# Belis0811/MaskUnet

Hardware: AMD Instinct MI355X
Metric: 128x128 images/sec (fwd+bwd) (higher is better)
Workload: dtype f16; 1 GPU; ADE20K-semantic shape 128x128, c_out=150, batch=64/GPU, 1-head MaskAttn-UNet fwd+bwd, train mode; global_batch=64, parallelism=dp1, mask_mode=fixed, loss=maskunet_amd.CrossEntropyLoss on module output, optimizer_in_step=False, hip_graph=False

## Files before the change

include/maskunet_hip.h:

```cpp
#ifndef MASKUNET_HIP_H
#define MASKUNET_HIP_H

#ifdef __cplusplus
extern "C" {
#endif

#define MU_OK 0
#define MU_ERR_ARG (-1)
#define MU_ERR_SHAPE (-2)
#define MU_ERR_LAUNCH (-3)
#define MU_ERR_WORKSPACE (-4)

#define MU_F32 0
#define MU_F16 1
#define MU_F32X 2

#define MU_ACT_NONE 0
#define MU_ACT_GELU 1
#define MU_ACT_RELU 2

const char* mu_version_host(void);

int mu_transpose(const void* src, int src_dtype, long src_ld, void* dst, int dst_dtype, long dst_ld, int batch, int R, int C,
                 void* stream);
int mu_transpose_pad(const void* src, int src_dtype, long src_ld, void* dst, int dst_dtype, long dst_ld, int batch, int R, int C,
                     int R_pad, void* stream);
int mu_split_encode(const void* src, void* dst, long n_elems, void* stream);
int mu_split_encode_h4(const void* src, void* dst, long n_elems, void* stream);
int mu_split_encode_h4x(const void* src, void* dst, void* dst16, long n_elems, void* stream);
long mu_dy_encode_h_workspace_bytes(void);
int mu_dy_encode_h(const void* dy, void* dy_h, float* dy_scale, long n_elems, void* workspace, long ws_bytes, void* stream);
int mu_split_encode_h(const void* src, void* dst, long n_elems, void* stream);
int mu_conv1x1_fwd_enc_h(const void* x, const void* w, const float* bias, void* y, long M, int Cin, int Cout, long x_ld, long y_ld,
                         void* stream);
int mu_cast(const void* src, int src_dtype, void* dst, int dst_dtype, long n, void* stream);
int mu_prep_weight(const float* w_oihw, void* dst, int dtype, int O, int I, int taps, int rows_pad, int cols_pad, int mode,
                   void* stream);

int mu_prep_weights_multi(const void* jobs, int njobs, long ntiles, void* dst_base, int dtype, void* stream);

int mu_prep_qkv(const float* wq, const float* wk, const float* wv, const float* bq, const float* bk, const float* bv, void* dst,
                float* bias, int dtype, int C, void* stream);

int mu_conv_fwd(const void* x, const void* w, const float* bias, void* y, int B, int H, int W, int Cin, int Cout, int taps, long x_ld,
                long y_ld, int dtype, void* stream);
int mu_conv1x1_add_supported(int Cin, int Cout, int dtype);
int mu_conv1x1_fwd_add(const void* x, const void* w, const void* addend, void* y, long M, int Cin, int Cout, long x_ld, long y_ld, int dtype,
                       void* stream);
int mu_conv_fwd_fused(const void* x, const void* w, const float* scale, const float* shift, const void* res, int act, void* y, int B, int H,
                      int W, int Cin, int Cout, int taps, long x_ld, long y_ld, int dtype, void* stream);
int mu_conv_stats_rows(int B, int H, int W, int Cin, int Cout, int taps, int dtype);
int mu_conv_fwd_stats(const void* x, const void* w, const float* bias, void* y, int B, int H, int W, int Cin, int Cout, int taps,
                      long x_ld, long y_ld, int dtype, float* stat_part, void* stream);
int mu_conv_fwd_plan(int B, int H, int W, int Cin, int Cout, int taps, int dtype, int with_stats);
int mu_conv_fwd_fused_plan(int B, int H, int W, int Cin, int Cout, int taps, int dtype);
int mu_conv_dgrad_h_plan(int B, int H, int W, int Cin, int Cout);
int mu_conv_wgrad_plan(int B, int H, int W, int Cin, int Cout, int taps, int cin_valid, int dtype, int pair);
int mu_conv_wgrad_bias_plan(int B, int H, int W, int Cin, int Cout, int taps, int cin_valid, int dtype);
int mu_conv_plan_count(int op);
const char* mu_conv_plan_name(int op, int id);
int mu_conv_dgrad_h(const void* dy_h, const void* w_hl, const float* dy_scale, void* dx, int B, int H, int W, int Cin, int Cout, long dy_ld,
                    long dx_ld, void* stream);
long mu_conv_wgrad_h_workspace_bytes(int B, int H, int W, int Cin, int Cout);
int mu_conv_wgrad_h(const void* x, const void* dy_h, const float* dy_scale, float* dw_oihw, int B, int H, int W, int Cin, int Cout,
                    int cin_valid, int cout_valid, long x_ld, long dy_ld, void* workspace, long ws_bytes, void* stream);
int mu_conv_wgrad_h1(const void* x_h, const void* dy_h, const float* dy_scale, float* dw_oihw, int B, int H, int W, int Cin, int Cout,
                     int cin_valid, int cout_valid, long x_ld, long dy_ld, void* workspace, long ws_bytes, void* stream);
long mu_conv_wgrad_workspace_bytes(int B, int H, int W, int Cin, int Cout, int taps);
int mu_conv_wgrad(const void* x, const void* dy, float* dw_oihw, int B, int H, int W, int Cin, int Cout, int taps, int cin_valid,
                  int cout_valid, long x_ld, long dy_ld, void* workspace, long ws_bytes, int dtype, void* stream);
int mu_conv_wgrad_bias_supported(int Cin, int Cout, int taps, int dtype);
int mu_conv_wgrad_bias(const void* x, const void* dy, float* dw_oihw, float* db, int B, int H, int W, int Cin, int Cout, int taps,
                       int cin_valid, int cout_valid, long x_ld, long dy_ld, void* workspace, long ws_bytes, int dtype, void* stream);
long mu_colsum_workspace_bytes(int C);
int mu_colsum(const void* x, long M, int C, long ld, float* out, void* workspace, long ws_bytes, int dtype, void* stream);

long mu_bn_workspace_bytes(int C);
int mu_bn_train_stats(const void* x, long M, int C, long ld, float* mean, float* rstd, float* running_mean, float* running_var,
                      long* num_batches_tracked, int c_valid, float momentum, float eps, void* workspace, long ws_bytes, int dtype,
                      void* stream);
int mu_bn_train_stats_rows(const float* stat_part, int rows, long M, int C, float* mean, float* rstd, float* running_mean,
                           float* running_var, long* num_batches_tracked, int c_valid, float momentum, float eps, void* workspace,
                           long ws_bytes, void* stream);
int mu_bn_eval_stats(const float* running_mean, const float* running_var, float eps, float* mean, float* rstd, int C, int c_valid,
                     void* stream);
int mu_bn_eval_fold(const float* running_mean1, const float* running_var1, const float* gamma1, const float* beta1, float eps1,
                    const float* running_mean2, const float* running_var2, const float* gamma2, const float* beta2, float eps2,
                    const float* conv_bias, float* scale, float* shift, int C, int c_valid, void* stream);
int mu_bn_act_fwd(const void* x, const void* res, void* y, long M, int C, long ld, const float* mean, const float* rstd,
                  const float* gamma, const float* beta, int act, int dtype, void* stream);
int mu_bn_act_fwd_enc(const void* x, const void* res, void* y_enc, void* y16, long M, int C, const float* mean, const float* rstd,
                      const float* gamma, const float* beta, int act, void* stream);
int mu_bn_act_bwd(const void* x, const void* res, const void* grad_out, void* dx, void* dres, long M, int C, long ld,
                  const float* mean, const float* rstd, const float* gamma, const float* beta, int act, int training, float* dgamma,
                  float* dbeta, void* workspace, long ws_bytes, int dtype, void* stream);
int mu_bn_pair_compose(const float* rstd1, const float* gamma1, const float* beta1, const float* gamma2, int C, int c_valid, long M,
                       float eps1, float eps2, float momentum2, float* running_mean2, float* running_var2,
                       long* num_batches_tracked2, float* gamma_eff, float* xhat_scale, float* dgamma2_coef, float* dgamma1_coef,
                       void* stream);
int mu_bn_act_bwd_scaled(const void* x, const void* res, const void* grad_out, void* dx, void* dres, long M, int C, long ld,
                         const float* mean, const float* rstd, const float* gamma, const float* beta, int act, int training,
                         float* dgamma, float* dbeta, const float* xhat_scale, void* workspace, long ws_bytes, int dtype, void* stream);

int mu_bn_pair_bwd(const void* x, const void* grad_out, void* dx, long M, int C, long ld, const float* mean, const float* rstd,
                   const float* gamma_eff, const float* beta2, const float* xhat_scale, const float* dgamma2_coef,
                   const float* dgamma1_coef, float* pair_grads, float* dbeta2, void* workspace, long ws_bytes, int dtype, void* stream);

int mu_bn_act_bwd_h(const void* x, const void* res, const void* grad_out, void* dx_h, void* dres, long M, int C, const float* mean,
                    const float* rstd, const float* gamma, const float* beta, int act, int training, float* dgamma, float* dbeta,
                    float* dy_scale, void* workspace, long ws_bytes, void* stream);
int mu_bn_pair_bwd_h(const void* x, const void* grad_out, void* dx_h, long M, int C, const float* mean, const float* rstd,
                     const float* gamma_eff, const float* beta2, const float* xhat_scale, const float* dgamma2_coef,
                     const float* dgamma1_coef, float* pair_grads, float* dbeta2, float* dy_scale, void* workspace, long ws_bytes,
                     void* stream);

long mu_ln_sample_workspace_bytes(int B);
int mu_ln_sample_fwd(const void* x, const float* w, const float* b, void* y, float* mean, float* rstd, int B, long L, float eps,
                     void* workspace, long ws_bytes, int dtype, void* stream);
int mu_ln_sample_bwd(const void* x, const void* dy, const float* w, const float* mean, const float* rstd, void* dx, float* dw,
                     float* db, int B, long L, void* workspace, long ws_bytes, int dtype, void* stream);

int mu_maxpool2_fwd(const void* x, void* y, int B, int H, int W, int C, int dtype, void* stream);
int mu_maxpool2_bwd(const void* x, const void* dy, void* dx, int B, int H, int W, int C, int dtype, void* stream);
int mu_maxpool2_bwd_acc(const void* x, const void* dy, const void* dy2, const void* dx_add, void* dx, int B, int H, int W, int C, int dtype,
                        void* stream);
int mu_upcat_fwd(const void* x, const void* skip, void* y, int B, int h, int w, int Cx, int Cs, int dtype, void* stream);
int mu_upcat_bwd(const void* dy, void* dx, void* dskip, int B, int h, int w, int Cx, int Cs, int dtype, void* stream);
int mu_upcat_bwd_acc(const void* dy, const void* dy2, void* dx, void* dskip, int B, int h, int w, int Cx, int Cs, int dtype, void* stream);
int mu_upcat_compact_fwd(const void* x, const void* skip, void* y, int B, int h, int w, int Cx_ld, int Cx_valid, int Cs_ld, int Cs_valid,
                         int Ct_ld, int dtype, void* stream);
int mu_upcat_compact_bwd(const void* dy, void* dx, void* dskip, int B, int h, int w, int Cx_ld, int Cx_valid, int Cs_ld, int Cs_valid,
                         int Ct_ld, int dtype, void* stream);
int mu_dropout(const void* x, void* y, long n, float p, unsigned long long seed, const unsigned char* mask, unsigned char* mask_out,
               int dtype, void* stream);
int mu_dropout_step(const void* x, void* y, long n, float p, unsigned long long seed, const unsigned long long* seed_step,
                    const unsigned char* mask, unsigned char* mask_out, int dtype, void* stream);

int mu_add(const void* a, const void* b, void* out, long n, int dtype, void* stream);

int mu_compact_keys(const void* keep, int keep_elem_bytes, int B, int N, int* kidx, int* kcnt, unsigned char* keep8, void* stream);
int mu_attn_fwd(const void* qkv, const void* x, const int* kidx, const int* kcnt, const float* gamma, const float* beta, void* out,
                void* oattn, float* lse2, float* ln_mean, float* ln_rstd, int B, int N, int C, int nkmax, float eps, int dtype,
                void* stream);
long mu_attn_bwd_workspace_bytes(int B, int N, int C);
int mu_attn_bwd(const void* qkv, const void* x, const void* oattn, const void* grad_out, const int* kidx, const int* kcnt,
                const float* lse2, const float* ln_mean, const float* ln_rstd, const float* gamma, void* dY, float* delta, void* dqkv,
                float* dgamma, float* dbeta, int B, int N, int C, int nkmax, void* workspace, long ws_bytes, int dtype, void* stream);
int mu_attn_fwd_padded(const void* qkv, const void* x, const int* kidx, const int* kcnt, const float* gamma, const float* beta, void* out,
                       void* oattn, float* lse2, float* ln_mean, float* ln_rstd, int B, int N, int C, int c_valid, int nkmax, float eps,
                       int dtype, void* stream);
int mu_attn_bwd_phases_padded(const void* qkv, const void* x, const void* oattn, const void* grad_out, const int* kidx, const int* kcnt,
                              const float* lse2, const float* ln_mean, const float* ln_rstd, const float* gamma, void* dY, float* delta,
                              void* dqkv, float* dgamma, float* dbeta, int B, int N, int C, int c_valid, int nkmax, void* workspace,
                              long ws_bytes, int dtype, int phases, void* stream);
int mu_gather_rows(const void* src, long src_ld, const int* idx, const int* cnt, void* dst, int rows_out, int C, int dtype, void* stream);
int mu_scatter_rows(const float* src, const int* idx, const int* cnt, void* dst, long dst_ld, int dst_rows, int C, int dtype, void* stream);
int mu_softmax_rows(void* S, int N, int ld, const int* cnt, float scale, int dtype, void* stream);
int mu_attn_wide_ds(const void* P, void* dP, int N, int ld, const int* cnt, float scale, int dtype, void* stream);
int mu_ln_rows_fwd(const void* o, const void* x, const float* gamma, const float* beta, void* out, float* mean, float* rstd, long rows,
                   int C, int c_valid, float eps, int dtype, void* stream);
int mu_ln_rows_bwd(const void* grad_out, const void* o, const void* x, const float* mean, const float* rstd, const float* gamma, void* dY,
                   void* g_xhat, long rows, int C, int c_valid, int dtype, void* stream);
#define MU_ATTN_KIDX_PERMUTATION 8
#define MU_ATTN_DQKV_ENCODED 16
int mu_attn_bwd_phases(const void* qkv, const void* x, const void* oattn, const void* grad_out, const int* kidx, const int* kcnt,
                       const float* lse2, const float* ln_mean, const float* ln_rstd, const float* gamma, void* dY, float* delta,
                       void* dqkv, float* dgamma, float* dbeta, int B, int N, int C, int nkmax, void* workspace, long ws_bytes,
                       int dtype, int phases, void* stream);

long mu_ce_workspace_bytes(void);
int mu_ce_fwd(const void* logits, const long* labels, long M, int Cp, int C, long ignore_index, float* lse, float* loss, float* count,
              void* workspace, long ws_bytes, int dtype, void* stream);
int mu_ce_bwd(const void* logits, const long* labels, const float* lse, const float* count, const float* grad_out, float grad_scale,
              long M, int Cp, int C, long ignore_index, void* dlogits, int dtype, void* stream);
int mu_ce_nchw_fwd(const void* logits, const long* labels, int B, int C, long HW, long ignore_index, float* lse, float* loss,
                   float* count, void* workspace, long ws_bytes, int dtype, void* stream);
int mu_ce_nchw_bwd(const void* logits, const long* labels, const float* lse, const float* count, const float* grad_out,
                   float grad_scale, int B, int C, long HW, long ignore_index, void* dlogits, int dtype, void* stream);
int mu_mean_iou(const void* logits, const long* labels, long M, int C, long inner, long outer_stride, long c_stride, long p_stride,
                float smooth, unsigned int* counts, float* out, int dtype, void* stream);
long mu_inst_triplet_workspace_bytes(int id_cap, int max_inst);
int mu_inst_triplet_fwd(const float* feat, const long* mask, int B, int C, int H, int W, int ignore_label, float margin,
                        const float* u, int id_cap, int max_inst, void* workspace, long ws_bytes, float* loss, void* stream);
int mu_inst_triplet_bwd(const float* feat, int B, int C, int H, int W, const void* workspace, int id_cap, int max_inst,
                        const float* grad_out, float* dfeat, void* stream);
int mu_argmax_prob(const void* logits, long M, int C, long inner, long outer_stride, long c_stride, long p_stride,
                   float inv_temperature, int* cls, float* prob_or_null, int dtype, void* stream);
long mu_instances_workspace_bytes(int B, int H, int W, int max_inst);
int mu_instances_supported(int H, int W, int max_inst);
int mu_instances(const int* cls, const float* prob_or_null, int B, int H, int W, int max_inst, int* ids, int* table, float* score,
                 int* count, int* order, void* workspace, long ws_bytes, void* stream);
long mu_dbscan_workspace_bytes(int B, int H, int W, int num_classes, int max_inst);
int mu_dbscan_supported(int H, int W, int D, int num_classes, int max_inst);
int mu_dbscan_instances(const int* cls, const void* emb, int B, int H, int W, int D, long inner, long outer_stride, long c_stride,
                        long p_stride, int dtype, int num_classes, float eps, int min_samples, int max_inst, int* ids, int* table,
                        float* score, int* count, int* order, void* workspace, long ws_bytes, void* stream);
#define MU_IDMAP_I32 0
#define MU_IDMAP_I64 1
#define MU_IDMAP_RGB8 2
int mu_id_instances_supported(int H, int W, int max_inst, int class_cap);
long mu_id_instances_workspace_bytes(int B, int H, int W, int max_inst, int class_cap);
int mu_id_instances(const void* id_map, int id_kind, const int* sem, int B, int H, int W, int max_inst, int class_cap, int* ids,
                    int* table, float* score, int* count, int* order, int* values, int* invalid, void* workspace, long ws_bytes,
                    void* stream);
#define MU_SEM_EVAL_LDS_MAX_C 192
int mu_sem_eval_supported(int C);
long mu_sem_eval_workspace_bytes(int B, long HW, int C);
int mu_sem_eval(const void* logits, const long* labels, int B, long HW, int C, long inner, long outer_stride, long c_stride,
                long p_stride, long ignore_index, float inv_temperature, int* img_counts, double* img_loss, long* confusion,
                int* cls_or_null, float* prob_or_null, void* workspace, long ws_bytes, int dtype, void* stream);
int mu_instance_pairs_supported(int H, int W, int max_inst_pred, int max_inst_gt);
long mu_instance_pairs_workspace_bytes(int B, int H, int W, int max_inst_pred, int max_inst_gt);
int mu_instance_pairs(const int* pred_ids, const int* gt_ids, int B, int H, int W, int max_inst_pred, int max_inst_gt, int* pairs,
                      int* n_pairs, void* workspace, long ws_bytes, void* stream);
int mu_instance_match_supported(int H, int W, int max_inst_pred, int max_inst_gt, int num_classes, int K, int max_dets, int T);
long mu_instance_match_workspace_bytes(int B, int K);
int mu_instance_match(const int* pairs, const int* n_pairs, const int* pred_table, const float* pred_score, const int* pred_order,
                      const int* pred_count, const int* gt_table, const int* gt_count, int B, int H, int W, int max_inst_pred,
                      int max_inst_gt, int num_classes, int K, int max_dets, const double* thr, int T, int* det_valid, int* det_class,
                      float* det_score, int* det_gt, double* det_iou, int* gt_per_class, int* pq_gt, double* pq_iou, int* pq_fp,
                      int* overflow, void* workspace, long ws_bytes, void* stream);
int mu_coco_match_supported(int H, int W, int max_inst_pred, int max_inst_gt, int num_classes, int K, int max_dets, int T, int A);
long mu_coco_match_workspace_bytes(int B, int K);
int mu_coco_match(const int* pairs, const int* n_pairs, const int* pred_table, const float* pred_score, const int* pred_order,
                  const int* pred_count, const int* gt_table, const int* gt_count, const int* gt_crowd_or_null,
                  const double* gt_area_or_null, int B, int H, int W, int max_inst_pred, int max_inst_gt, int num_classes, int K,
                  int max_dets, const double* thr, int T, const double* area_rng, int A, int* det_valid, int* det_class, int* det_rank,
                  float* det_score, int* det_gt, double* det_iou, unsigned char* det_ignore, int* gt_counted, int* pq_gt_per_class,
                  int* pq_gt, double* pq_iou, int* pq_fp, int* overflow, void* workspace, long ws_bytes, void* stream);
int mu_rle_encode_supported(int H, int W, int K, int max_id);
long mu_rle_encode_workspace_bytes(int B, int H, int W, int K, int max_id);
int mu_rle_encode(const int* ids, const int* sel, int B, int H, int W, int K, int max_id, int* offsets, int* counts, int* area,
                  int* str_offsets, unsigned char* str_bytes, void* workspace, long ws_bytes, void* stream);
int mu_rle_decode_supported(int H, int W, int K);
int mu_rle_decode(const int* offsets, const int* counts, int B, int H, int W, int K, long counts_per_image, int* ids, int* valid,
                  void* stream);
int mu_coco_masks_supported(int Ho, int Wo, int max_points);
long mu_coco_masks_workspace_bytes(int B, int A, int Ho, int Wo);
int mu_coco_masks(const double* xy, const int* poly_offsets, const int* ann_poly_offsets, const int* rle_counts, const int* ann_rle_offsets,
                  const int* img_ann_offsets, const int* sizes, int B, int A, int P, long n_points, long n_counts, int Ho, int Wo,
                  int max_points, long* cover, int* ids, unsigned char* masks_or_null, int* area, int* valid, void* workspace,
                  long ws_bytes, void* stream);
int mu_u8_to_nhwc(const unsigned char* src, void* dst, long npix, int C, int Cp, int dtype, void* stream);
int mu_resize_u8_nhwc(const unsigned char* src, int B, int Hs, int Ws, int C, int swap_rb, void* dst, unsigned char* u8_out, int Hd, int Wd,
                      int Cp, int dtype, void* stream);
int mu_resize_nearest_u8(const unsigned char* src, int B, int Hs, int Ws, long* dst, int Hd, int Wd, void* stream);
long mu_pil_resize_workspace_bytes(int B, int max_h, int max_w, int Hd, int Wd);
int mu_pil_resize_u8_nhwc(const unsigned char* src, const long* offsets, const int* sizes, int B, int C, int max_h, int max_w, int swap_rb,
// ... 14 lines not shown
```

maskunet_amd/_lib.py:

```python
from __future__ import annotations

import ctypes
import os
from ctypes import c_char_p, c_float, c_int, c_long, c_ulonglong, c_void_p

import torch

_HERE = os.path.dirname(os.path.abspath(__file__))
LIB_PATH = os.environ.get("MU_LIB_PATH") or os.path.join(_HERE, "libmaskunet_hip.so")

MU_F32, MU_F16, MU_F32X = 0, 1, 2
ACT_NONE, ACT_GELU, ACT_RELU = 0, 1, 2
MU_IDMAP_I32, MU_IDMAP_I64, MU_IDMAP_RGB8 = 0, 1, 2
_ERR = {-1: "MU_ERR_ARG", -2: "MU_ERR_SHAPE", -3: "MU_ERR_LAUNCH", -4: "MU_ERR_WORKSPACE"}

P, I, L, F = c_void_p, c_int, c_long, c_float
SIGNATURES = {
    "mu_version_host": (c_char_p, []),
    "mu_transpose": (I, [P, I, L, P, I, L, I, I, I, P]),
    "mu_transpose_pad": (I, [P, I, L, P, I, L, I, I, I, I, P]),
    "mu_cast": (I, [P, I, P, I, L, P]),
    "mu_split_encode": (I, [P, P, L, P]),
    "mu_split_encode_h": (I, [P, P, L, P]),
    "mu_split_encode_h4": (I, [P, P, L, P]),
    "mu_split_encode_h4x": (I, [P, P, P, L, P]),
    "mu_conv_wgrad_h1": (I, [P, P, P, P, I, I, I, I, I, I, I, L, L, P, L, P]),
    "mu_bn_act_fwd_enc": (I, [P, P, P, P, L, I, P, P, P, P, I, P]),
    "mu_dy_encode_h_workspace_bytes": (L, []),
    "mu_dy_encode_h": (I, [P, P, P, L, P, L, P]),
    "mu_conv_dgrad_h": (I, [P, P, P, P, I, I, I, I, I, L, L, P]),
    "mu_conv_wgrad_h_workspace_bytes": (L, [I, I, I, I, I]),
    "mu_conv_wgrad_h": (I, [P, P, P, P, I, I, I, I, I, I, I, L, L, P, L, P]),
    "mu_bn_act_bwd_h": (I, [P, P, P, P, P, L, I, P, P, P, P, I, I, P, P, P, P, L, P]),
    "mu_bn_pair_bwd_h": (I, [P, P, P, L, I, P, P, P, P, P, P, P, P, P, P, P, L, P]),
    "mu_conv1x1_fwd_enc_h": (I, [P, P, P, P, L, I, I, L, L, P]),
    "mu_prep_weight": (I, [P, P, I, I, I, I, I, I, I, P]),
    "mu_conv_fwd": (I, [P, P, P, P, I, I, I, I, I, I, L, L, I, P]),
    "mu_conv_stats_rows": (I, [I, I, I, I, I, I, I]),
    "mu_conv_fwd_plan": (I, [I, I, I, I, I, I, I, I]),
    "mu_conv_fwd_fused_plan": (I, [I, I, I, I, I, I, I]),
    "mu_conv_dgrad_h_plan": (I, [I, I, I, I, I]),
    "mu_conv_wgrad_plan": (I, [I, I, I, I, I, I, I, I, I]),
    "mu_conv_wgrad_bias_plan": (I, [I, I, I, I, I, I, I, I]),
    "mu_conv_plan_count": (I, [I]),
    "mu_conv_plan_name": (c_char_p, [I, I]),
    "mu_conv_fwd_stats": (I, [P, P, P, P, I, I, I, I, I, I, L, L, I, P, P]),
    "mu_conv_wgrad_workspace_bytes": (L, [I, I, I, I, I, I]),
    "mu_conv_wgrad": (I, [P, P, P, I, I, I, I, I, I, I, I, L, L, P, L, I, P]),
    "mu_conv_wgrad_bias_supported": (I, [I, I, I, I]),
    "mu_conv_wgrad_bias": (I, [P, P, P, P, I, I, I, I, I, I, I, I, L, L, P, L, I, P]),
    "mu_colsum_workspace_bytes": (L, [I]),
    "mu_colsum": (I, [P, L, I, L, P, P, L, I, P]),
    "mu_bn_workspace_bytes": (L, [I]),
    "mu_bn_train_stats": (I, [P, L, I, L, P, P, P, P, P, I, F, F, P, L, I, P]),
    "mu_bn_train_stats_rows": (I, [P, I, L, I, P, P, P, P, P, I, F, F, P, L, P]),
    "mu_bn_eval_stats": (I, [P, P, F, P, P, I, I, P]),
    "mu_bn_act_fwd": (I, [P, P, P, L, I, L, P, P, P, P, I, I, P]),
    "mu_bn_act_bwd": (I, [P, P, P, P, P, L, I, L, P, P, P, P, I, I, P, P, P, L, I, P]),
    "mu_bn_pair_compose": (I, [P, P, P, P, I, I, L, F, F, F, P, P, P, P, P, P, P, P]),
    "mu_bn_act_bwd_scaled": (I, [P, P, P, P, P, L, I, L, P, P, P, P, I, I, P, P, P, P, L, I, P]),
    "mu_bn_pair_bwd": (I, [P, P, P, L, I, L, P, P, P, P, P, P, P, P, P, P, L, I, P]),
    "mu_ln_sample_workspace_bytes": (L, [I]),
    "mu_ln_sample_fwd": (I, [P, P, P, P, P, P, I, L, F, P, L, I, P]),
    "mu_ln_sample_bwd": (I, [P, P, P, P, P, P, P, P, I, L, P, L, I, P]),
    "mu_maxpool2_fwd": (I, [P, P, I, I, I, I, I, P]),
    "mu_maxpool2_bwd": (I, [P, P, P, I, I, I, I, I, P]),
    "mu_upcat_fwd": (I, [P, P, P, I, I, I, I, I, I, P]),
    "mu_upcat_bwd": (I, [P, P, P, I, I, I, I, I, I, P]),
    "mu_upcat_compact_fwd": (I, [P, P, P, I, I, I, I, I, I, I, I, I, P]),
    "mu_upcat_compact_bwd": (I, [P, P, P, I, I, I, I, I, I, I, I, I, P]),
    "mu_dropout": (I, [P, P, L, F, c_ulonglong, P, P, I, P]),
    "mu_dropout_step": (I, [P, P, L, F, c_ulonglong, P, P, P, I, P]),
    "mu_add": (I, [P, P, P, L, I, P]),
    "mu_attn_fwd": (I, [P, P, P, P, P, P, P, P, P, P, P, I, I, I, I, F, I, P]),
    "mu_attn_bwd_workspace_bytes": (L, [I, I, I]),
    "mu_attn_bwd": (I, [P, P, P, P, P, P, P, P, P, P, P, P, P, P, P, I, I, I, I, P, L, I, P]),
    "mu_gather_rows": (I, [P, L, P, P, P, I, I, I, P]),
    "mu_scatter_rows": (I, [P, P, P, P, L, I, I, I, P]),
    "mu_softmax_rows": (I, [P, I, I, P, F, I, P]),
    "mu_attn_wide_ds": (I, [P, P, I, I, P, F, I, P]),
    "mu_ln_rows_fwd": (I, [P, P, P, P, P, P, P, L, I, I, F, I, P]),
    "mu_ln_rows_bwd": (I, [P, P, P, P, P, P, P, P, L, I, I, I, P]),
    "mu_ce_workspace_bytes": (L, []),
    "mu_ce_fwd": (I, [P, P, L, I, I, L, P, P, P, P, L, I, P]),
    "mu_ce_bwd": (I, [P, P, P, P, P, F, L, I, I, L, P, I, P]),
    "mu_ce_nchw_fwd": (I, [P, P, I, I, L, L, P, P, P, P, L, I, P]),
    "mu_ce_nchw_bwd": (I, [P, P, P, P, P, F, I, I, L, L, P, I, P]),
    "mu_mean_iou": (I, [P, P, L, I, L, L, L, L, F, P, P, I, P]),
    "mu_sem_eval_supported": (I, [I]),
    "mu_sem_eval_workspace_bytes": (L, [I, L, I]),
    "mu_sem_eval": (I, [P, P, I, L, I, L, L, L, L, L, F, P, P, P, P, P, P, L, I, P]),
    "mu_inst_triplet_workspace_bytes": (L, [I, I]),
    "mu_inst_triplet_fwd": (I, [P, P, I, I, I, I, I, F, P, I, I, P, L, P, P]),
    "mu_inst_triplet_bwd": (I, [P, I, I, I, I, P, I, I, P, P, P]),
    "mu_argmax_prob": (I, [P, L, I, L, L, L, L, F, P, P, I, P]),
    "mu_instances_workspace_bytes": (L, [I, I, I, I]),
    "mu_instances_supported": (I, [I, I, I]),
    "mu_instances": (I, [P, P, I, I, I, I, P, P, P, P, P, P, L, P]),
    "mu_dbscan_workspace_bytes": (L, [I, I, I, I, I]),
    "mu_dbscan_supported": (I, [I, I, I, I, I]),
    "mu_dbscan_instances": (I, [P, P, I, I, I, I, L, L, L, L, I, I, F, I, I, P, P, P, P, P, P, L, P]),
    "mu_id_instances_supported": (I, [I, I, I, I]),
    "mu_id_instances_workspace_bytes": (L, [I, I, I, I, I]),
    "mu_id_instances": (I, [P, I, P, I, I, I, I, I] + [P] * 8 + [L, P]),
    "mu_instance_pairs_supported": (I, [I, I, I, I]),
    "mu_instance_pairs_workspace_bytes": (L, [I, I, I, I, I]),
    "mu_instance_pairs": (I, [P, P, I, I, I, I, I, P, P, P, L, P]),
    "mu_instance_match_supported": (I, [I, I, I, I, I, I, I, I]),
    "mu_instance_match_workspace_bytes": (L, [I, I]),
    "mu_instance_match": (I, [P] * 8 + [I] * 8 + [P, I] + [P] * 10 + [P, L, P]),
    "mu_coco_match_supported": (I, [I, I, I, I, I, I, I, I, I]),
    "mu_coco_match_workspace_bytes": (L, [I, I]),
    "mu_coco_match": (I, [P] * 10 + [I] * 8 + [P, I, P, I] + [P] * 13 + [P, L, P]),
    "mu_rle_encode_supported": (I, [I, I, I, I]),
    "mu_rle_encode_workspace_bytes": (L, [I, I, I, I, I]),
    "mu_rle_encode": (I, [P, P, I, I, I, I, I, P, P, P, P, P, P, L, P]),
    "mu_rle_decode_supported": (I, [I, I, I]),
    "mu_rle_decode": (I, [P, P, I, I, I, I, L, P, P, P]),
    "mu_coco_masks_supported": (I, [I, I, I]),
    "mu_coco_masks_workspace_bytes": (L, [I, I, I, I]),
    "mu_coco_masks": (I, [P] * 7 + [I, I, I, L, L, I, I, I] + [P] * 6 + [L, P]),
    "mu_u8_to_nhwc": (I, [P, P, L, I, I, I, P]),
    "mu_adamw_chunk": (I, []),
    "mu_adamw_multi": (I, [P, P, P, I, I, F, F, F, F, F, F, P, P, I, P, P]),
    "mu_prep_qkv": (I, [P, P, P, P, P, P, P, P, I, I, P]),
    "mu_prep_weights_multi": (I, [P, I, L, P, I, P]),
    "mu_conv1x1_add_supported": (I, [I, I, I]),
    "mu_conv1x1_fwd_add": (I, [P, P, P, P, L, I, I, L, L, I, P]),
    "mu_maxpool2_bwd_acc": (I, [P, P, P, P, P, I, I, I, I, I, P]),
    "mu_upcat_bwd_acc": (I, [P, P, P, P, I, I, I, I, I, I, P]),
    "mu_compact_keys": (I, [P, I, I, I, P, P, P, P]),
    "mu_resize_u8_nhwc": (I, [P, I, I, I, I, I, P, P, I, I, I, I, P]),
    "mu_resize_nearest_u8": (I, [P, I, I, I, P, I, I, P]),
    "mu_pil_resize_workspace_bytes": (L, [I, I, I, I, I]),
    "mu_pil_resize_u8_nhwc": (I, [P, P, P, I, I, I, I, I, P, P, P, I, I, I, I, P, L, P]),
    "mu_conv_fwd_fused": (I, [P, P, P, P, P, I, P, I, I, I, I, I, I, L, L, I, P]),
    "mu_bn_eval_fold": (I, [P, P, P, P, F, P, P, P, P, F, P, P, P, I, I, P]),
    "mu_attn_bwd_phases": (I, [P, P, P, P, P, P, P, P, P, P, P, P, P, P, P, I, I, I, I, P, L, I, I, P]),
    "mu_clock_probe": (I, [P, P, I, I, P]),
    "mu_attn_fwd_padded": (I, [P, P, P, P, P, P, P, P, P, P, P, I, I, I, I, I, F, I, P]),
    "mu_attn_bwd_phases_padded": (I, [P, P, P, P, P, P, P, P, P, P, P, P, P, P, P, I, I, I, I, I, P, L, I, I, P]),
}

_lib = None


def load() -> ctypes.CDLL:
    global _lib
    if _lib is not None:
        return _lib
    if not os.path.exists(LIB_PATH):
        raise RuntimeError(
            f"maskunet_amd: HIP library not found at {LIB_PATH}. It must be built (hipcc --offload-arch=gfx950): "
            "run `make -C maskunet_amd/csrc` or `python -c 'import __graft_entry__ as g; g.build()'`. "
            "There is no CPU fallback.")
    lib = ctypes.CDLL(LIB_PATH)
    for name, (res, args) in SIGNATURES.items():
        if os.environ.get("MU_LIB_PATH") and not hasattr(lib, name):
            continue
        fn = getattr(lib, name)
        fn.restype = res
        fn.argtypes = args
    _lib = lib
    return lib


def dt(t_or_dtype) -> int:
    d = t_or_dtype.dtype if isinstance(t_or_dtype, torch.Tensor) else t_or_dtype
    if d == torch.float32:
        return MU_F32
    if d == torch.float16:
        return MU_F16
    raise TypeError(f"maskunet_amd supports float32 and float16 compute, got {d}")


F32_MATMUL_PRECISION = os.environ.get("MU_F32_MATMUL", "highest")
if F32_MATMUL_PRECISION not in ("highest", "high"):
    raise ValueError(f'MU_F32_MATMUL must be "highest" or "high", got {F32_MATMUL_PRECISION!r}')


def set_float32_matmul_precision(precision: str):
    global F32_MATMUL_PRECISION
    if precision not in ("highest", "high"):
        raise ValueError('precision must be "highest" or "high"')
    F32_MATMUL_PRECISION = precision


def get_float32_matmul_precision() -> str:
    return F32_MATMUL_PRECISION


def mdt(t_or_dtype) -> int:
    d = dt(t_or_dtype)
    return MU_F32X if (d == MU_F32 and F32_MATMUL_PRECISION == "high") else d


def ptr(t):
    if t is None:
        return None
# ... 54 lines not shown
```

maskunet_amd/csrc/conv.hip:

```cpp
#include "common.h"
#include <stdlib.h>
#include <type_traits>
#include "../../include/maskunet_hip.h"

template <typename T> struct Mma;
template <> struct Mma<h16> {
    static constexpr int VN = 8;
    using Frag = h16x8;
    static __device__ __forceinline__ Frag ld(const void* p) { return *reinterpret_cast<const Frag*>(p); }
    static __device__ __forceinline__ void mma(const Frag& a, const Frag& b, f32x4& c) {
        c = __builtin_amdgcn_mfma_f32_16x16x32_f16(a, b, c, 0, 0, 0);
    }
    static constexpr bool PAIR = false;
    using Frag2 = Frag;
    static __device__ __forceinline__ Frag2 ld2(const void* p0, const void*) { return ld(p0); }
    static __device__ __forceinline__ void mma2(const Frag2& a, const Frag2& b, f32x4& c) { mma(a, b, c); }
};
template <> struct Mma<xf32> {
    static constexpr int VN = 4;
    using Frag = SplitF4;
    static __device__ __forceinline__ Frag ld(const void* p) { return mu_frag_enc(*reinterpret_cast<const uint4*>(p)); }
    static __device__ __forceinline__ void mma(const Frag& a, const Frag& b, f32x4& c) { mu_mma_split(a, b, c); }
    static constexpr bool PAIR = true;
    using Frag2 = SplitF8;
// ... 357 lines not shown
    for (int i = 0; i < TM; ++i)
#pragma unroll
        for (int j = 0; j < TN; ++j) acc[i][j] = (f32x4){0.f, 0.f, 0.f, 0.f};

    stage(0, 0);
    __syncthreads();
    for (int s = 0; s < nsteps; ++s) {
        const int buf = s & 1;
        if (s + 1 < nsteps) stage(s + 1, buf ^ 1);
        const char* Ab = lds + buf * STAGE;
        const char* Bb = Ab + BCO * 128;
        if constexpr (M_::PAIR) {
            typename M_::Frag2 a[TM], b[TN];
#pragma unroll
            for (int i = 0; i < TM; ++i) {
                const int row = (wr * TM + i) * 16 + r16;
                a[i] = M_::ld2(Ab + row * 128 + ((g ^ (row & 7)) << 4), Ab + row * 128 + (((4 + g) ^ (row & 7)) << 4));
            }
#pragma unroll
            for (int j = 0; j < TN; ++j) {
                const int row = (wc * TN + j) * 16 + r16;
                b[j] = M_::ld2(Bb + row * 128 + ((g ^ (row & 7)) << 4), Bb + row * 128 + (((4 + g) ^ (row & 7)) << 4));
            }
#pragma unroll
            for (int i = 0; i < TM; ++i)
#pragma unroll
                for (int j = 0; j < TN; ++j) M_::mma2(a[i], b[j], acc[i][j]);
        } else {
#pragma unroll
        for (int kk = 0; kk < 2; ++kk) {
            Frag a[TM], b[TN];
#pragma unroll
            for (int i = 0; i < TM; ++i) {
                const int row = (wr * TM + i) * 16 + r16;
                a[i] = M_::ld(Ab + row * 128 + (((kk * 4 + g) ^ (row & 7)) << 4));
            }
#pragma unroll
            for (int j = 0; j < TN; ++j) {
                const int row = (wc * TN + j) * 16 + r16;
                b[j] = M_::ld(Bb + row * 128 + (((kk * 4 + g) ^ (row & 7)) << 4));
            }
#pragma unroll
            for (int i = 0; i < TM; ++i)
#pragma unroll
                for (int j = 0; j < TN; ++j) M_::mma(a[i], b[j], acc[i][j]);
        }
        }
        __syncthreads();
    }
    mma_unshift<T>(acc);

    if constexpr (EPI) {
#pragma unroll
        for (int j = 0; j < TN; ++j) {
            const int px = (wc * TN + j) * 16 + r16;
#pragma unroll
            for (int i = 0; i < TM; ++i) {
                const int co = (wr * TM + i) * 16 + 4 * g;
                float v[4];
#pragma unroll
                for (int r = 0; r < 4; ++r) {
                    const bool in = co0 + co + r < Cout;
                    v[r] = acc[i][j][r];
                    if constexpr (FEPI) { if (scale && in) v[r] *= scale[co0 + co + r]; }
                    v[r] += (bias && in ? bias[co0 + co + r] : 0.f);
                }
                h16x4 o = {(h16)v[0], (h16)v[1], (h16)v[2], (h16)v[3]};
                *reinterpret_cast<h16x4*>(lds + px * OPITCH + co * 2) = o;
            }
        }
        __syncthreads();
        constexpr int CH = BCO / 8;
        for (int idx = tid; idx < BPX * CH; idx += 256) {
            const int px = idx / CH, ch = idx - px * CH;
            const long p = px0 + px;
            if (p < Mtot && co0 + ch * 8 < Cout) {
                uint4 o = *reinterpret_cast<const uint4*>(lds + px * OPITCH + ch * 16);
                if constexpr (FEPI) {
                    uint4 a4 = make_uint4(0, 0, 0, 0);
                    if (addend) a4 = *reinterpret_cast<const uint4*>(addend + p * y_ld + co0 + ch * 8);
                    const h16x8 ov = *reinterpret_cast<const h16x8*>(&o), av = *reinterpret_cast<const h16x8*>(&a4);
                    h16x8 r;
#pragma unroll
                    for (int e = 0; e < 8; ++e) r[e] = (h16)epi_act<T>((float)ov[e] + (float)av[e], act);
                    o = *reinterpret_cast<const uint4*>(&r);
                }
                *reinterpret_cast<uint4*>(y + p * y_ld + co0 + ch * 8) = o;
            }
        }
        return;
    }
#pragma unroll
    for (int j = 0; j < TN; ++j) {
        const long p = px0 + (wc * TN + j) * 16 + r16;
        if (p >= Mtot) continue;
#pragma unroll
        for (int i = 0; i < TM; ++i) {
            const int co = co0 + (wr * TM + i) * 16 + 4 * g;
            if (co >= Cout) continue;
            float v[4];
#pragma unroll
            for (int r = 0; r < 4; ++r) {
                v[r] = acc[i][j][r];
                if constexpr (FEPI) { if (scale) v[r] *= scale[co + r]; }
                v[r] += (bias ? bias[co + r] : 0.f);
                if constexpr (FEPI) v[r] = epi_act<T>(v[r] + (addend ? (float)addend[p * y_ld + co + r] : 0.f), act);
            }
            if constexpr (sizeof(T) == 2) {
                h16x4 o = {(h16)v[0], (h16)v[1], (h16)v[2], (h16)v[3]};
                *reinterpret_cast<h16x4*>(y + p * y_ld + co) = o;
            } else {
                if constexpr (std::is_same<T, xf32>::value && !FEPI) {
                    if (act == MU_NT2_ENC_H) {
                        uint32_t h0, h1, l0, l1;
                        mu_hsplit2(v[0], v[1], h0, l0);
                        mu_hsplit2(v[2], v[3], h1, l1);
                        char* gp = reinterpret_cast<char*>(y + p * y_ld + (co & ~7)) + (g & 1) * 8;
                        *reinterpret_cast<uint2*>(gp) = make_uint2(h0, h1);
                        *reinterpret_cast<uint2*>(gp + 16) = make_uint2(l0, l1);
                        continue;
                    }
                }
                *reinterpret_cast<float4*>(y + p * y_ld + co) = make_float4(v[0], v[1], v[2], v[3]);
            }
        }
    }
}


__device__ __forceinline__ void tile_stats_accum(const h16x8& o, float (&ssum)[8], float (&ssq)[8]) {
#pragma unroll
    for (int c = 0; c < 8; ++c) {
        const float v = (float)o[c];
        ssum[c] += v;
        ssq[c] = fmaf(v, v, ssq[c]);
    }
}
__device__ __forceinline__ void tile_stats_store(float (&ssum)[8], float (&ssq)[8], float* __restrict__ row, int co, int lane) {
#pragma unroll
    for (int c = 0; c < 8; ++c) {
#pragma unroll
        for (int m = 8; m < 64; m <<= 1) {
            ssum[c] += __shfl_xor(ssum[c], m);
            ssq[c] += __shfl_xor(ssq[c], m);
        }
    }
    if (lane < 8) {
#pragma unroll
        for (int c = 0; c < 8; c += 2)
            *reinterpret_cast<float4*>(row + (co + c) * 2) = make_float4(ssum[c], ssq[c], ssum[c + 1], ssq[c + 1]);
    }
}

template <typename T, int TM, int TN, int WR, bool RINGP, bool FEPI, int HL = 0>
__device__ __forceinline__ void conv_nt3_body(const T* __restrict__ x, const T* __restrict__ w, const float* __restrict__ bias,
                                              T* __restrict__ y, int B, int H, int W, int Cin, int Cout, long x_ld, long y_ld,
                                              const float* __restrict__ scale, const T* __restrict__ res, int act,
                                              float* __restrict__ stat_part = nullptr, float* __restrict__ yf = nullptr,
                                              const float* __restrict__ oscale = nullptr) {
    using M_ = Mma<T>;
    using Frag = typename M_::Frag;
    constexpr int VN = M_::VN, KC = 8 * VN;
    constexpr int NWV = 4;
    constexpr int WC = NWV / WR;
    constexpr int BCO = WR * TM * 16;
    constexpr int TH = WC * TN, TW = 16, HW_ = TW + 2;
    constexpr int HROWS = (TH + 2) * HW_;
    constexpr int HINST = (HROWS + 7) / 8;
    static_assert((HINST + NWV - 1) / NWV <= 9, "halo does not fit the 9 tap steps");
    constexpr int PA = BCO / (8 * NWV);
    static_assert(BCO % (8 * NWV) == 0, "weight tile rows must split over the waves");
    constexpr int HBYTES = HINST * 1024, WBYTES = BCO * 128;
    constexpr bool RING = RINGP && sizeof(T) == 2 && BCO == 64;
    constexpr int NWS = RING ? 3 : 2;

    __shared__ __attribute__((aligned(16))) char lds[2 * HBYTES + NWS * WBYTES + (RING ? 1024 : 0)];
    char* Hs = lds;
    char* Ws = lds + 2 * HBYTES;
    char* dump = lds + 2 * HBYTES + NWS * WBYTES;

    const int tiles_w = W / TW, tiles_h = H / TH;
    const int ntile = B * tiles_h * tiles_w, ncb = Cout / BCO;
    const int L = xcd_remap(blockIdx.x, ntile * ncb);
    const int cb = L % ncb, tl = L / ncb;
    const int co0 = cb * BCO;
    const int tw_ = tl % tiles_w, th_ = (tl / tiles_w) % tiles_h, bimg = tl / (tiles_w * tiles_h);
    const int h0 = th_ * TH, w0 = tw_ * TW;

    const int tid = threadIdx.x, lane = tid & 63, wave = tid >> 6;
    const int wr = wave / WC, wc = wave % WC;
    const int r16 = lane & 15, g = lane >> 4;
    const int srow = lane >> 3, sch = lane & 7;

    constexpr bool HL2 = HL == 2;
    const int kchunks = HL2 ? 2 * (Cin / KC) : Cin / KC;
    const int Cw = HL ? 2 * Cin : Cin;
    const int nsteps = 9 * kchunks;

    int wl[PA];
#pragma unroll
    for (int i = 0; i < PA; ++i) {
        const int row = (i * NWV + wave) * 8 + srow;
        wl[i] = (co0 + row) * Cw + (sch ^ (row & 7)) * VN;
    }
    constexpr int HPW = (HINST + NWV - 1) / NWV;
    int hl[HPW];
#pragma unroll
    for (int k = 0; k < HPW; ++k) {
        const int hr = (k * NWV + wave) * 8 + srow;
        const int hy = hr / HW_, hx = hr - hy * HW_;
        const int hh = h0 - 1 + hy, ww = w0 - 1 + hx;
        const bool ok = (k * NWV + wave) < HINST && hr < HROWS && hh >= 0 && hh < H && ww >= 0 && ww < W;
        hl[k] = ok ? (int)(((long)hh * W + ww) * x_ld) + (sch ^ (hx & 7)) * VN : -1;
    }
    const T* xb = x + (long)bimg * H * W * x_ld;

    auto stage_w = [&](int s, int buf) {
        const int tap = s % 9, c_ = s / 9;
        const int ci0 = HL2 ? ((c_ & 1) ? Cin : 0) + (c_ >> 1) * KC : c_ * KC;
        const T* wb = w + (long)tap * Cout * Cw + ci0;
        char* Wb = Ws + buf * WBYTES;
#pragma unroll
        for (int i = 0; i < PA; ++i) glds16(wb + wl[i], Wb + (i * NWV + wave) * 1024);
    };
    auto stage_h = [&](int k, int ci0, int buf) {
        const void* src = hl[k] >= 0 ? (const void*)(xb + hl[k] + ci0) : (const void*)mu_zero_page;
        glds16(src, Hs + buf * HBYTES + (k * NWV + wave) * 1024);
    };
    auto hchunk = [&](int c) { return HL2 ? (c >> 1) : c; };
    auto next_h = [&](int c) { return c + 1 < kchunks && (!HL2 || ((c + 1) & 1) == 0); };

    f32x4 acc[TM][TN];
#pragma unroll
    for (int i = 0; i < TM; ++i)
#pragma unroll
        for (int j = 0; j < TN; ++j) acc[i][j] = (f32x4){0.f, 0.f, 0.f, 0.f};

    int aoff[2], boff[3][2];
#pragma unroll
    for (int kk = 0; kk < 2; ++kk) {
        aoff[kk] = (wr * TM * 16 + r16) * 128 + (((kk * 4 + g) ^ (r16 & 7)) << 4);
#pragma unroll
        for (int dw = 0; dw < 3; ++dw) boff[dw][kk] = (wc * TN * HW_ + r16 + dw) * 128 + (((kk * 4 + g) ^ ((r16 + dw) & 7)) << 4);
    }

    stage_w(0, 0);
    if constexpr (RING) { if (nsteps > 1) stage_w(1, 1); }
#pragma unroll
    for (int k = 0; k < HPW; ++k)
        if (k * NWV + wave < HINST) stage_h(k, 0, 0);
    __syncthreads();

    int s = 0, wslot = 0;
    for (int c = 0; c < kchunks; ++c) {
        const int hbuf = (hchunk(c) & 1) * HBYTES;
#pragma unroll
        for (int dh = 0; dh < 3; ++dh) {
#pragma unroll
            for (int dw = 0; dw < 3; ++dw, ++s) {
                const int t = dh * 3 + dw;
                if constexpr (RING) {
                    const int nslot = wslot == 0 ? 2 : wslot - 1;
                    if (s + 2 < nsteps) stage_w(s + 2, nslot);
                    else {
#pragma unroll
                        for (int i = 0; i < PA; ++i) glds16(mu_zero_page, dump);
                    }
                    if (t < HPW && next_h(c) && t * NWV + wave < HINST) stage_h(t, hchunk(c + 1) * KC, hchunk(c + 1) & 1);
                    else glds16(mu_zero_page, dump);
                } else {
                if (s + 1 < nsteps) stage_w(s + 1, (s + 1) & 1);
                if (t < HPW && next_h(c) && t * NWV + wave < HINST)
                    stage_h(t, hchunk(c + 1) * KC, hchunk(c + 1) & 1);
                }
                const char* Wb = Ws + (RING ? wslot : (s & 1)) * WBYTES;
                const char* Hb = Hs + hbuf + dh * (HW_ * 128);
                if constexpr (M_::PAIR) {
                    typename M_::Frag2 a[TM], b[TN];
#pragma unroll
                    for (int i = 0; i < TM; ++i) a[i] = M_::ld2(Wb + aoff[0] + i * 2048, Wb + aoff[1] + i * 2048);
#pragma unroll
                    for (int j = 0; j < TN; ++j) b[j] = M_::ld2(Hb + boff[dw][0] + j * (HW_ * 128), Hb + boff[dw][1] + j * (HW_ * 128));
#pragma unroll
                    for (int i = 0; i < TM; ++i)
#pragma unroll
                        for (int j = 0; j < TN; ++j) M_::mma2(a[i], b[j], acc[i][j]);
                } else {
#pragma unroll
                for (int kk = 0; kk < 2; ++kk) {
                    Frag a[TM], b[TN];
                    const char* wa = Wb + aoff[kk];
                    const char* hb = Hb + boff[dw][kk];
#pragma unroll
                    for (int i = 0; i < TM; ++i) a[i] = M_::ld(wa + i * 2048);
#pragma unroll
                    for (int j = 0; j < TN; ++j) b[j] = M_::ld(hb + j * (HW_ * 128));
#pragma unroll
                    for (int i = 0; i < TM; ++i)
#pragma unroll
                        for (int j = 0; j < TN; ++j) M_::mma(a[i], b[j], acc[i][j]);
                }
                }
                if constexpr (RING) {
                    asm volatile("s_waitcnt vmcnt(%0)" ::"n"(PA + 1) : "memory");
                    __builtin_amdgcn_sched_barrier(0);
                    __builtin_amdgcn_s_barrier();
                    __builtin_amdgcn_sched_barrier(0);
                    wslot = wslot == 2 ? 0 : wslot + 1;
                } else {
                    __syncthreads();
                }
            }
        }
    }
    if constexpr (RING) {
        asm volatile("s_waitcnt vmcnt(0)" ::: "memory");
        __builtin_amdgcn_s_barrier();
    }

    mma_unshift<T>(acc);
    if constexpr (HL) {
        const float os = oscale[1] * (1.0f / (float)(1 << MU_XH_WSHIFT));
#pragma unroll
        for (int j = 0; j < TN; ++j) {
            const long p = ((long)bimg * H + h0 + wc * TN + j) * W + w0 + r16;
#pragma unroll
            for (int i = 0; i < TM; ++i) {
                const int co = co0 + (wr * TM + i) * 16 + 4 * g;
                *reinterpret_cast<f32x4*>(yf + p * y_ld + co) = acc[i][j] * os;
            }
        }
        return;
    }
    if constexpr (sizeof(T) == 2 && TM == 4) {
        char* Os = lds + wave * (TN * 16 * 128);
#pragma unroll
        for (int j = 0; j < TN; ++j) {
            const int p = j * 16 + r16;
#pragma unroll
            for (int i = 0; i < TM; ++i) {
                const int co = i * 16 + 4 * g;
                float v[4];
#pragma unroll
                for (int r = 0; r < 4; ++r) {
                    v[r] = acc[i][j][r];
                    if constexpr (FEPI) { if (scale) v[r] *= scale[co0 + wr * 64 + co + r]; }
                    v[r] += (bias ? bias[co0 + wr * 64 + co + r] : 0.f);
                }
                h16x4 o = {(h16)v[0], (h16)v[1], (h16)v[2], (h16)v[3]};
                *reinterpret_cast<h16x4*>(Os + p * 128 + (((co >> 2) ^ (((p >> 1) & 7) << 1)) << 3)) = o;
            }
        }
        const int q = lane & 7;
        float ssum[8] = {0.f, 0.f, 0.f, 0.f, 0.f, 0.f, 0.f, 0.f}, ssq[8] = {0.f, 0.f, 0.f, 0.f, 0.f, 0.f, 0.f, 0.f};
#pragma unroll
        for (int it = 0; it < TN * 2; ++it) {
            const int p = it * 8 + (lane >> 3);
            h16x8 o = *reinterpret_cast<const h16x8*>(Os + p * 128 + ((q ^ ((p >> 1) & 7)) << 4));
            const long gp = ((long)bimg * H + h0 + wc * TN + (p >> 4)) * W + w0 + (p & 15);
            if constexpr (FEPI) {
                h16x8 rv = (h16x8)(h16)0;
                if (res) rv = *reinterpret_cast<const h16x8*>(res + gp * y_ld + co0 + wr * 64 + q * 8);
#pragma unroll
                for (int e = 0; e < 8; ++e) o[e] = (h16)epi_act<T>((float)o[e] + (float)rv[e], act);
            }
            *reinterpret_cast<h16x8*>(y + gp * y_ld + co0 + wr * 64 + q * 8) = o;
            if constexpr (!FEPI) { if (stat_part) tile_stats_accum(o, ssum, ssq); }
        }
        if constexpr (!FEPI) {
            if (stat_part) tile_stats_store(ssum, ssq, stat_part + ((long)tl * WC + wc) * Cout * 2, co0 + wr * 64 + q * 8, lane);
        }
        return;
    }
    float tsum[TM][4], tsq[TM][4];
#pragma unroll
    for (int i = 0; i < TM; ++i)
#pragma unroll
        for (int r = 0; r < 4; ++r) { tsum[i][r] = 0.f; tsq[i][r] = 0.f; }
#pragma unroll
    for (int j = 0; j < TN; ++j) {
        const long p = ((long)bimg * H + h0 + wc * TN + j) * W + w0 + r16;
#pragma unroll
        for (int i = 0; i < TM; ++i) {
            const int co = co0 + (wr * TM + i) * 16 + 4 * g;
            float v[4];
#pragma unroll
            for (int r = 0; r < 4; ++r) {
                v[r] = acc[i][j][r];
                if constexpr (FEPI) { if (scale) v[r] *= scale[co + r]; }
                v[r] += (bias ? bias[co + r] : 0.f);
                if constexpr (FEPI) v[r] = epi_act<T>(v[r] + (res ? (float)res[p * y_ld + co + r] : 0.f), act);
            }
            if constexpr (sizeof(T) == 2) {
                h16x4 o = {(h16)v[0], (h16)v[1], (h16)v[2], (h16)v[3]};
                *reinterpret_cast<h16x4*>(y + p * y_ld + co) = o;
            } else {
                *reinterpret_cast<float4*>(y + p * y_ld + co) = make_float4(v[0], v[1], v[2], v[3]);
                if constexpr (!FEPI) {
#pragma unroll
                    for (int r = 0; r < 4; ++r) { tsum[i][r] += v[r]; tsq[i][r] = fmaf(v[r], v[r], tsq[i][r]); }
                }
            }
        }
    }
    if constexpr (!FEPI && sizeof(T) == 4) {
        if (stat_part) {
            static_assert(TM == 4, "statistics epilogue: four channel fragments per wave");
            float v8[2][4][2], v4[4][2], v2[2][2], v1[2];
            const bool b3 = r16 & 8, b2 = r16 & 4, b1 = r16 & 2, b0 = r16 & 1;
#pragma unroll
            for (int i = 0; i < 2; ++i)
#pragma unroll
                for (int r = 0; r < 4; ++r) {
                    const float ks = b3 ? tsum[i + 2][r] : tsum[i][r], ss = b3 ? tsum[i][r] : tsum[i + 2][r];
                    const float kq = b3 ? tsq[i + 2][r] : tsq[i][r], sq = b3 ? tsq[i][r] : tsq[i + 2][r];
                    v8[i][r][0] = ks + __shfl_xor(ss, 8);
                    v8[i][r][1] = kq + __shfl_xor(sq, 8);
                }
#pragma unroll
            for (int r = 0; r < 4; ++r)
#pragma unroll
                for (int k = 0; k < 2; ++k) v4[r][k] = (b2 ? v8[1][r][k] : v8[0][r][k]) + __shfl_xor(b2 ? v8[0][r][k] : v8[1][r][k], 4);
#pragma unroll
            for (int r = 0; r < 2; ++r)
#pragma unroll
                for (int k = 0; k < 2; ++k) v2[r][k] = (b1 ? v4[r + 2][k] : v4[r][k]) + __shfl_xor(b1 ? v4[r][k] : v4[r + 2][k], 2);
#pragma unroll
            for (int k = 0; k < 2; ++k) v1[k] = (b0 ? v2[1][k] : v2[0][k]) + __shfl_xor(b0 ? v2[0][k] : v2[1][k], 1);
            float* row = stat_part + ((long)tl * WC + wc) * Cout * 2;
            *reinterpret_cast<float2*>(row + (co0 + (wr * TM + (r16 >> 2)) * 16 + 4 * g + (r16 & 3)) * 2) = make_float2(v1[0], v1[1]);
        }
    }
}


template <typename T, int TM, int TN, int WR, bool RINGP = false>
__global__ __launch_bounds__(256, 2) void conv_nt3_kernel(const T* __restrict__ x, const T* __restrict__ w, const float* __restrict__ bias,
                                                          T* __restrict__ y, int B, int H, int W, int Cin, int Cout, long x_ld, long y_ld,
                                                          float* __restrict__ stat_part = nullptr) {
    conv_nt3_body<T, TM, TN, WR, RINGP, false>(x, w, bias, y, B, H, W, Cin, Cout, x_ld, y_ld, nullptr, nullptr, 0, stat_part);
}
template <int TM, int TN, int WR, bool RINGP = false, int HL = 2>
__global__ __launch_bounds__(256, 2) void conv_nt3hl_kernel(const h16* __restrict__ dy, const h16* __restrict__ w, float* __restrict__ dx, int B, int H,
                                                            int W, int Cin, int Cout, long x_ld, long y_ld, const float* __restrict__ oscale) {
    conv_nt3_body<h16, TM, TN, WR, RINGP, false, HL>(dy, w, nullptr, nullptr, B, H, W, Cin, Cout, x_ld, y_ld, nullptr, nullptr, 0, nullptr, dx, oscale);
}
template <typename T, int TM, int TN, int WR>
__global__ __launch_bounds__(256, 2) void conv_nt3f_kernel(const T* __restrict__ x, const T* __restrict__ w, const float* __restrict__ bias,
                                                           T* __restrict__ y, int B, int H, int W, int Cin, int Cout, long x_ld, long y_ld,
                                                           const float* __restrict__ scale, const T* __restrict__ res, int act) {
    conv_nt3_body<T, TM, TN, WR, false, true>(x, w, bias, y, B, H, W, Cin, Cout, x_ld, y_ld, scale, res, act);
}

template <bool FEPI, int HL = 0>
__device__ __forceinline__ void conv_nt4_body(const h16* __restrict__ x, const h16* __restrict__ w, const float* __restrict__ bias,
                                              h16* __restrict__ y, int B, int H, int W, int Cin, int Cout, long x_ld, long y_ld,
                                              float* __restrict__ stat_part, const float* __restrict__ scale, const h16* __restrict__ res, int act,
                                              float* __restrict__ yf = nullptr, const float* __restrict__ oscale = nullptr) {
    using M_ = Mma<h16>;
    using Frag = M_::Frag;
    constexpr int VN = 8, KC = 64, TM = 4, TN = 4, WC = 4, NWV = 8, BCO = 128;
    constexpr int TH = 16, TW = 16, HW_ = TW + 2, HROWS = (TH + 2) * HW_;
    constexpr int HINST = (HROWS + 7) / 8;
    constexpr int HPW = 7;
    static_assert(HPW * NWV >= HINST, "halo does not fit the 7 tap steps");
    constexpr int HBYTES = HINST * 1024, WBYTES = BCO * 128, NWB = 4;

    __shared__ __attribute__((aligned(16))) char lds[2 * HBYTES + NWB * WBYTES + 1024];
    char* Hs = lds;
    char* Ws = lds + 2 * HBYTES;
    char* dump = lds + 2 * HBYTES + NWB * WBYTES;

    const int tiles_w = W / TW, tiles_h = H / TH;
    const int ntile = B * tiles_h * tiles_w, ncb = Cout / BCO;
    const int L = xcd_remap(blockIdx.x, ntile * ncb);
    const int cb = L % ncb, tl = L / ncb;
    const int co0 = cb * BCO;
    const int tw_ = tl % tiles_w, th_ = (tl / tiles_w) % tiles_h, bimg = tl / (tiles_w * tiles_h);
    const int h0 = th_ * TH, w0 = tw_ * TW;

    const int tid = threadIdx.x, lane = tid & 63, wave = __builtin_amdgcn_readfirstlane(tid >> 6);
    const int wr = wave >> 2, wc = wave & 3;
    const int r16 = lane & 15, g = lane >> 4;
    const int srow = lane >> 3, sch = lane & 7;

    constexpr bool HL2 = HL == 2;
    const int kchunks = HL2 ? 2 * (Cin / KC) : Cin / KC;
    const int Cw = HL ? 2 * Cin : Cin;
    const int nsteps = 9 * kchunks;

    int wl[2];
#pragma unroll
    for (int i = 0; i < 2; ++i) {
        const int row = (i * NWV + wave) * 8 + srow;
        wl[i] = (co0 + row) * Cw + (sch ^ (row & 7)) * VN;
    }
    int hl[HPW];
#pragma unroll
    for (int k = 0; k < HPW; ++k) {
        const int hr = (k * NWV + wave) * 8 + srow;
        const int hy = hr / HW_, hx = hr - hy * HW_;
        const int hh = h0 - 1 + hy, ww = w0 - 1 + hx;
        const bool ok = hr < HROWS && hh >= 0 && hh < H && ww >= 0 && ww < W;
        hl[k] = ok ? (int)(((long)hh * W + ww) * x_ld) + (sch ^ (hx & 7)) * VN : -1;
    }
    const h16* xb = x + (long)bimg * H * W * x_ld;

    auto stage_w = [&](int s) {
        if (s < nsteps) {
            const int tap = s % 9, c_ = s / 9;
            const int ci0 = HL2 ? ((c_ & 1) ? Cin : 0) + (c_ >> 1) * KC : c_ * KC;
            const h16* wb = w + (long)tap * Cout * Cw + ci0;
            char* Wb = Ws + (s & 3) * WBYTES;
#pragma unroll
            for (int i = 0; i < 2; ++i) glds16(wb + wl[i], Wb + (i * NWV + wave) * 1024);
        } else {
            glds16(mu_zero_page, dump);
            glds16(mu_zero_page, dump);
        }
    };
    auto stage_h = [&](int k, int c) {
        const int off = hl[k];
        const int hc = HL2 ? (c >> 1) : c;
        if (c < kchunks && (!HL2 || (c & 1) == 0) && k * NWV + wave < HINST) {
            const void* src = off >= 0 ? (const void*)(xb + off + hc * KC) : (const void*)mu_zero_page;
            glds16(src, Hs + (hc & 1) * HBYTES + (k * NWV + wave) * 1024);
        } else {
            glds16(mu_zero_page, dump);
        }
    };

    f32x4 acc[TM][TN];
#pragma unroll
    for (int i = 0; i < TM; ++i)
#pragma unroll
        for (int j = 0; j < TN; ++j) acc[i][j] = (f32x4){0.f, 0.f, 0.f, 0.f};

    int aoff[2], boff[3][2];
#pragma unroll
    for (int kk = 0; kk < 2; ++kk) {
        aoff[kk] = (wr * TM * 16 + r16) * 128 + (((kk * 4 + g) ^ (r16 & 7)) << 4);
#pragma unroll
        for (int dw = 0; dw < 3; ++dw) boff[dw][kk] = (wc * TN * HW_ + r16 + dw) * 128 + (((kk * 4 + g) ^ ((r16 + dw) & 7)) << 4);
    }

#pragma unroll
    for (int k = 0; k < HPW; ++k) stage_h(k, 0);
    stage_w(0);
    stage_w(1);
    stage_w(2);
    asm volatile("s_waitcnt vmcnt(0)" ::: "memory");
    __builtin_amdgcn_s_barrier();
    if (wr == 1) __builtin_amdgcn_s_barrier();

    int s = 0;
    for (int c = 0; c < kchunks; ++c) {
        const int hbuf = ((HL2 ? (c >> 1) : c) & 1) * HBYTES;
#pragma unroll
        for (int t = 0; t < 9; ++t, ++s) {
            const int dh = t / 3, dw = t % 3;
            const char* Wb = Ws + (s & 3) * WBYTES;
            const char* Hb = Hs + hbuf + dh * (HW_ * 128);
#pragma unroll
            for (int kk = 0; kk < 2; ++kk) {
                Frag a[TM], b[TN];
                const char* wa = Wb + aoff[kk];
                const char* hb = Hb + boff[dw][kk];
#pragma unroll
                for (int i = 0; i < TM; ++i) a[i] = M_::ld(wa + i * 2048);
#pragma unroll
                for (int j = 0; j < TN; ++j) b[j] = M_::ld(hb + j * (HW_ * 128));
                if ((kk == 0) == (t != 0)) {
                    if (t < HPW) stage_h(t, c + 1); else glds16(mu_zero_page, dump);
                }
                if (kk == 1) stage_w(s + 3);
                __builtin_amdgcn_s_barrier();
                asm volatile("s_waitcnt lgkmcnt(0)" ::: "memory");
                __builtin_amdgcn_sched_barrier(0);
                __builtin_amdgcn_s_setprio(1);
#pragma unroll
                for (int i = 0; i < TM; ++i)
#pragma unroll
                    for (int j = 0; j < TN; ++j) M_::mma(a[i], b[j], acc[i][j]);
                __builtin_amdgcn_s_setprio(0);
                if (kk == 0) {
                    if (t == 0) asm volatile("s_waitcnt vmcnt(3)" ::: "memory");
                    else asm volatile("s_waitcnt vmcnt(4)" ::: "memory");
                }
                __builtin_amdgcn_sched_barrier(0);
                __builtin_amdgcn_s_barrier();
            }
        }
    }
    if (wr == 0) __builtin_amdgcn_s_barrier();

    if constexpr (HL) {
        const float os = oscale[1] * (1.0f / (float)(1 << MU_XH_WSHIFT));
        char* Of = lds + wave * 16384;
#pragma unroll
        for (int j = 0; j < TN; ++j) {
            const int p = j * 16 + r16;
#pragma unroll
            for (int i = 0; i < TM; ++i) {
                const int co = i * 16 + 4 * g;
                *reinterpret_cast<f32x4*>(Of + p * 256 + ((((co >> 2)) ^ (p & 15)) << 4)) = acc[i][j] * os;
            }
        }
        const int q4 = lane & 15, pl = lane >> 4;
#pragma unroll
        for (int it = 0; it < 16; ++it) {
            const int p = it * 4 + pl;
            const f32x4 o = *reinterpret_cast<const f32x4*>(Of + p * 256 + ((q4 ^ (p & 15)) << 4));
            const long gp = ((long)bimg * H + h0 + wc * TN + (p >> 4)) * W + w0 + (p & 15);
            *reinterpret_cast<f32x4*>(yf + gp * y_ld + co0 + wr * 64 + q4 * 4) = o;
        }
        return;
    }
    char* Os = lds + wave * 8192;
#pragma unroll
    for (int j = 0; j < TN; ++j) {
        const int p = j * 16 + r16;
#pragma unroll
        for (int i = 0; i < TM; ++i) {
            const int co = i * 16 + 4 * g;
            float v[4];
#pragma unroll
            for (int r = 0; r < 4; ++r) {
                v[r] = acc[i][j][r];
                if constexpr (FEPI) { if (scale) v[r] *= scale[co0 + wr * 64 + co + r]; }
                v[r] += (bias ? bias[co0 + wr * 64 + co + r] : 0.f);
            }
            h16x4 o = {(h16)v[0], (h16)v[1], (h16)v[2], (h16)v[3]};
            *reinterpret_cast<h16x4*>(Os + p * 128 + (((co >> 2) ^ (((p >> 1) & 7) << 1)) << 3)) = o;
        }
    }
    const int q = lane & 7;
    float ssum[8] = {0.f, 0.f, 0.f, 0.f, 0.f, 0.f, 0.f, 0.f}, ssq[8] = {0.f, 0.f, 0.f, 0.f, 0.f, 0.f, 0.f, 0.f};
#pragma unroll
    for (int it = 0; it < 8; ++it) {
        const int p = it * 8 + (lane >> 3);
        h16x8 o = *reinterpret_cast<const h16x8*>(Os + p * 128 + ((q ^ ((p >> 1) & 7)) << 4));
        const long gp = ((long)bimg * H + h0 + wc * TN + (p >> 4)) * W + w0 + (p & 15);
        if constexpr (FEPI) {
            h16x8 rv = (h16x8)(h16)0;
            if (res) rv = *reinterpret_cast<const h16x8*>(res + gp * y_ld + co0 + wr * 64 + q * 8);
#pragma unroll
            for (int e = 0; e < 8; ++e) o[e] = (h16)epi_act<h16>((float)o[e] + (float)rv[e], act);
        }
        *reinterpret_cast<h16x8*>(y + gp * y_ld + co0 + wr * 64 + q * 8) = o;
        if (stat_part) tile_stats_accum(o, ssum, ssq);
    }
    if (stat_part) tile_stats_store(ssum, ssq, stat_part + ((long)tl * 4 + wc) * Cout * 2, co0 + wr * 64 + q * 8, lane);
}

__global__ __launch_bounds__(512, 1) void conv_nt4_kernel(const h16* __restrict__ x, const h16* __restrict__ w, const float* __restrict__ bias,
                                                          h16* __restrict__ y, int B, int H, int W, int Cin, int Cout, long x_ld, long y_ld,
                                                          float* __restrict__ stat_part) {
    conv_nt4_body<false>(x, w, bias, y, B, H, W, Cin, Cout, x_ld, y_ld, stat_part, nullptr, nullptr, 0);
}
template <int HL>
__global__ __launch_bounds__(512, 1) void conv_nt4hl_kernel(const h16* __restrict__ dy, const h16* __restrict__ w, float* __restrict__ dx, int B, int H,
                                                            int W, int Cin, int Cout, long x_ld, long y_ld, const float* __restrict__ oscale) {
    conv_nt4_body<false, HL>(dy, w, nullptr, nullptr, B, H, W, Cin, Cout, x_ld, y_ld, nullptr, nullptr, nullptr, 0, dx, oscale);
}
__global__ __launch_bounds__(512, 1) void conv_nt4f_kernel(const h16* __restrict__ x, const h16* __restrict__ w, const float* __restrict__ bias,
                                                           h16* __restrict__ y, int B, int H, int W, int Cin, int Cout, long x_ld, long y_ld,
                                                           const float* __restrict__ scale, const h16* __restrict__ res, int act) {
    conv_nt4_body<true>(x, w, bias, y, B, H, W, Cin, Cout, x_ld, y_ld, nullptr, scale, res, act);
}

template <typename XT>
__global__ __launch_bounds__(512, 1) void conv_nt4x_kernel(const XT* __restrict__ x, const XT* __restrict__ w, const float* __restrict__ bias,
                                                           XT* __restrict__ y, int B, int H, int W, int Cin, int Cout, long x_ld, long y_ld,
                                                           float* __restrict__ stat_part) {
    using M_ = Mma<XT>;
    using Frag2 = typename M_::Frag2;
    constexpr int VN = 4, KC = 32, TM = 4, TN = 4, NWV = 8, BCO = 128;
    constexpr int TH = 16, TW = 16, HW_ = TW + 2, HROWS = (TH + 2) * HW_;
    constexpr int HINST = (HROWS + 7) / 8;
    constexpr int HPW = 7;
    constexpr int HBYTES = HINST * 1024, WBYTES = BCO * 128, NWB = 4;

    __shared__ __attribute__((aligned(16))) char lds[2 * HBYTES + NWB * WBYTES + 1024];
    char* Hs = lds;
    char* Ws = lds + 2 * HBYTES;
    char* dump = lds + 2 * HBYTES + NWB * WBYTES;

    const int tiles_w = W / TW, tiles_h = H / TH;
    const int ntile = B * tiles_h * tiles_w, ncb = Cout / BCO;
    const int L = xcd_remap(blockIdx.x, ntile * ncb);
    const int cb = L % ncb, tl = L / ncb;
    const int co0 = cb * BCO;
    const int tw_ = tl % tiles_w, th_ = (tl / tiles_w) % tiles_h, bimg = tl / (tiles_w * tiles_h);
    const int h0 = th_ * TH, w0 = tw_ * TW;

    const int tid = threadIdx.x, lane = tid & 63, wave = __builtin_amdgcn_readfirstlane(tid >> 6);
    const int wr = wave >> 2, wc = wave & 3;
    const int r16 = lane & 15, g = lane >> 4;
    const int srow = lane >> 3, sch = lane & 7;

    const int kchunks = Cin / KC;
    const int nsteps = 9 * kchunks;

    int wl[2];
#pragma unroll
    for (int i = 0; i < 2; ++i) {
        const int row = (i * NWV + wave) * 8 + srow;
        wl[i] = (co0 + row) * Cin + (sch ^ (row & 7)) * VN;
    }
    int hl[HPW];
#pragma unroll
    for (int k = 0; k < HPW; ++k) {
        const int hr = (k * NWV + wave) * 8 + srow;
        const int hy = hr / HW_, hx = hr - hy * HW_;
        const int hh = h0 - 1 + hy, ww = w0 - 1 + hx;
        const bool ok = hr < HROWS && hh >= 0 && hh < H && ww >= 0 && ww < W;
        hl[k] = ok ? (int)(((long)hh * W + ww) * x_ld) + (sch ^ (hx & 7)) * VN : -1;
    }
    const XT* xb = x + (long)bimg * H * W * x_ld;

    auto stage_w = [&](int s) {
        if (s < nsteps) {
            const int tap = s % 9, ci0 = (s / 9) * KC;
            const XT* wb = w + (long)tap * Cout * Cin + ci0;
            char* Wb = Ws + (s & 3) * WBYTES;
#pragma unroll
            for (int i = 0; i < 2; ++i) glds16(wb + wl[i], Wb + (i * NWV + wave) * 1024);
        } else {
            glds16(mu_zero_page, dump);
            glds16(mu_zero_page, dump);
        }
    };
    auto stage_h = [&](int k, int c) {
        const int off = hl[k];
        if (c < kchunks && k * NWV + wave < HINST) {
            const void* src = off >= 0 ? (const void*)(xb + off + c * KC) : (const void*)mu_zero_page;
            glds16(src, Hs + (c & 1) * HBYTES + (k * NWV + wave) * 1024);
        } else {
            glds16(mu_zero_page, dump);
        }
    };

    f32x4 acc[TM][TN];
#pragma unroll
    for (int i = 0; i < TM; ++i)
#pragma unroll
        for (int j = 0; j < TN; ++j) acc[i][j] = (f32x4){0.f, 0.f, 0.f, 0.f};

    int aoff[2], boff[3][2];
#pragma unroll
    for (int kk = 0; kk < 2; ++kk) {
        aoff[kk] = (wr * TM * 16 + r16) * 128 + (((kk * 4 + g) ^ (r16 & 7)) << 4);
#pragma unroll
        for (int dw = 0; dw < 3; ++dw) boff[dw][kk] = (wc * TN * HW_ + r16 + dw) * 128 + (((kk * 4 + g) ^ ((r16 + dw) & 7)) << 4);
    }

#pragma unroll
    for (int k = 0; k < HPW; ++k) stage_h(k, 0);
    stage_w(0);
    stage_w(1);
    stage_w(2);
    asm volatile("s_waitcnt vmcnt(0)" ::: "memory");
    __builtin_amdgcn_s_barrier();
    if (wr == 1) __builtin_amdgcn_s_barrier();

    int s = 0;
    for (int c = 0; c < kchunks; ++c) {
        const int hbuf = (c & 1) * HBYTES;
#pragma unroll
        for (int t = 0; t < 9; ++t, ++s) {
            const int dh = t / 3, dw = t % 3;
            const char* Wb = Ws + (s & 3) * WBYTES;
            const char* Hb = Hs + hbuf + dh * (HW_ * 128);
            const char* wa0 = Wb + aoff[0];
            const char* wa1 = Wb + aoff[1];
            const char* hb0 = Hb + boff[dw][0];
            const char* hb1 = Hb + boff[dw][1];
            Frag2 a[TM], b[2];
#pragma unroll
            for (int i = 0; i < TM; ++i) a[i] = M_::ld2(wa0 + i * 2048, wa1 + i * 2048);
#pragma unroll
            for (int j = 0; j < 2; ++j) b[j] = M_::ld2(hb0 + j * (HW_ * 128), hb1 + j * (HW_ * 128));
            if (t != 0) {
                if (t < HPW) stage_h(t, c + 1); else glds16(mu_zero_page, dump);
            }
            __builtin_amdgcn_s_barrier();
            asm volatile("s_waitcnt lgkmcnt(0)" ::: "memory");
            __builtin_amdgcn_sched_barrier(0);
            __builtin_amdgcn_s_setprio(1);
#pragma unroll
            for (int i = 0; i < TM; ++i)
#pragma unroll
                for (int j = 0; j < 2; ++j) M_::mma2(a[i], b[j], acc[i][j]);
            __builtin_amdgcn_s_setprio(0);
            if (t == 0) asm volatile("s_waitcnt vmcnt(3)" ::: "memory");
            else asm volatile("s_waitcnt vmcnt(4)" ::: "memory");
            __builtin_amdgcn_sched_barrier(0);
            __builtin_amdgcn_s_barrier();
#pragma unroll
            for (int j = 0; j < 2; ++j) b[j] = M_::ld2(hb0 + (j + 2) * (HW_ * 128), hb1 + (j + 2) * (HW_ * 128));
            if (t == 0) stage_h(0, c + 1);
            stage_w(s + 3);
            __builtin_amdgcn_s_barrier();
            asm volatile("s_waitcnt lgkmcnt(0)" ::: "memory");
            __builtin_amdgcn_sched_barrier(0);
            __builtin_amdgcn_s_setprio(1);
#pragma unroll
            for (int i = 0; i < TM; ++i)
#pragma unroll
                for (int j = 0; j < 2; ++j) M_::mma2(a[i], b[j], acc[i][j + 2]);
            __builtin_amdgcn_s_setprio(0);
            __builtin_amdgcn_sched_barrier(0);
            __builtin_amdgcn_s_barrier();
        }
    }
    if (wr == 0) __builtin_amdgcn_s_barrier();

    mma_unshift<XT>(acc);
    char* Os = lds + wave * 16384;
#pragma unroll
    for (int j = 0; j < TN; ++j) {
        const int p = j * 16 + r16;
#pragma unroll
        for (int i = 0; i < TM; ++i) {
            const int co = i * 16 + 4 * g;
            f32x4 v = acc[i][j];
            if (bias) {
#pragma unroll
                for (int r = 0; r < 4; ++r) v[r] += bias[co0 + wr * 64 + co + r];
            }
            *reinterpret_cast<f32x4*>(Os + p * 256 + ((((co >> 2)) ^ (p & 15)) << 4)) = v;
        }
    }
    const int q = lane & 15, pl = lane >> 4;
    f32x4 ssum = {0.f, 0.f, 0.f, 0.f}, ssq = {0.f, 0.f, 0.f, 0.f};
#pragma unroll
    for (int it = 0; it < 16; ++it) {
        const int p = it * 4 + pl;
        const f32x4 o = *reinterpret_cast<const f32x4*>(Os + p * 256 + ((q ^ (p & 15)) << 4));
        const long gp = ((long)bimg * H + h0 + wc * TN + (p >> 4)) * W + w0 + (p & 15);
        *reinterpret_cast<f32x4*>(reinterpret_cast<float*>(y) + gp * y_ld + co0 + wr * 64 + q * 4) = o;
        if (stat_part) {
            ssum += o;
            ssq += o * o;
        }
    }
    if (stat_part) {
#pragma unroll
        for (int c = 0; c < 4; ++c) {
            ssum[c] += __shfl_xor(ssum[c], 16); ssq[c] += __shfl_xor(ssq[c], 16);
            ssum[c] += __shfl_xor(ssum[c], 32); ssq[c] += __shfl_xor(ssq[c], 32);
        }
        if (lane < 16) {
            float* row = stat_part + ((long)tl * 4 + wc) * Cout * 2 + (co0 + wr * 64 + q * 4) * 2;
            *reinterpret_cast<float4*>(row) = make_float4(ssum[0], ssq[0], ssum[1], ssq[1]);
            *reinterpret_cast<float4*>(row + 4) = make_float4(ssum[2], ssq[2], ssum[3], ssq[3]);
        }
    }
}

__global__ __launch_bounds__(512, 1) void conv_nt4p_kernel(const h16* __restrict__ x, const h16* __restrict__ w, const float* __restrict__ bias,
                                                           h16* __restrict__ y, int B, int H, int W, int Cin, int Cout, long x_ld, long y_ld,
                                                           float* __restrict__ stat_part) {
    using M_ = Mma<h16>;
    using Frag = M_::Frag;
    constexpr int VN = 8, KC = 64, TM = 4, TN = 4, NWV = 8, BCO = 128;
    constexpr int TH = 16, TW = 16, HW_ = TW + 2, HROWS = (TH + 2) * HW_;
    constexpr int HINST = (HROWS + 7) / 8;
    constexpr int HPW = 7;
    constexpr int HBYTES = HINST * 1024, WBYTES = BCO * 128, NWB = 4;

    __shared__ __attribute__((aligned(16))) char lds[2 * HBYTES + NWB * WBYTES + 1024 + 8192];
    char* Hs = lds;
    char* Ws = lds + 2 * HBYTES;
    char* dump = lds + 2 * HBYTES + NWB * WBYTES;
    char* spare = dump + 1024;

    const int tiles_w = W / TW, tiles_h = H / TH;
    const int ntile = B * tiles_h * tiles_w, ncb = Cout / BCO;
    const int nblk = gridDim.x / ncb;
    const int L = xcd_remap(blockIdx.x, gridDim.x);
    const int cb = L % ncb, bx = L / ncb;
    const int co0 = cb * BCO;

    const int tid = threadIdx.x, lane = tid & 63, wave = __builtin_amdgcn_readfirstlane(tid >> 6);
    const int wr = wave >> 2, wc = wave & 3;
    const int r16 = lane & 15, g = lane >> 4;
    const int srow = lane >> 3, sch = lane & 7;
    const int kchunks = Cin / KC;

    int wl[2];
#pragma unroll
    for (int i = 0; i < 2; ++i) {
        const int row = (i * NWV + wave) * 8 + srow;
        wl[i] = (co0 + row) * Cin + (sch ^ (row & 7)) * VN;
    }
    int hl[HPW];
    const h16* xb;
    auto halo_offsets = [&](int tl) {
        const int tw_ = tl % tiles_w, th_ = (tl / tiles_w) % tiles_h, bi = tl / (tiles_w * tiles_h);
        const int hh0 = th_ * TH - 1, ww0 = tw_ * TW - 1;
        xb = x + (long)bi * H * W * x_ld;
#pragma unroll
        for (int k = 0; k < HPW; ++k) {
            const int hr = (k * NWV + wave) * 8 + srow;
            const int hy = hr / HW_, hx = hr - hy * HW_;
            const int hh = hh0 + hy, ww = ww0 + hx;
            const bool ok = hr < HROWS && hh >= 0 && hh < H && ww >= 0 && ww < W;
            hl[k] = ok ? (int)(((long)hh * W + ww) * x_ld) + (sch ^ (hx & 7)) * VN : -1;
        }
    };
    auto stage_w = [&](int slot, int tap, int chunk, bool real) {
        if (real) {
            const h16* wb = w + (long)tap * Cout * Cin + chunk * KC;
            char* Wb = Ws + slot * WBYTES;
#pragma unroll
            for (int i = 0; i < 2; ++i) glds16a(wb + wl[i], Wb + (i * NWV + wave) * 1024);
        } else {
            glds16a(mu_zero_page, dump);
            glds16a(mu_zero_page, dump);
        }
    };
    auto stage_h = [&](int k, int chunk, int buf, bool real) {
        if (real && k * NWV + wave < HINST) {
            const int off = hl[k];
            const void* src = off >= 0 ? (const void*)(xb + off + chunk * KC) : (const void*)mu_zero_page;
            glds16a(src, Hs + buf * HBYTES + (k * NWV + wave) * 1024);
        } else {
            glds16a(mu_zero_page, dump);
        }
    };

    int aoff[2], boff[3][2];
#pragma unroll
    for (int kk = 0; kk < 2; ++kk) {
        aoff[kk] = (wr * TM * 16 + r16) * 128 + (((kk * 4 + g) ^ (r16 & 7)) << 4);
#pragma unroll
        for (int dw = 0; dw < 3; ++dw) boff[dw][kk] = (wc * TN * HW_ + r16 + dw) * 128 + (((kk * 4 + g) ^ ((r16 + dw) & 7)) << 4);
    }

    int tl = bx;
    if (tl >= ntile) return;
    halo_offsets(tl);

#pragma unroll
    for (int k = 0; k < HPW; ++k) stage_h(k, 0, 0, true);
#pragma unroll
    for (int q = 0; q < 3; ++q) stage_w(q, q % 9, q / 9, q < 9 * kchunks);
    asm volatile("s_waitcnt vmcnt(0)" ::: "memory");
    __builtin_amdgcn_s_barrier();
    if (wr == 1) __builtin_amdgcn_s_barrier();

    int sg = 0, G = 0;
    for (; tl < ntile; tl += nblk) {
        const bool has_next = tl + nblk < ntile;
        f32x4 acc[TM][TN];
#pragma unroll
        for (int i = 0; i < TM; ++i)
#pragma unroll
            for (int j = 0; j < TN; ++j) acc[i][j] = (f32x4){0.f, 0.f, 0.f, 0.f};

        for (int c = 0; c < kchunks; ++c, ++G) {
            const int hbuf = (G & 1) * HBYTES;
            const bool last_chunk = c + 1 == kchunks;
            if (last_chunk) { if (has_next) halo_offsets(tl + nblk); }
            else if (c == 0) halo_offsets(tl);
            const bool pf_real = !last_chunk || has_next;
            const int pf_chunk = last_chunk ? 0 : c + 1;
#pragma unroll
            for (int t = 0; t < 9; ++t, ++sg) {
                const int dh = t / 3, dw = t % 3;
                const char* Wb = Ws + (sg & 3) * WBYTES;
                const char* Hb = Hs + hbuf + dh * (HW_ * 128);
#pragma unroll
                for (int kk = 0; kk < 2; ++kk) {
                    Frag a[TM], b[TN];
                    const char* wa = Wb + aoff[kk];
                    const char* hb = Hb + boff[dw][kk];
#pragma unroll
                    for (int i = 0; i < TM; ++i) a[i] = M_::ld(wa + i * 2048);
#pragma unroll
                    for (int j = 0; j < TN; ++j) b[j] = M_::ld(hb + j * (HW_ * 128));
                    if ((kk == 0) == (t != 0)) {
                        if (t < HPW) stage_h(t, pf_chunk, (G + 1) & 1, pf_real);
                        else glds16a(mu_zero_page, dump);
                    }
                    if (kk == 1) {
                        const int t3 = (t + 3) % 9, c3 = c + (t + 3) / 9;
                        if (c3 < kchunks) stage_w((sg + 3) & 3, t3, c3, true);
                        else stage_w((sg + 3) & 3, t3, 0, has_next);
                    }
                    __builtin_amdgcn_s_barrier();
                    asm volatile("s_waitcnt lgkmcnt(0)" ::: "memory");
                    __builtin_amdgcn_sched_barrier(0);
                    __builtin_amdgcn_s_setprio(1);
#pragma unroll
                    for (int i = 0; i < TM; ++i)
#pragma unroll
                        for (int j = 0; j < TN; ++j) M_::mma(a[i], b[j], acc[i][j]);
                    __builtin_amdgcn_s_setprio(0);
                    if (kk == 0) {
                        if (t == 0) { if (c == 0) asm volatile("s_waitcnt vmcnt(11)" ::: "memory"); else asm volatile("s_waitcnt vmcnt(3)" ::: "memory"); }
                        else if (t == 1) { if (c == 0) asm volatile("s_waitcnt vmcnt(12)" ::: "memory"); else asm volatile("s_waitcnt vmcnt(4)" ::: "memory"); }
                        else asm volatile("s_waitcnt vmcnt(4)" ::: "memory");
                    }
                    __builtin_amdgcn_sched_barrier(0);
                    __builtin_amdgcn_s_barrier();
                }
            }
        }
        if (wr == 0) __builtin_amdgcn_s_barrier();

        char* Os = wave < 5 ? Hs + ((G - 1) & 1) * HBYTES + wave * 8192
                            : (wave < 7 ? Ws + ((sg + 3) & 3) * WBYTES + (wave - 5) * 8192 : spare);
        const int tw_ = tl % tiles_w, th_ = (tl / tiles_w) % tiles_h, bimg = tl / (tiles_w * tiles_h);
        const int h0 = th_ * TH, w0 = tw_ * TW;
#pragma unroll
        for (int j = 0; j < TN; ++j) {
            const int p = j * 16 + r16;
#pragma unroll
            for (int i = 0; i < TM; ++i) {
                const int co = i * 16 + 4 * g;
                float v[4];
#pragma unroll
                for (int r = 0; r < 4; ++r) v[r] = acc[i][j][r] + (bias ? bias[co0 + wr * 64 + co + r] : 0.f);
                h16x4 o = {(h16)v[0], (h16)v[1], (h16)v[2], (h16)v[3]};
                *reinterpret_cast<h16x4*>(Os + p * 128 + (((co >> 2) ^ (((p >> 1) & 7) << 1)) << 3)) = o;
            }
        }
        {
            const int q = lane & 7;
            float ssum[8] = {0.f, 0.f, 0.f, 0.f, 0.f, 0.f, 0.f, 0.f}, ssq[8] = {0.f, 0.f, 0.f, 0.f, 0.f, 0.f, 0.f, 0.f};
#pragma unroll
            for (int it = 0; it < 8; ++it) {
                const int p = it * 8 + (lane >> 3);
                const h16x8 o = *reinterpret_cast<const h16x8*>(Os + p * 128 + ((q ^ ((p >> 1) & 7)) << 4));
                const long gp = ((long)bimg * H + h0 + wc * TN + (p >> 4)) * W + w0 + (p & 15);
                *reinterpret_cast<h16x8*>(y + gp * y_ld + co0 + wr * 64 + q * 8) = o;
                if (stat_part) tile_stats_accum(o, ssum, ssq);
            }
            if (stat_part) tile_stats_store(ssum, ssq, stat_part + ((long)tl * 4 + wc) * Cout * 2, co0 + wr * 64 + q * 8, lane);
        }
        if (has_next && wr == 1) __builtin_amdgcn_s_barrier();
    }
}

__global__ __launch_bounds__(512, 1) void conv_nt5_kernel(const h16* __restrict__ x, const h16* __restrict__ w, const float* __restrict__ bias,
                                                          h16* __restrict__ y, int B, int H, int W, long x_ld, long y_ld,
                                                          float* __restrict__ stat_part, int Cout_total) {
    using M_ = Mma<h16>;
    using Frag = M_::Frag;
    constexpr int VN = 8, CI = 64, CO = 64, TM = 4, TN = 4, NWV = 8, GW = 4;
    constexpr int TH = 16, TW = 16, HW_ = TW + 2, HROWS = (TH + 2) * HW_;
    constexpr int HINST = (HROWS + 7) / 8, HPW = (HINST + GW - 1) / GW;
    constexpr int HBYTES = HINST * 1024, TAPB = CO * 128, WBYTES = 9 * TAPB;
    constexpr int NST = TM * TN;

    __shared__ __attribute__((aligned(16))) char lds[2 * HBYTES + WBYTES + 1024];
    char* Ws = lds + 2 * HBYTES;
    char* dump = Ws + WBYTES;

    const int tiles_w = W / TW, tiles_h = H / TH;
    const int ntile = B * tiles_h * tiles_w, nblk = gridDim.x;
    const int bx = xcd_remap(blockIdx.x, gridDim.x);
    if (bx >= ntile) return;
    const int nt = (ntile - bx + nblk - 1) / nblk;

    const int tid = threadIdx.x, lane = tid & 63, wave = __builtin_amdgcn_readfirstlane(tid >> 6);
    const int grp = wave >> 2, wg = wave & 3;
    const int r16 = lane & 15, g = lane >> 4;
    const int srow = lane >> 3, sch = lane & 7;
    char* Hg = lds + grp * HBYTES;
    const int co_base = blockIdx.y * CO;

    auto stage_halo = [&](int tl) {
        const int tw_ = tl % tiles_w, th_ = (tl / tiles_w) % tiles_h, bi = tl / (tiles_w * tiles_h);
        const int hh0 = th_ * TH - 1, ww0 = tw_ * TW - 1;
        const h16* xb = x + (long)bi * H * W * x_ld;
#pragma unroll
        for (int k = 0; k < HPW; ++k) {
            const int inst = k * GW + wg;
            const int hr = inst * 8 + srow;
            const int hy = hr / HW_, hx = hr - hy * HW_;
            const int hh = hh0 + hy, ww = ww0 + hx;
            const bool ok = hr < HROWS && hh >= 0 && hh < H && ww >= 0 && ww < W;
            const void* src = ok ? (const void*)(xb + ((long)hh * W + ww) * x_ld + (sch ^ (hx & 7)) * VN) : (const void*)mu_zero_page;
            if (inst < HINST) glds16a(src, Hg + inst * 1024);
            else glds16a(mu_zero_page, dump);
        }
    };

    int aoff[2], boff[3][2];
#pragma unroll
    for (int kk = 0; kk < 2; ++kk) {
        aoff[kk] = r16 * 128 + (((kk * 4 + g) ^ (r16 & 7)) << 4);
#pragma unroll
        for (int dw = 0; dw < 3; ++dw) boff[dw][kk] = (wg * TN * HW_ + r16 + dw) * 128 + (((kk * 4 + g) ^ ((r16 + dw) & 7)) << 4);
    }
    float bv[TM][4];
#pragma unroll
    for (int i = 0; i < TM; ++i)
#pragma unroll
        for (int r = 0; r < 4; ++r) bv[i][r] = bias ? bias[co_base + i * 16 + 4 * g + r] : 0.f;

    {
        const int row = wave * 8 + srow;
#pragma unroll
        for (int t = 0; t < 9; ++t) glds16a(w + ((long)t * Cout_total + co_base + row) * CI + (sch ^ (row & 7)) * VN, Ws + t * TAPB + wave * 1024);
    }
    if (grp == 0) stage_halo(bx);
    asm volatile("s_waitcnt vmcnt(0)" ::: "memory");
    __builtin_amdgcn_sched_barrier(0);
    __builtin_amdgcn_s_barrier();
    __builtin_amdgcn_sched_barrier(0);

    f32x4 acc[TM][TN];
#pragma unroll
    for (int i = 0; i < TM; ++i)
#pragma unroll
        for (int j = 0; j < TN; ++j) acc[i][j] = (f32x4){0.f, 0.f, 0.f, 0.f};

    for (int p = 0; p <= nt; ++p) {
        if (grp == (p & 1)) {
            if (p < nt) {
#pragma unroll
                for (int i = 0; i < TM; ++i)
#pragma unroll
                    for (int j = 0; j < TN; ++j) acc[i][j] = (f32x4){0.f, 0.f, 0.f, 0.f};
                __builtin_amdgcn_s_setprio(1);
#pragma unroll
                for (int t = 0; t < 9; ++t) {
                    const int dh = t / 3, dw = t % 3;
                    const char* Wb = Ws + t * TAPB;
                    const char* Hb = Hg + dh * (HW_ * 128);
#pragma unroll
                    for (int kk = 0; kk < 2; ++kk) {
                        Frag a[TM], b[TN];
#pragma unroll
                        for (int i = 0; i < TM; ++i) a[i] = M_::ld(Wb + aoff[kk] + i * 2048);
#pragma unroll
                        for (int j = 0; j < TN; ++j) b[j] = M_::ld(Hb + boff[dw][kk] + j * (HW_ * 128));
#pragma unroll
                        for (int i = 0; i < TM; ++i)
#pragma unroll
                            for (int j = 0; j < TN; ++j) M_::mma(a[i], b[j], acc[i][j]);
                    }
                }
                __builtin_amdgcn_s_setprio(0);
            }
            asm volatile("s_waitcnt lgkmcnt(0)" ::: "memory");
        } else {
            const bool pf = p + 1 < nt, ep = p >= 1;
            if (pf) stage_halo(bx + (p + 1) * nblk);
            if (ep) {
                const int tl = bx + (p - 1) * nblk;
                const int tw_ = tl % tiles_w, th_ = (tl / tiles_w) % tiles_h, bimg = tl / (tiles_w * tiles_h);
                h16* yb = y + (((long)bimg * H + th_ * TH + wg * TN) * W + tw_ * TW + r16) * y_ld + co_base + 4 * g;
                float tsum[TM][4], tsq[TM][4];
#pragma unroll
                for (int i = 0; i < TM; ++i)
#pragma unroll
                    for (int r = 0; r < 4; ++r) { tsum[i][r] = 0.f; tsq[i][r] = 0.f; }
#pragma unroll
                for (int j = 0; j < TN; ++j)
#pragma unroll
                    for (int i = 0; i < TM; ++i) {
                        const h16x4 o = {(h16)(acc[i][j][0] + bv[i][0]), (h16)(acc[i][j][1] + bv[i][1]), (h16)(acc[i][j][2] + bv[i][2]),
                                         (h16)(acc[i][j][3] + bv[i][3])};
                        *reinterpret_cast<h16x4*>(yb + (long)j * W * y_ld + i * 16) = o;
#pragma unroll
                        for (int r = 0; r < 4; ++r) { const float v = (float)o[r]; tsum[i][r] += v; tsq[i][r] = fmaf(v, v, tsq[i][r]); }
                    }
                if (stat_part) {
                    float v8[2][4][2], v4[4][2], v2[2][2], v1[2];
                    const bool b3 = r16 & 8, b2 = r16 & 4, b1 = r16 & 2, b0 = r16 & 1;
#pragma unroll
                    for (int i = 0; i < 2; ++i)
#pragma unroll
                        for (int r = 0; r < 4; ++r) {
                            v8[i][r][0] = (b3 ? tsum[i + 2][r] : tsum[i][r]) + __shfl_xor(b3 ? tsum[i][r] : tsum[i + 2][r], 8);
                            v8[i][r][1] = (b3 ? tsq[i + 2][r] : tsq[i][r]) + __shfl_xor(b3 ? tsq[i][r] : tsq[i + 2][r], 8);
                        }
#pragma unroll
                    for (int r = 0; r < 4; ++r)
#pragma unroll
                        for (int k = 0; k < 2; ++k) v4[r][k] = (b2 ? v8[1][r][k] : v8[0][r][k]) + __shfl_xor(b2 ? v8[0][r][k] : v8[1][r][k], 4);
#pragma unroll
                    for (int r = 0; r < 2; ++r)
#pragma unroll
                        for (int k = 0; k < 2; ++k) v2[r][k] = (b1 ? v4[r + 2][k] : v4[r][k]) + __shfl_xor(b1 ? v4[r][k] : v4[r + 2][k], 2);
#pragma unroll
                    for (int k = 0; k < 2; ++k) v1[k] = (b0 ? v2[1][k] : v2[0][k]) + __shfl_xor(b0 ? v2[0][k] : v2[1][k], 1);
                    *reinterpret_cast<float2*>(stat_part + (((long)tl * GW + wg) * CO + (r16 >> 2) * 16 + 4 * g + (r16 & 3)) * 2) = make_float2(v1[0], v1[1]);
                }
            }
            if (!pf || !ep) asm volatile("s_waitcnt vmcnt(0)" ::: "memory");
            else if (stat_part) asm volatile("s_waitcnt vmcnt(%0)" ::"n"(NST + 1) : "memory");
// ... 114 lines not shown
    const int B = g.B, H = g.H, W = g.W, npb = g.pb128, t16 = (int)g.t16, t8 = (int)g.t8;
    switch (conv_fused_pick(g, Cin, Cout, TAPS, conv_dtype_of<T>)) {
    case FF_NONE:
        break;
    case FF_NT4F:
        if constexpr (sizeof(T) == 2 && TAPS == 9)
            conv_nt4f_kernel<<<t16 * (Cout / 128), 512, 0, st>>>(x, w, bias, y, B, H, W, Cin, Cout, x_ld, y_ld, scale, res, act);
        break;
    case FF_NT3F_128:
        if constexpr (TAPS == 9)
            conv_nt3f_kernel<T, 4, 4, 2><<<t8 * (Cout / 128), 256, 0, st>>>(x, w, bias, y, B, H, W, Cin, Cout, x_ld, y_ld, scale, res, act);
        break;
    case FF_NT3F_64:
        if constexpr (TAPS == 9)
            conv_nt3f_kernel<T, 4, 2, 1><<<t8 * (Cout / 64), 256, 0, st>>>(x, w, bias, y, B, H, W, Cin, Cout, x_ld, y_ld, scale, res, act);
        break;
    case FF_HEAD160:
        if constexpr (TAPS == 1 && sizeof(T) == 2)
            conv_nt2_kernel<T, 5, 4, 2, 1, false, true><<<npb, 256, 0, st>>>(x, w, bias, y, B, H, W, Cin, Cout, x_ld, y_ld, res, scale, act);
        break;
    case FF_DMA128:
        conv_nt2_kernel<T, 4, 4, 2, TAPS, false, true><<<npb * (Cout / 128), 256, 0, st>>>(x, w, bias, y, B, H, W, Cin, Cout, x_ld, y_ld, res, scale, act);
        break;
    case FF_DMA64:
        conv_nt2_kernel<T, 4, 4, 1, TAPS, false, true><<<g.pb256 * (Cout / 64), 256, 0, st>>>(x, w, bias, y, B, H, W, Cin, Cout, x_ld, y_ld, res, scale, act);
        break;
    case FF_GEN128:
        conv_nt_kernel<T, 4, 4, 2, TAPS, true><<<npb * (Cout / 128), 256, 0, st>>>(x, w, bias, y, B, H, W, Cin, Cout, x_ld, y_ld, scale, res, act);
        break;
    case FF_GEN64:
        conv_nt_kernel<T, 4, 2, 1, TAPS, true><<<npb * (Cout / 64), 256, 0, st>>>(x, w, bias, y, B, H, W, Cin, Cout, x_ld, y_ld, scale, res, act);
        break;
    case FF_GEN32:
        conv_nt_kernel<T, 2, 2, 1, TAPS, true><<<npb * (Cout / 32), 256, 0, st>>>(x, w, bias, y, B, H, W, Cin, Cout, x_ld, y_ld, scale, res, act);
        break;
    case FF_COUNT:
        break;
    }
}

template <typename T, int TAPS>
static void conv_fwd_launch(const T* x, const T* w, const float* bias, T* y, const ConvGeom& g, int Cin, int Cout, long x_ld, long y_ld,
                            hipStream_t st, float* stat_part = nullptr) {
    const int B = g.B, H = g.H, W = g.W, npb = g.pb128, t16 = (int)g.t16, t8 = (int)g.t8;
    switch (conv_fwd_pick(g, Cin, Cout, TAPS, conv_dtype_of<T>, stat_part != nullptr)) {
    case K3_NT5:
        if constexpr (sizeof(T) == 2 && TAPS == 9)
            conv_nt5_kernel<<<t16 < 256 ? t16 : 256, 512, 0, st>>>((const h16*)x, (const h16*)w, bias, (h16*)y, B, H, W, x_ld, y_ld, stat_part, 64);
        break;
    case K3_NT5_HALVES:
        if constexpr (sizeof(T) == 2 && TAPS == 9)
            conv_nt5_kernel<<<dim3(256, 2), 512, 0, st>>>((const h16*)x, (const h16*)w, bias, (h16*)y, B, H, W, x_ld, y_ld, nullptr, 128);
        break;
    case K3_NT4P:
        if constexpr (sizeof(T) == 2 && TAPS == 9) conv_nt4p_kernel<<<256, 512, 0, st>>>(x, w, bias, y, B, H, W, Cin, Cout, x_ld, y_ld, stat_part);
        break;
    case K3_NT4:
        if constexpr (sizeof(T) == 2 && TAPS == 9) conv_nt4_kernel<<<t16 * (Cout / 128), 512, 0, st>>>(x, w, bias, y, B, H, W, Cin, Cout, x_ld, y_ld, stat_part);
        break;
    case K3_NT4X:
        if constexpr (mu_is_split<T>::value && TAPS == 9)
            conv_nt4x_kernel<T><<<t16 * (Cout / 128), 512, 0, st>>>(x, w, bias, y, B, H, W, Cin, Cout, x_ld, y_ld, stat_part);
        break;
    case K3_NT3_128:
        if constexpr (TAPS == 9) conv_nt3_kernel<T, 4, 4, 2><<<t8 * (Cout / 128), 256, 0, st>>>(x, w, bias, y, B, H, W, Cin, Cout, x_ld, y_ld, stat_part);
        break;
    case K3_NT3_64_RING:
        if constexpr (TAPS == 9) conv_nt3_kernel<T, 4, 2, 1, true><<<t8 * (Cout / 64), 256, 0, st>>>(x, w, bias, y, B, H, W, Cin, Cout, x_ld, y_ld, stat_part);
        break;
    case K3_NT3_64:
        if constexpr (TAPS == 9) conv_nt3_kernel<T, 4, 2, 1><<<t8 * (Cout / 64), 256, 0, st>>>(x, w, bias, y, B, H, W, Cin, Cout, x_ld, y_ld, stat_part);
        break;
    case KF_WIDE192_SB:
        if constexpr (TAPS == 1 && sizeof(T) == 2) conv_nt2_kernel<T, 6, 4, 2, 1, true><<<npb * (Cout / 192), 256, 0, st>>>(x, w, bias, y, B, H, W, Cin, Cout, x_ld, y_ld);
        break;
    case KF_WIDE192:
        if constexpr (TAPS == 1 && sizeof(T) == 2) conv_nt2_kernel<T, 6, 4, 2, 1><<<npb * (Cout / 192), 256, 0, st>>>(x, w, bias, y, B, H, W, Cin, Cout, x_ld, y_ld);
        break;
    case KF_HEAD160_SB:
        if constexpr (TAPS == 1 && sizeof(T) == 2) conv_nt2_kernel<T, 5, 4, 2, 1, true><<<npb, 256, 0, st>>>(x, w, bias, y, B, H, W, Cin, Cout, x_ld, y_ld);
        break;
    case KF_HEAD160:
        if constexpr (TAPS == 1 && (sizeof(T) == 2 || mu_is_split<T>::value))
            conv_nt2_kernel<T, 5, 4, 2, 1><<<npb, 256, 0, st>>>(x, w, bias, y, B, H, W, Cin, Cout, x_ld, y_ld);
        break;
    case KF_DMA128:
        conv_nt2_kernel<T, 4, 4, 2, TAPS><<<npb * (Cout / 128), 256, 0, st>>>(x, w, bias, y, B, H, W, Cin, Cout, x_ld, y_ld);
        break;
    case KF_DMA64:
        conv_nt2_kernel<T, 4, 4, 1, TAPS><<<g.pb256 * (Cout / 64), 256, 0, st>>>(x, w, bias, y, B, H, W, Cin, Cout, x_ld, y_ld);
        break;
    case KF_GEN128:
        conv_nt_kernel<T, 4, 4, 2, TAPS><<<npb * (Cout / 128), 256, 0, st>>>(x, w, bias, y, B, H, W, Cin, Cout, x_ld, y_ld);
        break;
    case KF_GEN64:
        conv_nt_kernel<T, 4, 2, 1, TAPS><<<npb * (Cout / 64), 256, 0, st>>>(x, w, bias, y, B, H, W, Cin, Cout, x_ld, y_ld);
        break;
    case KF_GEN32:
        conv_nt_kernel<T, 2, 2, 1, TAPS><<<npb * (Cout / 32), 256, 0, st>>>(x, w, bias, y, B, H, W, Cin, Cout, x_ld, y_ld);
        break;
    }
}

extern "C" int mu_conv_stats_rows(int B, int H, int W, int Cin, int Cout, int taps, int dtype) {
    if (taps != 9 || B <= 0 || (dtype != MU_F16 && dtype != MU_F32X)) return 0;
    return conv3x3_pick(conv_geom(B, H, W), Cin, Cout, dtype, true).stat_rows;
}

static bool conv_plan_args_ok(int B, int H, int W, int Cin, int Cout, int taps, int dtype) {
    return B > 0 && H > 0 && W > 0 && Cin > 0 && Cout > 0 && Cin % 32 == 0 && Cout % 32 == 0 && (taps == 1 || taps == 9) &&
           (dtype == MU_F32 || dtype == MU_F16 || dtype == MU_F32X);
}

extern "C" int mu_conv_fwd_plan(int B, int H, int W, int Cin, int Cout, int taps, int dtype, int with_stats) {
    if (!conv_plan_args_ok(B, H, W, Cin, Cout, taps, dtype)) return 0;
    if (with_stats && mu_conv_stats_rows(B, H, W, Cin, Cout, taps, dtype) == 0) return 0;
    return conv_fwd_pick(conv_geom(B, H, W), Cin, Cout, taps, dtype, with_stats != 0);
}
extern "C" int mu_conv_fwd_fused_plan(int B, int H, int W, int Cin, int Cout, int taps, int dtype) {
    if (!conv_plan_args_ok(B, H, W, Cin, Cout, taps, dtype)) return 0;
    return conv_fused_pick(conv_geom(B, H, W), Cin, Cout, taps, dtype);
}

extern "C" int mu_conv_fwd_stats(const void* x, const void* w, const float* bias, void* y, int B, int H, int W, int Cin, int Cout,
                                 int taps, long x_ld, long y_ld, int dtype, float* stat_part, void* stream) {
    if (const int rc = conv_io_check(x && w && y && B > 0 && H > 0 && W > 0, Cin, Cout, x_ld, y_ld)) return rc;
    if (stat_part && mu_conv_stats_rows(B, H, W, Cin, Cout, taps, dtype) == 0) return MU_ERR_SHAPE;
    const int rc = with_conv_type(dtype, taps, [&](auto t, auto tc) -> int {
        using T = decltype(t);
        conv_fwd_launch<T, decltype(tc)::value>((const T*)x, (const T*)w, bias, (T*)y, conv_geom(B, H, W), Cin, Cout, x_ld, y_ld, (hipStream_t)stream, stat_part);
        return MU_OK;
    });
    if (rc) return rc;
    MU_CHECK_LAUNCH();
    return MU_OK;
}

extern "C" int mu_conv_fwd(const void* x, const void* w, const float* bias, void* y, int B, int H, int W, int Cin, int Cout, int taps,
                           long x_ld, long y_ld, int dtype, void* stream) {
    return mu_conv_fwd_stats(x, w, bias, y, B, H, W, Cin, Cout, taps, x_ld, y_ld, dtype, nullptr, stream);
}

extern "C" int mu_conv_fwd_fused(const void* x, const void* w, const float* scale, const float* bias, const void* res, int act, void* y, int B,
                                 int H, int W, int Cin, int Cout, int taps, long x_ld, long y_ld, int dtype, void* stream) {
    if (const int rc = conv_io_check(x && w && y && B > 0 && H > 0 && W > 0, Cin, Cout, x_ld, y_ld)) return rc;
    if (act < MU_ACT_NONE || act > MU_ACT_RELU) return MU_ERR_ARG;
    const int rc = with_conv_type(dtype, taps, [&](auto t, auto tc) -> int {
        using T = decltype(t);
        conv_fwd_fused_launch<T, decltype(tc)::value>((const T*)x, (const T*)w, scale, bias, (const T*)res, act, (T*)y, conv_geom(B, H, W), Cin, Cout, x_ld,
                                                      y_ld, (hipStream_t)stream);
        return MU_OK;
    });
    if (rc) return rc;
    MU_CHECK_LAUNCH();
    return MU_OK;
}

enum ConvDgradHKernel { DH_NONE, DH_NT4HL, DH_NT3HL_128, DH_NT3HL_64, DH_GEN128, DH_GEN64, DH_GEN32, DH_COUNT };
static ConvDgradHKernel conv_dgrad_h_pick(const ConvGeom& g, int Cin, int Cout) {
    if (Cin % 64 == 0 && g.W % 16 == 0 && g.H % 8 == 0 && Cout % 64 == 0) {
        if (Cout % 128 == 0 && g.H % 16 == 0) return DH_NT4HL;
        return Cout % 128 == 0 ? DH_NT3HL_128 : DH_NT3HL_64;
    }
    return Cout % 128 == 0 ? DH_GEN128 : Cout % 64 == 0 ? DH_GEN64 : DH_GEN32;
}
extern "C" int mu_conv_dgrad_h_plan(int B, int H, int W, int Cin, int Cout) {
    if (!conv_plan_args_ok(B, H, W, Cin, Cout, 9, MU_F32X)) return 0;
    return conv_dgrad_h_pick(conv_geom(B, H, W), Cin, Cout);
}
extern "C" int mu_conv_dgrad_h(const void* dy_h, const void* w_hl, const float* dy_scale, void* dx, int B, int H, int W, int Cin, int Cout,
                               long dy_ld, long dx_ld, void* stream) {
    if (const int rc = conv_io_check(dy_h && w_hl && dy_scale && dx && B > 0 && H > 0 && W > 0, Cin, Cout, dy_ld, dx_ld, 32, 4)) return rc;
    hipStream_t st = (hipStream_t)stream;
    const h16* x = (const h16*)dy_h;
    const h16* w = (const h16*)w_hl;
    float* y = (float*)dx;
    const ConvGeom g = conv_geom(B, H, W);
    const int npb = g.pb128, t16 = (int)g.t16, t8 = (int)g.t8;
    constexpr int HL = 2;
    switch (conv_dgrad_h_pick(g, Cin, Cout)) {
    case DH_NT4HL:
        conv_nt4hl_kernel<HL><<<t16 * (Cout / 128), 512, 0, st>>>(x, w, y, B, H, W, Cin, Cout, dy_ld, dx_ld, dy_scale);
        break;
    case DH_NT3HL_128:
        conv_nt3hl_kernel<4, 4, 2, false, HL><<<t8 * (Cout / 128), 256, 0, st>>>(x, w, y, B, H, W, Cin, Cout, dy_ld, dx_ld, dy_scale);
        break;
    case DH_NT3HL_64:
        conv_nt3hl_kernel<4, 2, 1, true, HL><<<t8 * (Cout / 64), 256, 0, st>>>(x, w, y, B, H, W, Cin, Cout, dy_ld, dx_ld, dy_scale);
        break;
    case DH_GEN128:
        conv_nt_kernel<h16, 4, 4, 2, 9, false, HL><<<npb * (Cout / 128), 256, 0, st>>>(x, w, nullptr, nullptr, B, H, W, Cin, Cout, dy_ld, dx_ld, nullptr, nullptr, 0, y, dy_scale);
        break;
    case DH_GEN64:
        conv_nt_kernel<h16, 4, 2, 1, 9, false, HL><<<npb * (Cout / 64), 256, 0, st>>>(x, w, nullptr, nullptr, B, H, W, Cin, Cout, dy_ld, dx_ld, nullptr, nullptr, 0, y, dy_scale);
        break;
    case DH_GEN32:
        conv_nt_kernel<h16, 2, 2, 1, 9, false, HL><<<npb * (Cout / 32), 256, 0, st>>>(x, w, nullptr, nullptr, B, H, W, Cin, Cout, dy_ld, dx_ld, nullptr, nullptr, 0, y, dy_scale);
        break;
    case DH_NONE: case DH_COUNT:
        break;
    }
    MU_CHECK_LAUNCH();
    return MU_OK;
}

extern "C" int mu_conv1x1_add_supported(int Cin, int Cout, int dtype) {
    const int es = dtype == MU_F16 ? 2 : 4;
    return (dtype == MU_F16 || dtype == MU_F32 || dtype == MU_F32X) && Cin > 0 && Cout > 0 && (Cin * es) % 128 == 0 && Cout % 64 == 0 ? 1 : 0;
}

template <typename T, bool FEPI, typename... Tail>
static void conv1x1_launch(const T* x, const T* w, const float* bias, T* y, long M, int Cin, int Cout, long x_ld, long y_ld, hipStream_t st,
                           Tail... tail) {
    const ConvGeom g = conv_geom_rows(M);
    if (Cout % 128 == 0)
        conv_nt2_kernel<T, 4, 4, 2, 1, false, FEPI><<<g.pb128 * (Cout / 128), 256, 0, st>>>(x, w, bias, y, 1, 1, (int)M, Cin, Cout, x_ld, y_ld, tail...);
    else
        conv_nt2_kernel<T, 4, 4, 1, 1, false, FEPI><<<g.pb256 * (Cout / 64), 256, 0, st>>>(x, w, bias, y, 1, 1, (int)M, Cin, Cout, x_ld, y_ld, tail...);
}

extern "C" int mu_conv1x1_fwd_enc_h(const void* x, const void* w, const float* bias, void* y, long M, int Cin, int Cout, long x_ld, long y_ld,
                                    void* stream) {
    if (const int rc = conv_io_check(x && w && y && M > 0 && M <= 0x7fffffffL, Cin, Cout, x_ld, y_ld, 64)) return rc;
    conv1x1_launch<xf32, false>((const xf32*)x, (const xf32*)w, bias, (xf32*)y, M, Cin, Cout, x_ld, y_ld, (hipStream_t)stream, (const xf32*)nullptr,
                                (const float*)nullptr, MU_NT2_ENC_H);
    MU_CHECK_LAUNCH();
    return MU_OK;
}

extern "C" int mu_conv1x1_fwd_add(const void* x, const void* w, const void* addend, void* y, long M, int Cin, int Cout, long x_ld, long y_ld,
                                  int dtype, void* stream) {
    if (const int rc = conv_io_check(x && w && addend && y && M > 0 && M <= 0x7fffffffL, Cin, Cout, x_ld, y_ld, 64)) return rc;
    if (!mu_conv1x1_add_supported(Cin, Cout, dtype)) return MU_ERR_SHAPE;
    const int rc = with_conv_storage<1>(dtype, [&](auto t) -> int {
        using T = decltype(t);
        conv1x1_launch<T, true>((const T*)x, (const T*)w, nullptr, (T*)y, M, Cin, Cout, x_ld, y_ld, (hipStream_t)stream, (const T*)addend);
        return MU_OK;
    });
    if (rc) return rc;
    MU_CHECK_LAUNCH();
    return MU_OK;
}

template <typename T> struct WgTile;
template <> struct WgTile<h16> { static constexpr int PAD = 0; static constexpr int KP = 32; };
template <> struct WgTile<float> { static constexpr int PAD = 16; static constexpr int KP = 16; };
template <> struct WgTile<xf32> { static constexpr int PAD = 16; static constexpr int KP = 32; };

typedef __fp16 fp16x4v __attribute__((__vector_size__(4 * sizeof(__fp16))));

template <typename T, int TM, int TN, int WR, int TAPS, bool BIAS = false>
__global__ __launch_bounds__(256) void conv_wgrad_kernel(const T* __restrict__ x, const T* __restrict__ dy, float* __restrict__ part,
                                                         int B, int H, int W, int Cin, int Cout, long x_ld, long dy_ld, int nsplit,
                                                         long pix_per_split, float* __restrict__ bias_part = nullptr) {
    constexpr int VN = Mma<T>::VN;
    constexpr int WC = 4 / WR;
    constexpr int BCO = WR * TM * 16, BCI = WC * TN * 16;
    constexpr int KP = WgTile<T>::KP;
    constexpr int SA = BCO + WgTile<T>::PAD, SB = BCI + WgTile<T>::PAD;
    constexpr int CA = BCO / VN, CB = BCI / VN;
    constexpr int NA = (KP * CA + 255) / 256, NB = (KP * CB + 255) / 256;

    __shared__ __attribute__((aligned(16))) T lds[2 * KP * (SA + SB)];
    T* As = lds;
    T* Bs = lds + 2 * KP * SA;

    const long Mtot = (long)B * H * W;
    const int nco = (Cout + BCO - 1) / BCO, nci = (Cin + BCI - 1) / BCI;
    int bid = blockIdx.x;
    const int split = bid % nsplit; bid /= nsplit;
    const int cib = bid % nci; bid /= nci;
    const int cob = bid % nco; bid /= nco;
    const int tap = bid;
    const int dh = TAPS == 9 ? tap / 3 - 1 : 0, dw = TAPS == 9 ? tap % 3 - 1 : 0;
    const int co0 = cob * BCO, ci0 = cib * BCI;
    const long p_begin = (long)split * pix_per_split;
    const long p_end = p_begin + pix_per_split < Mtot ? p_begin + pix_per_split : Mtot;

    const int tid = threadIdx.x, lane = tid & 63, wave = tid >> 6;
    const int wr = wave / WC, wc = wave % WC;
    const int r16 = lane & 15, g = lane >> 4;

    uint4 ra[NA], rb[NB];
    auto gload = [&](long pbase) {
#pragma unroll
        for (int i = 0; i < NA; ++i) {
            const int idx = tid + i * 256, row = idx / CA, c = (idx % CA) * VN;
            const long p = pbase + row;
            if (idx < KP * CA && p < p_end && co0 + c < Cout) ra[i] = *reinterpret_cast<const uint4*>(dy + p * dy_ld + co0 + c);
            else ra[i] = make_uint4(0, 0, 0, 0);
        }
#pragma unroll
        for (int i = 0; i < NB; ++i) {
            const int idx = tid + i * 256, row = idx / CB, c = (idx % CB) * VN;
            const long p = pbase + row;
            bool ok = idx < KP * CB && p < p_end && ci0 + c < Cin;
            if (ok && TAPS == 9) {
                const int ww = (int)(p % W) + dw, hh = (int)((p / W) % H) + dh;
                ok = hh >= 0 && hh < H && ww >= 0 && ww < W;
            }
            if (ok) rb[i] = *reinterpret_cast<const uint4*>(x + (p + dh * W + dw) * x_ld + ci0 + c);
            else rb[i] = make_uint4(0, 0, 0, 0);
        }
    };
    constexpr bool XSWAP = std::is_same<T, xf32>::value;
    auto put = [&](T* dst, int row, const uint4& v) {
// ... 1284 lines not shown
```

maskunet_amd/csrc/norm.hip:

```cpp
#include "common.h"
#include "../../include/maskunet_hip.h"

#define MU_STAT_MAXBLK 1024

template <typename T, int MODE, int ACT = -1, int RES = -1, bool MAXT = false>
__global__ __launch_bounds__(256, 1) void bn_partial_kernel(const T* __restrict__ x, const T* __restrict__ g, const T* __restrict__ res,
                                                         T* __restrict__ dzbuf, long M, int C, long ld,
                                                         const float* __restrict__ mean, const float* __restrict__ rstd,
                                                         const float* __restrict__ gamma, const float* __restrict__ beta, int act_arg,
                                                         double* __restrict__ part, float* __restrict__ pmax = nullptr) {
    constexpr int N = Vec16<T>::N;
    constexpr int U = MODE == 0 ? 8 : 2;
    constexpr bool FAST = sizeof(T) == 2;
    const int act = ACT >= 0 ? ACT : act_arg;
    const bool has_res = RES >= 0 ? (RES != 0) : (res != nullptr);
    extern __shared__ __attribute__((aligned(16))) double sh[];
    const int cv = C / N;
    const int rpi = 256 / cv;
    const int tc = threadIdx.x % cv, tr = threadIdx.x / cv;
    const long r0 = (long)blockIdx.x * (U * rpi), r1 = M;
    const long rstride = (long)gridDim.x * (U * rpi);
    double s0[N], s1[N];
    float mxg[N], mxx[N];
#pragma unroll
    for (int i = 0; i < N; ++i) { mxg[i] = 0.f; mxx[i] = 0.f; }
#pragma unroll
    for (int i = 0; i < N; ++i) { s0[i] = 0.0; s1[i] = 0.0; }
    if (tr < rpi) {
        const int c = tc * N;
        float mu[N], rs[N], ga[N], be[N];
        if (MODE == 1) {
#pragma unroll
            for (int i = 0; i < N; ++i) { mu[i] = mean[c + i]; rs[i] = rstd[c + i]; ga[i] = gamma[c + i]; be[i] = beta[c + i]; }
        }
        for (long r = r0 + tr; r < r1; r += rstride) {
            Vec16<T> xv[U], gv[U], rv[U];
#pragma unroll
            for (int u = 0; u < U; ++u) {
                const long rr = r + (long)u * rpi;
                if (rr < r1) {
                    xv[u].load(x + rr * ld + c);
                    if (MODE == 1) {
                        gv[u].load(g + rr * ld + c);
                        if (has_res) rv[u].load_nt(res + rr * ld + c);
                    }
                } else {
                    xv[u].zero();
                    if (MODE == 1) { gv[u].zero(); rv[u].zero(); }
                }
            }
            float f0[N], f1[N];
#pragma unroll
            for (int i = 0; i < N; ++i) { f0[i] = 0.f; f1[i] = 0.f; }
#pragma unroll
            for (int u = 0; u < U; ++u) {
                if (MODE == 0) {
#pragma unroll
                    for (int i = 0; i < N; ++i) {
                        const float v = xv[u].get(i);
                        f0[i] += v;
                        f1[i] = fmaf(v, v, f1[i]);
                    }
                } else {
                    const long rr = r + (long)u * rpi;
                    Vec16<T> dz;
#pragma unroll
                    for (int i = 0; i < N; i += 2) {
                        const mu_f32x2 xh = (mu_f32x2{xv[u].get(i), xv[u].get(i + 1)} - mu_f32x2{mu[i], mu[i + 1]}) * mu_f32x2{rs[i], rs[i + 1]};
                        mu_f32x2 pre = __builtin_elementwise_fma(xh, mu_f32x2{ga[i], ga[i + 1]}, mu_f32x2{be[i], be[i + 1]});
                        if (has_res) pre += mu_f32x2{rv[u].get(i), rv[u].get(i + 1)};
                        float ag[2];
                        mu_act_grad2_t<FAST>(pre[0], pre[1], act, ag[0], ag[1]);
                        const mu_f32x2 dzf = mu_f32x2{gv[u].get(i), gv[u].get(i + 1)} * mu_f32x2{ag[0], ag[1]};
                        dz.set(i, dzf[0]);
                        dz.set(i + 1, dzf[1]);
                        const mu_f32x2 d = {dz.get(i), dz.get(i + 1)};
                        if constexpr (MAXT) {
                            if (rr < r1) {
                                mxg[i] = fmaxf(mxg[i], fabsf(d[0])); mxg[i + 1] = fmaxf(mxg[i + 1], fabsf(d[1]));
                                mxx[i] = fmaxf(mxx[i], fabsf(xh[0])); mxx[i + 1] = fmaxf(mxx[i + 1], fabsf(xh[1]));
                            }
                        }
                        mu_f32x2 a0 = {f0[i], f0[i + 1]}, a1 = {f1[i], f1[i + 1]};
                        a0 += d;
                        a1 = __builtin_elementwise_fma(d, xh, a1);
                        f0[i] = a0[0]; f0[i + 1] = a0[1];
                        f1[i] = a1[0]; f1[i + 1] = a1[1];
                    }
                    if (dzbuf && rr < r1) dz.store(dzbuf + rr * ld + c);
                }
            }
#pragma unroll
            for (int i = 0; i < N; ++i) { s0[i] += (double)f0[i]; s1[i] += (double)f1[i]; }
        }
#pragma unroll
        for (int i = 0; i < N; ++i) {
            sh[((long)tr * C + c + i) * 2 + 0] = s0[i];
            sh[((long)tr * C + c + i) * 2 + 1] = s1[i];
        }
    }
    __syncthreads();
    for (int c = threadIdx.x; c < C; c += 256) {
        double a = 0.0, b = 0.0;
        for (int k = 0; k < rpi; ++k) { a += sh[((long)k * C + c) * 2]; b += sh[((long)k * C + c) * 2 + 1]; }
        part[((long)blockIdx.x * C + c) * 2] = a;
        part[((long)blockIdx.x * C + c) * 2 + 1] = b;
    }
    if constexpr (MAXT) {
        __syncthreads();
        float* shm = reinterpret_cast<float*>(sh);
        if (tr < rpi) {
#pragma unroll
            for (int i = 0; i < N; ++i) {
                shm[((long)tr * C + tc * N + i) * 2 + 0] = mxg[i];
                shm[((long)tr * C + tc * N + i) * 2 + 1] = mxx[i];
            }
        }
        __syncthreads();
        for (int c = threadIdx.x; c < C; c += 256) {
            float a = 0.f, b = 0.f;
            for (int k = 0; k < rpi; ++k) { a = fmaxf(a, shm[((long)k * C + c) * 2]); b = fmaxf(b, shm[((long)k * C + c) * 2 + 1]); }
            *reinterpret_cast<float2*>(pmax + ((long)blockIdx.x * C + c) * 2) = make_float2(a, b);
        }
    }
}

template <bool FROWS = false>
__global__ void bn_fwd_final_kernel(const void* __restrict__ part_, int nblk, int C, long M, float eps, float momentum,
                                    float* __restrict__ mean, float* __restrict__ rstd, float* __restrict__ running_mean,
                                    float* __restrict__ running_var, int c_valid, long* __restrict__ num_batches_tracked) {
    const double* part = reinterpret_cast<const double*>(part_);
    const float* fpart = reinterpret_cast<const float*>(part_);
    if (num_batches_tracked && blockIdx.x == 0 && threadIdx.x == 0) *num_batches_tracked += 1;
    const int c = blockIdx.x * (blockDim.x >> 6) + (threadIdx.x >> 6), lane = threadIdx.x & 63;
    if (c >= C) return;
    double sv[MU_STAT_MAXBLK / 64], qv[MU_STAT_MAXBLK / 64];
#pragma unroll
    for (int u = 0; u < MU_STAT_MAXBLK / 64; ++u) {
        const int b = lane + 64 * u;
        if constexpr (FROWS) {
            const float2 v = b < nblk ? *reinterpret_cast<const float2*>(fpart + ((long)b * C + c) * 2) : make_float2(0.f, 0.f);
            sv[u] = (double)v.x; qv[u] = (double)v.y;
        } else {
            const double2 v = b < nblk ? *reinterpret_cast<const double2*>(part + ((long)b * C + c) * 2) : make_double2(0.0, 0.0);
            sv[u] = v.x; qv[u] = v.y;
        }
    }
    double s = 0.0, q = 0.0;
#pragma unroll
    for (int u = 0; u < MU_STAT_MAXBLK / 64; ++u) { s += sv[u]; q += qv[u]; }
    s = wave_sum_d(s); q = wave_sum_d(q);
    if (lane) return;
    double m = s / (double)M;
    double var = q / (double)M - m * m;
    if (var < 0.0) var = 0.0;
    mean[c] = (float)m;
    rstd[c] = (float)(1.0 / sqrt(var + (double)eps));
    if (running_mean && c < c_valid) {
        double unb = M > 1 ? var * ((double)M / (double)(M - 1)) : var;
        running_mean[c] = (float)((1.0 - (double)momentum) * (double)running_mean[c] + (double)momentum * m);
        running_var[c] = (float)((1.0 - (double)momentum) * (double)running_var[c] + (double)momentum * unb);
    }
}

__global__ void bn_eval_stats_kernel(const float* __restrict__ running_mean, const float* __restrict__ running_var, float eps,
                                     float* __restrict__ mean, float* __restrict__ rstd, int C, int c_valid) {
    int c = blockIdx.x * blockDim.x + threadIdx.x;
    if (c >= C) return;
    if (c < c_valid) { mean[c] = running_mean[c]; rstd[c] = 1.0f / sqrtf(running_var[c] + eps); }
    else { mean[c] = 0.f; rstd[c] = 1.f; }
}

__global__ void bn_bwd_final_kernel(const double* __restrict__ part, int nblk, int C, long M, int training,
                                    float* __restrict__ dgamma, float* __restrict__ dbeta, float* __restrict__ s1, float* __restrict__ s2,
                                    const float* __restrict__ xscale = nullptr, const float* __restrict__ pc2 = nullptr,
                                    const float* __restrict__ pc1 = nullptr, float* __restrict__ pair_grads = nullptr,
                                    const float* __restrict__ pmax = nullptr, const float* __restrict__ gamma = nullptr,
                                    const float* __restrict__ rstd = nullptr, float* __restrict__ bound = nullptr) {
    const int c = blockIdx.x * (blockDim.x >> 6) + (threadIdx.x >> 6), lane = threadIdx.x & 63;
    if (c >= C) return;
    double av[MU_STAT_MAXBLK / 64], bv[MU_STAT_MAXBLK / 64];
#pragma unroll
    for (int u = 0; u < MU_STAT_MAXBLK / 64; ++u) {
        const int k = lane + 64 * u;
        const double2 v = k < nblk ? *reinterpret_cast<const double2*>(part + ((long)k * C + c) * 2) : make_double2(0.0, 0.0);
        av[u] = v.x; bv[u] = v.y;
    }
    float2 pv[MU_STAT_MAXBLK / 64];
    if (bound) {
#pragma unroll
        for (int u = 0; u < MU_STAT_MAXBLK / 64; ++u) {
            const int k = lane + 64 * u;
            pv[u] = k < nblk ? *reinterpret_cast<const float2*>(pmax + ((long)k * C + c) * 2) : make_float2(0.f, 0.f);
        }
    }
    double a = 0.0, b = 0.0;
#pragma unroll
    for (int u = 0; u < MU_STAT_MAXBLK / 64; ++u) { a += av[u]; b += bv[u]; }
    a = wave_sum_d(a); b = wave_sum_d(b);
    float mg = 0.f, mx = 0.f;
    if (bound) {
#pragma unroll
        for (int u = 0; u < MU_STAT_MAXBLK / 64; ++u) { mg = fmaxf(mg, pv[u].x); mx = fmaxf(mx, pv[u].y); }
        mg = wave_max(mg); mx = wave_max(mx);
    }
    if (lane) return;
    dbeta[c] = (float)a;
    dgamma[c] = (float)b;
    if (pair_grads) {
        pair_grads[c] = pc2[c] * (float)b;
        pair_grads[C + c] = pc1[c] * (float)b;
        pair_grads[2 * C + c] = 0.f;
    }
    const float s1c = training ? (float)(a / (double)M) : 0.f;
    const float s2c = training ? (float)((xscale ? (double)xscale[c] : 1.0) * b / (double)M) : 0.f;
    s1[c] = s1c;
    s2[c] = s2c;
    if (bound) bound[c] = fabsf(gamma[c] * rstd[c]) * (mg + fabsf(s1c) + mx * fabsf(s2c));
}

template <typename T, bool ENC = false, int ACT = -1, int RES = -1>
__global__ __launch_bounds__(256) void bn_act_fwd_kernel(const T* __restrict__ x, const T* __restrict__ res, T* __restrict__ y, long M,
                                                         int C, long ld, const float* __restrict__ mean, const float* __restrict__ rstd,
                                                         const float* __restrict__ gamma, const float* __restrict__ beta, int act_arg,
                                                         h16* __restrict__ y16 = nullptr) {
    constexpr int N = Vec16<T>::N;
    constexpr int U = 2;
    constexpr bool FAST = sizeof(T) == 2;
    const int act = ACT >= 0 ? ACT : act_arg;
    const bool has_res = RES >= 0 ? (RES != 0) : (res != nullptr);
    const int cv = C / N;
    const long total = M * cv;
    const long stride = (long)gridDim.x * 256;
    const long first = (long)blockIdx.x * 256 + threadIdx.x;
    const int c = (int)(first % cv) * N;
    const long rstep = stride / cv;
    float a[N], b[N];
#pragma unroll
    for (int i = 0; i < N; ++i) {
        a[i] = rstd[c + i] * gamma[c + i];
        b[i] = beta[c + i] - mean[c + i] * a[i];
    }
    for (long idx = first; idx < total; idx += U * stride) {
        const long r = idx / cv;
        Vec16<T> xv[U], rv[U];
#pragma unroll
        for (int u = 0; u < U; ++u) {
            if (idx + u * stride < total) {
                xv[u].load_nt(x + (r + u * rstep) * ld + c);
                if (has_res) rv[u].load_nt(res + (r + u * rstep) * ld + c);
            }
        }
#pragma unroll
        for (int u = 0; u < U; ++u) {
            if (idx + u * stride < total) {
                Vec16<T> o;
#pragma unroll
                for (int i = 0; i < N; i += 2) {
                    mu_f32x2 pp = __builtin_elementwise_fma(mu_f32x2{xv[u].get(i), xv[u].get(i + 1)}, mu_f32x2{a[i], a[i + 1]}, mu_f32x2{b[i], b[i + 1]});
                    if (has_res) pp += mu_f32x2{rv[u].get(i), rv[u].get(i + 1)};
                    float o0, o1;
                    mu_act2_t<FAST>(pp[0], pp[1], act, o0, o1);
                    o.set(i, o0);
                    o.set(i + 1, o1);
                }
                if constexpr (ENC) {
                    float o0 = o.get(0), o1 = o.get(1), o2 = o.get(2), o3 = o.get(3);
                    asm("" : "+v"(o0), "+v"(o1), "+v"(o2), "+v"(o3));
                    const uint4 e4 = mu_ench4((f32x4){o0, o1, o2, o3});
                    *reinterpret_cast<uint4*>(y + (r + u * rstep) * ld + c) = e4;
                    if (y16) *reinterpret_cast<uint2*>(y16 + (r + u * rstep) * (long)C + c) = make_uint2(e4.x, e4.y);
                } else {
                    o.store(y + (r + u * rstep) * ld + c);
                }
            }
        }
    }
}

template <typename T, bool RECOMP, bool ENC = false, int ACT = -1>
__global__ __launch_bounds__(256) void bn_bwd_apply_kernel(const T* __restrict__ x, const T* dzbuf, T* dx, long M, int C, long ld,
                                                           const float* __restrict__ mean, const float* __restrict__ rstd,
                                                           const float* __restrict__ gamma, const float* __restrict__ beta, int act_arg,
                                                           const float* __restrict__ s1, const float* __restrict__ s2,
                                                           const float* __restrict__ bound = nullptr, float* __restrict__ dy_scale = nullptr) {
    constexpr int N = Vec16<T>::N;
    constexpr int U = 2;
    constexpr bool FAST = sizeof(T) == 2;
    const int act = ACT >= 0 ? ACT : act_arg;
    const int cv = C / N;
    const long total = M * cv;
    const long stride = (long)gridDim.x * 256;
    const long first = (long)blockIdx.x * 256 + threadIdx.x;
    const int c = (int)(first % cv) * N;
    const long rstep = stride / cv;
    float gr[N], k0[N], k1[N], mu[N], rsv[N], ga[N], be[N];
#pragma unroll
    for (int i = 0; i < N; ++i) {
        const float rs = rstd[c + i];
        gr[i] = gamma[c + i] * rs;
        k1[i] = -gr[i] * rs * s2[c + i];
        k0[i] = -gr[i] * s1[c + i] - k1[i] * mean[c + i];
        mu[i] = mean[c + i]; rsv[i] = rs; ga[i] = gamma[c + i]; be[i] = RECOMP ? beta[c + i] : 0.f;
    }
    float S = 1.f;
    if constexpr (ENC) {
        float bm = 0.f;
        for (int k = threadIdx.x & 63; k < C; k += 64) bm = fmaxf(bm, bound[k]);
        bm = wave_max(bm);
        const int e = (int)((__float_as_uint(bm) >> 23) & 0xff) - 127;
        if (bm > 0.f && e > -127 && e < 128) {
            int k = 13 - e;
            k = k < -100 ? -100 : (k > 100 ? 100 : k);
            S = __uint_as_float((uint32_t)(127 + k) << 23);
        }
        if (blockIdx.x == 0 && threadIdx.x == 0) { dy_scale[0] = S; dy_scale[1] = 1.0f / S; }
    }
    for (long idx = first; idx < total; idx += U * stride) {
        const long r = idx / cv;
        Vec16<T> xv[U], dz[U];
#pragma unroll
        for (int u = 0; u < U; ++u) {
            if (idx + u * stride < total) {
                xv[u].load_nt(x + (r + u * rstep) * ld + c);
                dz[u].load_nt(dzbuf + (r + u * rstep) * ld + c);
            }
        }
#pragma unroll
        for (int u = 0; u < U; ++u) {
            if (idx + u * stride < total) {
                Vec16<T> o;
#pragma unroll
                for (int i = 0; i < N; i += 2) {
                    const mu_f32x2 xf = {xv[u].get(i), xv[u].get(i + 1)};
                    mu_f32x2 d = {dz[u].get(i), dz[u].get(i + 1)};
                    if (RECOMP) {
                        Vec16<T> t;
                        const mu_f32x2 xh = (xf - mu_f32x2{mu[i], mu[i + 1]}) * mu_f32x2{rsv[i], rsv[i + 1]};
                        const mu_f32x2 pre = __builtin_elementwise_fma(xh, mu_f32x2{ga[i], ga[i + 1]}, mu_f32x2{be[i], be[i + 1]});
// ... 144 lines not shown
    return with_storage(dtype, [&](auto tag) -> int {
        using T = decltype(tag);
        StatGeom sg;
        if (int e = stat_geom(C, Vec16<T>::N, sg)) return e;
        bn_partial_kernel<T, 0><<<nblk, 256, sg.lds, st>>>((const T*)x, nullptr, nullptr, nullptr, M, C, ld, nullptr, nullptr, nullptr, nullptr, 0, part);
        bn_fwd_final_kernel<false><<<mu_cdiv(C, 4), 256, 0, st>>>(part, nblk, C, M, eps, momentum, mean, rstd, running_mean, running_var, c_valid,
                                                            num_batches_tracked);
        MU_CHECK_LAUNCH();
        return MU_OK;
    });
}

__global__ __launch_bounds__(256) void bn_fold_rows_kernel(const float* __restrict__ part, int rows, int rpb, int C2, double* __restrict__ out) {
    const int r0 = blockIdx.x * rpb, r1 = r0 + rpb < rows ? r0 + rpb : rows;
    for (int c = threadIdx.x; c < C2; c += 256) {
        double a[8] = {0.0, 0.0, 0.0, 0.0, 0.0, 0.0, 0.0, 0.0};
        int r = r0;
        for (; r + 7 < r1; r += 8) {
#pragma unroll
            for (int u = 0; u < 8; ++u) a[u] += (double)part[(long)(r + u) * C2 + c];
        }
        for (; r < r1; ++r) a[0] += (double)part[(long)r * C2 + c];
        out[(long)blockIdx.x * C2 + c] = ((a[0] + a[1]) + (a[2] + a[3])) + ((a[4] + a[5]) + (a[6] + a[7]));
    }
}

extern "C" int mu_bn_train_stats_rows(const float* stat_part, int rows, long M, int C, float* mean, float* rstd, float* running_mean,
                                      float* running_var, long* num_batches_tracked, int c_valid, float momentum, float eps,
                                      void* workspace, long ws_bytes, void* stream) {
    if (!stat_part || !mean || !rstd || !workspace || rows <= 0 || M <= 0 || C <= 0) return MU_ERR_ARG;
    int rpb = 16;
    if ((rows + rpb - 1) / rpb > MU_STAT_MAXBLK) rpb = ((rows + MU_STAT_MAXBLK - 1) / MU_STAT_MAXBLK + 7) / 8 * 8;
    const int nblk = (rows + rpb - 1) / rpb;
    if (ws_bytes < mu_bn_workspace_bytes(C)) return MU_ERR_WORKSPACE;
    hipStream_t st = (hipStream_t)stream;
    if (rows <= MU_STAT_MAXBLK) {
        bn_fwd_final_kernel<true><<<mu_cdiv(C, 4), 256, 0, st>>>(stat_part, rows, C, M, eps, momentum, mean, rstd, running_mean, running_var,
                                                                 c_valid, num_batches_tracked);
        MU_CHECK_LAUNCH();
        return MU_OK;
    }
    bn_fold_rows_kernel<<<nblk, 256, 0, st>>>(stat_part, rows, rpb, 2 * C, (double*)workspace);
    bn_fwd_final_kernel<false><<<mu_cdiv(C, 4), 256, 0, st>>>((const double*)workspace, nblk, C, M, eps, momentum, mean, rstd, running_mean,
                                                        running_var, c_valid, num_batches_tracked);
    MU_CHECK_LAUNCH();
    return MU_OK;
}

extern "C" int mu_bn_eval_stats(const float* running_mean, const float* running_var, float eps, float* mean, float* rstd, int C,
                                int c_valid, void* stream) {
    if (!running_mean || !running_var || !mean || !rstd || C <= 0) return MU_ERR_ARG;
    bn_eval_stats_kernel<<<mu_cdiv(C, 64), 64, 0, (hipStream_t)stream>>>(running_mean, running_var, eps, mean, rstd, C, c_valid);
    MU_CHECK_LAUNCH();
    return MU_OK;
}

__global__ void bn_eval_fold_kernel(const float* __restrict__ rm1, const float* __restrict__ rv1, const float* __restrict__ g1,
                                    const float* __restrict__ b1, float eps1, const float* __restrict__ rm2, const float* __restrict__ rv2,
                                    const float* __restrict__ g2, const float* __restrict__ b2, float eps2, const float* __restrict__ conv_bias,
                                    float* __restrict__ scale, float* __restrict__ shift, int C, int c_valid) {
    const int c = blockIdx.x * blockDim.x + threadIdx.x;
    if (c >= C) return;
    if (c >= c_valid) { scale[c] = 0.f; shift[c] = 0.f; return; }
    float a = (g1 ? g1[c] : 1.f) / sqrtf(rv1[c] + eps1);
    float sh = (b1 ? b1[c] : 0.f) + ((conv_bias ? conv_bias[c] : 0.f) - rm1[c]) * a;
    if (rm2) {
        const float a2 = (g2 ? g2[c] : 1.f) / sqrtf(rv2[c] + eps2);
        sh = (sh - rm2[c]) * a2 + (b2 ? b2[c] : 0.f);
        a *= a2;
    }
    scale[c] = a;
    shift[c] = sh;
}

extern "C" int mu_bn_eval_fold(const float* running_mean1, const float* running_var1, const float* gamma1, const float* beta1, float eps1,
                               const float* running_mean2, const float* running_var2, const float* gamma2, const float* beta2, float eps2,
                               const float* conv_bias, float* scale, float* shift, int C, int c_valid, void* stream) {
    if (!running_mean1 || !running_var1 || !scale || !shift || C <= 0 || c_valid <= 0 || c_valid > C) return MU_ERR_ARG;
    if ((running_mean2 != nullptr) != (running_var2 != nullptr)) return MU_ERR_ARG;
    bn_eval_fold_kernel<<<mu_cdiv(C, 64), 64, 0, (hipStream_t)stream>>>(running_mean1, running_var1, gamma1, beta1, eps1, running_mean2, running_var2,
                                                                       gamma2, beta2, eps2, conv_bias, scale, shift, C, c_valid);
    MU_CHECK_LAUNCH();
    return MU_OK;
}

#define MU_BN_ACT_SWITCH(act, CALL)                              \
    switch (act) {                                               \
        case MU_ACT_GELU: { constexpr int A_ = MU_ACT_GELU; CALL; } break; \
        case MU_ACT_RELU: { constexpr int A_ = MU_ACT_RELU; CALL; } break; \
        default:          { constexpr int A_ = MU_ACT_NONE; CALL; } break; \
    }
template <typename T, bool ENC>
static int bn_act_fwd_launch(const T* x, const T* res, T* y, long M, int C, long ld, const float* mean, const float* rstd,
                             const float* gamma, const float* beta, int act, hipStream_t st, h16* y16 = nullptr) {
    constexpr int N = Vec16<T>::N;
    const int grid = ew_grid(M * (C / N), C / N);
    if (res) { MU_BN_ACT_SWITCH(act, (bn_act_fwd_kernel<T, ENC, A_, 1><<<grid, 256, 0, st>>>(x, res, y, M, C, ld, mean, rstd, gamma, beta, act, y16))) }
    else     { MU_BN_ACT_SWITCH(act, (bn_act_fwd_kernel<T, ENC, A_, 0><<<grid, 256, 0, st>>>(x, res, y, M, C, ld, mean, rstd, gamma, beta, act, y16))) }
    MU_CHECK_LAUNCH();
    return MU_OK;
}

extern "C" int mu_bn_act_fwd_enc(const void* x, const void* res, void* y_enc, void* y16, long M, int C, const float* mean, const float* rstd,
                                 const float* gamma, const float* beta, int act, void* stream) {
    if (!x || !y_enc || !y16 || !mean || !rstd || !gamma || !beta || M <= 0 || C <= 0 || C % 8) return MU_ERR_ARG;
    if (act != MU_ACT_NONE && act != MU_ACT_GELU && act != MU_ACT_RELU) return MU_ERR_ARG;
    return bn_act_fwd_launch<float, true>((const float*)x, (const float*)res, (float*)y_enc, M, C, C, mean, rstd, gamma, beta, act, (hipStream_t)stream, (h16*)y16);
}

extern "C" int mu_bn_act_fwd(const void* x, const void* res, void* y, long M, int C, long ld, const float* mean, const float* rstd,
                             const float* gamma, const float* beta, int act, int dtype, void* stream) {
    if (!x || !y || !mean || !rstd || !gamma || !beta || M <= 0 || C <= 0 || C % 8 || ld < C) return MU_ERR_ARG;
    hipStream_t st = (hipStream_t)stream;
    if (act != MU_ACT_NONE && act != MU_ACT_GELU && act != MU_ACT_RELU) return MU_ERR_ARG;
    if (dtype == MU_F32X)
        return bn_act_fwd_launch<float, true>((const float*)x, (const float*)res, (float*)y, M, C, ld, mean, rstd, gamma, beta, act, st);
    return with_storage(dtype, [&](auto tag) -> int {
        using T = decltype(tag);
        return bn_act_fwd_launch<T, false>((const T*)x, (const T*)res, (T*)y, M, C, ld, mean, rstd, gamma, beta, act, st);
    });
}

template <typename T>
struct BnBwd {
    const T *x, *res, *g;
    T *dx, *dres;
    long M; int C; long ld;
    const float *mean, *rstd, *gamma, *beta;
    int act, training;
    float *dgamma, *dbeta;
    const float* xscale = nullptr;
    const float *pc2 = nullptr, *pc1 = nullptr;
    float* pair_grads = nullptr;
    float* dy_scale = nullptr;
};

template <typename T, bool ENC>
static int bn_bwd_launch(const BnBwd<T>& a, const BnWs& ws, hipStream_t st) {
    static_assert(!ENC || sizeof(T) == 4, "fp16 dx rows come from fp32 storage");
    StatGeom sg;
    if (int e = stat_geom(a.C, Vec16<T>::N, sg)) return e;
    if (a.act != MU_ACT_NONE && a.act != MU_ACT_GELU && a.act != MU_ACT_RELU) return MU_ERR_ARG;
    if (ENC && (!a.dy_scale || a.ld != a.C)) return MU_ERR_ARG;
    int nblk = stat_blocks(a.M);
    if (nblk > 768) nblk = 768;
    const int agrid = ew_grid(a.M * sg.cv, sg.cv);
    float* pmax = ENC ? ws.pmax : nullptr;
    float* bound = ENC ? ws.bound : nullptr;
    if (a.res) {
        MU_BN_ACT_SWITCH(a.act, (bn_partial_kernel<T, 1, A_, 1, ENC><<<nblk, 256, sg.lds, st>>>(a.x, a.g, a.res, a.dres, a.M, a.C, a.ld, a.mean, a.rstd, a.gamma, a.beta, a.act, ws.part, pmax)))
    } else {
        MU_BN_ACT_SWITCH(a.act, (bn_partial_kernel<T, 1, A_, 0, ENC><<<nblk, 256, sg.lds, st>>>(a.x, a.g, nullptr, nullptr, a.M, a.C, a.ld, a.mean, a.rstd, a.gamma, a.beta, a.act, ws.part, pmax)))
    }
    bn_bwd_final_kernel<<<mu_cdiv(a.C, 4), 256, 0, st>>>(ws.part, nblk, a.C, a.M, a.training, a.dgamma, a.dbeta, ws.s1, ws.s2, a.xscale, a.pc2, a.pc1, a.pair_grads,
                                                         pmax, ENC ? a.gamma : nullptr, ENC ? a.rstd : nullptr, bound);
    if (a.res) bn_bwd_apply_kernel<T, false, ENC><<<agrid, 256, 0, st>>>(a.x, a.dres, a.dx, a.M, a.C, a.ld, a.mean, a.rstd, a.gamma, a.beta, a.act, ws.s1, ws.s2, bound, a.dy_scale);
    else { MU_BN_ACT_SWITCH(a.act, (bn_bwd_apply_kernel<T, true, ENC, A_><<<agrid, 256, 0, st>>>(a.x, a.g, a.dx, a.M, a.C, a.ld, a.mean, a.rstd, a.gamma, a.beta, a.act, ws.s1, ws.s2, bound, a.dy_scale))) }
    MU_CHECK_LAUNCH();
    return MU_OK;
}

extern "C" int mu_bn_act_bwd_scaled(const void* x, const void* res, const void* grad_out, void* dx, void* dres, long M, int C, long ld,
                                    const float* mean, const float* rstd, const float* gamma, const float* beta, int act, int training,
                                    float* dgamma, float* dbeta, const float* xhat_scale, void* workspace, long ws_bytes, int dtype,
                                    void* stream) {
    if (!x || !grad_out || !dx || !mean || !rstd || !gamma || !beta || !dgamma || !dbeta || !workspace) return MU_ERR_ARG;
    if ((res != nullptr) != (dres != nullptr)) return MU_ERR_ARG;
    if (M <= 0 || C <= 0 || C % 8 || ld < C) return MU_ERR_ARG;
    if (ws_bytes < BnWs::bytes(C)) return MU_ERR_WORKSPACE;
    return with_storage(dtype, [&](auto tag) -> int {
        using T = decltype(tag);
        BnBwd<T> a{(const T*)x, (const T*)res, (const T*)grad_out, (T*)dx, (T*)dres, M, C, ld, mean, rstd, gamma, beta, act, training, dgamma, dbeta};
        a.xscale = xhat_scale;
        return bn_bwd_launch<T, false>(a, BnWs(workspace, C), (hipStream_t)stream);
    });
}

extern "C" int mu_bn_act_bwd(const void* x, const void* res, const void* grad_out, void* dx, void* dres, long M, int C, long ld,
                             const float* mean, const float* rstd, const float* gamma, const float* beta, int act, int training,
                             float* dgamma, float* dbeta, void* workspace, long ws_bytes, int dtype, void* stream) {
    return mu_bn_act_bwd_scaled(x, res, grad_out, dx, dres, M, C, ld, mean, rstd, gamma, beta, act, training, dgamma, dbeta, nullptr,
                                workspace, ws_bytes, dtype, stream);
}

__global__ void bn_pair_compose_kernel(const float* __restrict__ rstd1, const float* __restrict__ gamma1, const float* __restrict__ beta1,
                                       const float* __restrict__ gamma2, int C, int c_valid, long M, float eps1, float eps2, float momentum2,
                                       float* __restrict__ running_mean2, float* __restrict__ running_var2, long* __restrict__ nbt2,
                                       float* __restrict__ gamma_eff, float* __restrict__ xhat_scale, float* __restrict__ dgamma2_coef,
                                       float* __restrict__ dgamma1_coef) {
    const int c = blockIdx.x * blockDim.x + threadIdx.x;
    if (nbt2 && c == 0) *nbt2 += 1;
    if (c >= C) return;
    const double r1 = (double)rstd1[c], g1 = (double)gamma1[c], g2 = (double)gamma2[c];
    double q = 1.0 - (double)eps1 * r1 * r1;
    if (q < 0.0) q = 0.0;
    const double var2 = g1 * g1 * q;
    const double r2 = 1.0 / sqrt(var2 + (double)eps2);
    gamma_eff[c] = (float)(g1 * g2 * r2);
    xhat_scale[c] = (float)(r2 * r2 * (g1 * g1 + (double)eps2));
    dgamma2_coef[c] = (float)(g1 * r2);
    dgamma1_coef[c] = (float)(g2 * r2 * r2 * r2 * (double)eps2);
    if (running_mean2 && c < c_valid) {
        const double unb = M > 1 ? var2 * ((double)M / (double)(M - 1)) : var2;
        running_mean2[c] = (float)((1.0 - (double)momentum2) * (double)running_mean2[c] + (double)momentum2 * (double)beta1[c]);
        running_var2[c] = (float)((1.0 - (double)momentum2) * (double)running_var2[c] + (double)momentum2 * unb);
    }
}

extern "C" int mu_bn_pair_compose(const float* rstd1, const float* gamma1, const float* beta1, const float* gamma2, int C, int c_valid,
                                  long M, float eps1, float eps2, float momentum2, float* running_mean2, float* running_var2,
                                  long* num_batches_tracked2, float* gamma_eff, float* xhat_scale, float* dgamma2_coef,
                                  float* dgamma1_coef, void* stream) {
    if (!rstd1 || !gamma1 || !beta1 || !gamma2 || !gamma_eff || !xhat_scale || !dgamma2_coef || !dgamma1_coef || C <= 0 || M <= 0)
        return MU_ERR_ARG;
    if ((running_mean2 != nullptr) != (running_var2 != nullptr)) return MU_ERR_ARG;
    bn_pair_compose_kernel<<<mu_cdiv(C, 64), 64, 0, (hipStream_t)stream>>>(rstd1, gamma1, beta1, gamma2, C, c_valid, M, eps1, eps2, momentum2,
                                                                          running_mean2, running_var2, num_batches_tracked2, gamma_eff,
                                                                          xhat_scale, dgamma2_coef, dgamma1_coef);
    MU_CHECK_LAUNCH();
    return MU_OK;
}

extern "C" int mu_bn_pair_bwd(const void* x, const void* grad_out, void* dx, long M, int C, long ld, const float* mean, const float* rstd,
                              const float* gamma_eff, const float* beta2, const float* xhat_scale, const float* dgamma2_coef,
                              const float* dgamma1_coef, float* pair_grads, float* dbeta2, void* workspace, long ws_bytes, int dtype,
                              void* stream) {
    if (!x || !grad_out || !dx || !mean || !rstd || !gamma_eff || !beta2 || !xhat_scale || !dgamma2_coef || !dgamma1_coef || !pair_grads ||
        !dbeta2 || !workspace)
        return MU_ERR_ARG;
    if (M <= 0 || C <= 0 || C % 8 || ld < C) return MU_ERR_ARG;
    if (ws_bytes < BnWs::bytes(C)) return MU_ERR_WORKSPACE;
    const BnWs ws(workspace, C);
    return with_storage(dtype, [&](auto tag) -> int {
        using T = decltype(tag);
        BnBwd<T> a{(const T*)x, nullptr, (const T*)grad_out, (T*)dx, nullptr, M, C, ld, mean, rstd, gamma_eff, beta2, MU_ACT_NONE, 1, ws.A, dbeta2};
        a.xscale = xhat_scale; a.pc2 = dgamma2_coef; a.pc1 = dgamma1_coef; a.pair_grads = pair_grads;
        return bn_bwd_launch<T, false>(a, ws, (hipStream_t)stream);
    });
}

extern "C" int mu_bn_act_bwd_h(const void* x, const void* res, const void* grad_out, void* dx_h, void* dres, long M, int C,
                               const float* mean, const float* rstd, const float* gamma, const float* beta, int act, int training,
                               float* dgamma, float* dbeta, float* dy_scale, void* workspace, long ws_bytes, void* stream) {
    if (!x || !grad_out || !dx_h || !mean || !rstd || !gamma || !beta || !dgamma || !dbeta || !dy_scale || !workspace) return MU_ERR_ARG;
    if ((res != nullptr) != (dres != nullptr)) return MU_ERR_ARG;
    if (M <= 0 || C <= 0 || C % 8) return MU_ERR_ARG;
    if (ws_bytes < BnWs::bytes(C)) return MU_ERR_WORKSPACE;
    BnBwd<float> a{(const float*)x, (const float*)res, (const float*)grad_out, (float*)dx_h, (float*)dres, M, C, C, mean, rstd, gamma, beta, act, training, dgamma, dbeta};
    a.dy_scale = dy_scale;
    return bn_bwd_launch<float, true>(a, BnWs(workspace, C), (hipStream_t)stream);
}

extern "C" int mu_bn_pair_bwd_h(const void* x, const void* grad_out, void* dx_h, long M, int C, const float* mean, const float* rstd,
                                const float* gamma_eff, const float* beta2, const float* xhat_scale, const float* dgamma2_coef,
                                const float* dgamma1_coef, float* pair_grads, float* dbeta2, float* dy_scale, void* workspace, long ws_bytes,
                                void* stream) {
    if (!x || !grad_out || !dx_h || !mean || !rstd || !gamma_eff || !beta2 || !xhat_scale || !dgamma2_coef || !dgamma1_coef || !pair_grads ||
        !dbeta2 || !dy_scale || !workspace)
        return MU_ERR_ARG;
    if (M <= 0 || C <= 0 || C % 8) return MU_ERR_ARG;
    if (ws_bytes < BnWs::bytes(C)) return MU_ERR_WORKSPACE;
    const BnWs ws(workspace, C);
    BnBwd<float> a{(const float*)x, nullptr, (const float*)grad_out, (float*)dx_h, nullptr, M, C, C, mean, rstd, gamma_eff, beta2, MU_ACT_NONE, 1, ws.A, dbeta2};
    a.xscale = xhat_scale; a.pc2 = dgamma2_coef; a.pc1 = dgamma1_coef; a.pair_grads = pair_grads; a.dy_scale = dy_scale;
    return bn_bwd_launch<float, true>(a, ws, (hipStream_t)stream);
}

#define LN_CHUNKS 128

template <typename T, int MODE>
__global__ __launch_bounds__(256) void lns_partial_kernel(const T* __restrict__ x, const T* __restrict__ dy, const float* __restrict__ w,
                                                          const float* __restrict__ mean, const float* __restrict__ rstd, long L,
                                                          double* __restrict__ part) {
    constexpr int N = Vec16<T>::N;
    const int b = blockIdx.y;
    const long nvec = L / N;
    const long per = (nvec + gridDim.x - 1) / gridDim.x;
    const long v0 = (long)blockIdx.x * per, v1 = (v0 + per < nvec ? v0 + per : nvec);
    const T* xb = x + (long)b * L;
    double s0 = 0.0, s1 = 0.0;
    float mu = 0.f, rs = 0.f;
    if (MODE == 1) { mu = mean[b]; rs = rstd[b]; }
    for (long v = v0 + threadIdx.x; v < v1; v += 256) {
        Vec16<T> xv;
        xv.load(xb + v * N);
        if (MODE == 0) {
#pragma unroll
            for (int i = 0; i < N; ++i) { double t = (double)xv.get(i); s0 += t; s1 += t * t; }
        } else {
            Vec16<T> gv;
            gv.load(dy + (long)b * L + v * N);
#pragma unroll
            for (int i = 0; i < N; ++i) {
                float gw = gv.get(i) * w[v * N + i];
                float xh = (xv.get(i) - mu) * rs;
                s0 += (double)gw;
                s1 += (double)gw * (double)xh;
            }
        }
    }
    s0 = wave_sum_d(s0);
    s1 = wave_sum_d(s1);
    __shared__ double sh[8];
    const int wid = threadIdx.x >> 6, lane = threadIdx.x & 63;
    if (lane == 0) { sh[wid * 2] = s0; sh[wid * 2 + 1] = s1; }
    __syncthreads();
    if (threadIdx.x == 0) {
        double a = sh[0] + sh[2] + sh[4] + sh[6], c = sh[1] + sh[3] + sh[5] + sh[7];
        part[((long)b * gridDim.x + blockIdx.x) * 2] = a;
        part[((long)b * gridDim.x + blockIdx.x) * 2 + 1] = c;
    }
}

__global__ void lns_final_kernel(const double* __restrict__ part, int nchunk, long L, float eps, int mode, float* __restrict__ o0,
                                 float* __restrict__ o1, int B) {
    const int b = blockIdx.x * (blockDim.x >> 6) + (threadIdx.x >> 6), lane = threadIdx.x & 63;
    if (b >= B) return;
    double a = 0.0, c = 0.0;
    for (int k = lane; k < nchunk; k += 64) { a += part[((long)b * nchunk + k) * 2]; c += part[((long)b * nchunk + k) * 2 + 1]; }
    a = wave_sum_d(a); c = wave_sum_d(c);
    if (lane) return;
    if (mode == 0) {
        double m = a / (double)L, var = c / (double)L - m * m;
        if (var < 0.0) var = 0.0;
        o0[b] = (float)m;
        o1[b] = (float)(1.0 / sqrt(var + (double)eps));
    } else {
        o0[b] = (float)(a / (double)L);
        o1[b] = (float)(c / (double)L);
    }
}

template <typename T>
__global__ __launch_bounds__(256) void lns_fwd_apply_kernel(const T* __restrict__ x, const float* __restrict__ w, const float* __restrict__ bias,
                                                            const float* __restrict__ mean, const float* __restrict__ rstd, T* __restrict__ y,
// ... 94 lines not shown
```

maskunet_amd/ops.py:

```python
from __future__ import annotations

import math
import os
from types import SimpleNamespace
from typing import NamedTuple

import torch
import torch.nn.functional as F
from torch.autograd.function import once_differentiable

from . import _lib
from ._lib import ACT_GELU, ACT_NONE, ACT_RELU, call, dt, mdt, ptr, stream, workspace


def pad32(c: int) -> int:
    return (c + 31) // 32 * 32


def _pad_vec(v, n, fill):
    v = v.detach().float()
    if v.numel() == n:
        return v.contiguous()
    return F.pad(v, (0, n - v.numel()), value=fill)

# ... 484 lines not shown
    C = x.shape[-1]
    M = x.numel() // C
    cv, rm, rv = bn.weight.numel(), bn.running_mean, bn.running_var
    ws = workspace(_lib.load().mu_bn_workspace_bytes(C), x.device)
    if stats is not None and stats.numel() > 0:
        call("mu_bn_train_stats_rows", ptr(stats), stats.shape[0], M, C, ptr(mean), ptr(rstd), ptr(rm), ptr(rv), ptr(nbt), cv,
             float(momentum), float(bn.eps), ptr(ws), ws.numel(), stream())
    else:
        call("mu_bn_train_stats", ptr(x), M, C, C, ptr(mean), ptr(rstd), ptr(rm), ptr(rv), ptr(nbt), cv, float(momentum), float(bn.eps),
             ptr(ws), ws.numel(), dt(x), stream())


def _bn_act_fwd(x, res, bn, act, stats=None, enc=False):
    x = x.contiguous()
    training = bn.training or bn.running_mean is None
    nbt = bn.num_batches_tracked if (bn.training and bn.num_batches_tracked is not None) else None
    if nbt is not None and (nbt.device != x.device or nbt.dtype != torch.int64):
        nbt.add_(1)
        nbt = None
    momentum = 0.1 if bn.momentum is None else bn.momentum
    C = x.shape[-1]
    M = x.numel() // C
    cv = bn.weight.numel()
    g_p, b_p = _pad_vec(bn.weight, C, 1.0), _pad_vec(bn.bias, C, 0.0)
    mean = torch.empty(C, dtype=torch.float32, device=x.device)
    rstd = torch.empty_like(mean)
    if training:
        _bn_train_stats(x, stats, bn, nbt, momentum, mean, rstd)
    else:
        call("mu_bn_eval_stats", ptr(bn.running_mean), ptr(bn.running_var), float(bn.eps), ptr(mean), ptr(rstd), C, cv, stream())
    y = torch.empty_like(x)
    if res is not None:
        res = res.contiguous()
    if enc:
        y16 = torch.empty(x.shape, dtype=torch.float16, device=x.device)
        call("mu_bn_act_fwd_enc", ptr(x), ptr(res), ptr(y), ptr(y16), M, C, ptr(mean), ptr(rstd), ptr(g_p), ptr(b_p), act, stream())
        y = _Enc3(y, y16)
    else:
        call("mu_bn_act_fwd", ptr(x), ptr(res), ptr(y), M, C, C, ptr(mean), ptr(rstd), ptr(g_p), ptr(b_p), act, dt(x), stream())
    return y, ((x, res, mean, rstd, g_p, b_p), (act, bool(training), cv))


def _dx_out(x, dx_h):
    if not dx_h:
        return torch.empty_like(x)
    return _DyH(torch.empty(x.shape, dtype=torch.float16, device=x.device), torch.empty(2, dtype=torch.float32, device=x.device))


def _bn_act_bwd(saved, gy, dx_h=False):
    (x, res, mean, rstd, g_p, b_p), (act, training, cv) = saved
    gy = gy.contiguous()
    C = x.shape[-1]
    M = x.numel() // C
    dres = torch.empty_like(x) if res is not None else None
    dgamma = torch.empty(C, dtype=torch.float32, device=x.device)
    dbeta = torch.empty_like(dgamma)
    ws = workspace(_lib.load().mu_bn_workspace_bytes(C), x.device)
    dx = _dx_out(x, dx_h)
    if dx_h:
        call("mu_bn_act_bwd_h", ptr(x), ptr(res), ptr(gy), ptr(dx.h), ptr(dres), M, C, ptr(mean), ptr(rstd), ptr(g_p), ptr(b_p),
             act, int(training), ptr(dgamma), ptr(dbeta), ptr(dx.scale), ptr(ws), ws.numel(), stream())
    else:
        call("mu_bn_act_bwd", ptr(x), ptr(res), ptr(gy), ptr(dx), ptr(dres), M, C, C, ptr(mean), ptr(rstd), ptr(g_p), ptr(b_p),
             act, int(training), ptr(dgamma), ptr(dbeta), ptr(ws), ws.numel(), dt(x), stream())
    return dx, dres, dgamma[:cv], dbeta[:cv]


class _BNAct(torch.autograd.Function):

    @staticmethod
    def forward(ctx, x, res, gamma, beta, bn, act, stats=None):
        y, (tensors, ctx.m) = _bn_act_fwd(x, res, bn, act, stats)
        ctx.save_for_backward(*tensors)
        return y

    @staticmethod
    @once_differentiable
    def backward(ctx, gy):
        return _bn_act_bwd((ctx.saved_tensors, ctx.m), gy) + (None, None, None)


BN_PAIR = os.environ.get("MU_BN_PAIR", "1") != "0"


def _bn_pair_ok(bn1, bn2, x):
    both_train = (bn1.training and bn2.training and bn1.running_mean is not None and bn2.running_mean is not None
                  and bn1.weight is not None and bn2.weight is not None)
    ok = both_train and BN_PAIR and all(t is not None and t.device == x.device and t.dtype == torch.int64
                                        for t in (bn1.num_batches_tracked, bn2.num_batches_tracked))
    return ok and bn1.momentum is not None and bn2.momentum is not None


def _bn_pair_fwd(x, bn1, bn2, stats=None):
    x = x.contiguous()
    C = x.shape[-1]
    M = x.numel() // C
    cv = bn1.weight.numel()
    g1p, b1p, g2p, b2p = _pad_vec(bn1.weight, C, 1.0), _pad_vec(bn1.bias, C, 0.0), _pad_vec(bn2.weight, C, 1.0), _pad_vec(bn2.bias, C, 0.0)
    dev = x.device
    mean = torch.empty(C, dtype=torch.float32, device=dev)
    rstd = torch.empty_like(mean)
    coef = torch.empty(4, C, dtype=torch.float32, device=dev)
    _bn_train_stats(x, stats, bn1, bn1.num_batches_tracked, bn1.momentum, mean, rstd)
    call("mu_bn_pair_compose", ptr(rstd), ptr(g1p), ptr(b1p), ptr(g2p), C, cv, M, float(bn1.eps), float(bn2.eps), float(bn2.momentum),
         ptr(bn2.running_mean), ptr(bn2.running_var), ptr(bn2.num_batches_tracked), ptr(coef[0]), ptr(coef[1]), ptr(coef[2]), ptr(coef[3]),
         stream())
    y = torch.empty_like(x)
    call("mu_bn_act_fwd", ptr(x), None, ptr(y), M, C, C, ptr(mean), ptr(rstd), ptr(coef[0]), ptr(b2p), ACT_NONE, dt(x), stream())
    return y, ((x, mean, rstd, coef, b2p), cv)


def _bn_pair_bwd(saved, gy, dx_h=False):
    (x, mean, rstd, coef, b2p), cv = saved
    gy = gy.contiguous()
    C = x.shape[-1]
    M = x.numel() // C
    dg = torch.empty(3, C, dtype=torch.float32, device=x.device)
    dbeta2 = torch.empty(C, dtype=torch.float32, device=x.device)
    ws = workspace(_lib.load().mu_bn_workspace_bytes(C), x.device)
    dx = _dx_out(x, dx_h)
    if dx_h:
        call("mu_bn_pair_bwd_h", ptr(x), ptr(gy), ptr(dx.h), M, C, ptr(mean), ptr(rstd), ptr(coef[0]), ptr(b2p), ptr(coef[1]), ptr(coef[2]),
             ptr(coef[3]), ptr(dg), ptr(dbeta2), ptr(dx.scale), ptr(ws), ws.numel(), stream())
    else:
        call("mu_bn_pair_bwd", ptr(x), ptr(gy), ptr(dx), M, C, C, ptr(mean), ptr(rstd), ptr(coef[0]), ptr(b2p), ptr(coef[1]), ptr(coef[2]),
             ptr(coef[3]), ptr(dg), ptr(dbeta2), ptr(ws), ws.numel(), dt(x), stream())
    return dx, dg[1, :cv], dg[2, :cv], dg[0, :cv], dbeta2[:cv]


class _BNPair(torch.autograd.Function):

    @staticmethod
    def forward(ctx, x, g1, b1, g2, b2, bn1, bn2, stats=None):
        y, (tensors, ctx.cv) = _bn_pair_fwd(x, bn1, bn2, stats)
        ctx.save_for_backward(*tensors)
        return y

    @staticmethod
    @once_differentiable
    def backward(ctx, gy):
        return _bn_pair_bwd((ctx.saved_tensors, ctx.cv), gy) + (None, None, None)


def bn_pair(x, bn1, bn2, stats=None):
    if not _bn_pair_ok(bn1, bn2, x):
        return bn_act(bn_act(x, bn1, ACT_NONE, stats=stats), bn2, ACT_NONE)
    return _BNPair.apply(x, bn1.weight, bn1.bias, bn2.weight, bn2.bias, bn1, bn2, stats)


def bn_act(x, bn, act=ACT_NONE, res=None, stats=None):
    return _BNAct.apply(x, res, bn.weight, bn.bias, bn, act, stats)


_keep_graph = getattr(torch._C._autograd, "_get_current_graph_task_keep_graph", lambda: True)


class _ConvBlocks(torch.autograd.Function):

    @staticmethod
    def forward(ctx, cfg, x, *params):
        blocks, tail_bn, res_link, grad_on, cache_ok = cfg
        x = x.contiguous()
        need = ctx.needs_input_grad[2:]

        def req(k):
            return (grad_on or k == 0) and any(ctx.needs_input_grad[:2 + k])

        enc_on = grad_on and _is_x(x)

        def into(w):
            return enc_on and w.shape[1] > 3

        units, plan, cur, fold = [], [], x, False
        for i, (w1, bn1, w2, bn2, residual) in enumerate(blocks):
            k = 6 * i
            nxt = blocks[i + 1] if i + 1 < len(blocks) else None
            n1, n2 = (req(k), need[k], False), (req(k + 3), need[k + 3], False)
            res = cur if residual else None
            (y, st), c1 = _conv_fwd(cur, w1, None, bn1.training, cache_ok, n1)
            y, b1 = _bn_act_fwd(y, None, bn1, ACT_GELU, st, enc=into(w2))
            (y, st), c2 = _conv_fwd(y, w2, None, bn2.training, cache_ok, n2)
            fold = nxt is None and tail_bn is not None and not residual and _bn_pair_ok(bn2, tail_bn, y)
            if fold:
                cur, b2 = _bn_pair_fwd(y, bn2, tail_bn, st)
            else:
                cur, b2 = _bn_act_fwd(y, res, bn2, ACT_GELU if residual else ACT_NONE, st,
                                      enc=nxt is not None and not nxt[4] and into(nxt[0]))
            if grad_on:
                units += [c1, b1, c2, b2]
                plan.append((residual, n1, into(w1), n2, into(w2)))
        if tail_bn is not None and not fold:
            cur, t = _bn_act_fwd(cur, None, tail_bn, ACT_NONE)
            units.append(t)
        ctx.save_for_backward(x if any(t is x for s in units[:4] for t in s[0]) else None, *params)
        ctx.units, ctx.plan, ctx.fold, ctx.tail = units, plan, fold, tail_bn is not None and not fold
        ctx.link = res_link if (res_link is not None and res_link.armed and blocks[0][4]) else None
        ctx.is_x = _is_x(x)
        return cur

    @staticmethod
    @once_differentiable
    def backward(ctx, gy):
        ctx.saved_tensors
        _same_mode(ctx.is_x, gy)
        units = list(ctx.units)
        if not _keep_graph():
            ctx.units = None
        grads = [None] * (len(ctx.needs_input_grad) - 2)
        if ctx.tail:
            gy, _, grads[-2], grads[-1] = _bn_act_bwd(units.pop(), gy)
        for i in reversed(range(len(ctx.plan))):
            residual, n1, h1, n2, h2 = ctx.plan[i]
            k, dres = 6 * i, None
            if ctx.fold and i == len(ctx.plan) - 1:
                gy, grads[k + 4], grads[k + 5], grads[-2], grads[-1] = _bn_pair_bwd(units.pop(), gy, h2)
            else:
                gy, dres, grads[k + 4], grads[k + 5] = _bn_act_bwd(units.pop(), gy, h2)
            if dres is not None and i == 0 and ctx.link is not None:
                ctx.link.put(dres)
                dres = None
            gy, grads[k + 3], _ = _conv_bwd(units.pop(), gy, n2)
            if gy is None:
                break
            gy, _, grads[k + 1], grads[k + 2] = _bn_act_bwd(units.pop(), gy, h1)
            gy, grads[k], _ = _conv_bwd(units.pop(), gy, n1)
            if gy is None:
                break
            if dres is not None:
                gy = gy + dres
        return (None, gy, *grads)


def conv_blocks(x, blocks, tail_bn=None, res_link=None):
    params = [p for w1, bn1, w2, bn2, _ in blocks for p in (w1, bn1.weight, bn1.bias, w2, bn2.weight, bn2.bias)]
    if tail_bn is not None:
        params += [tail_bn.weight, tail_bn.bias]
    return _ConvBlocks.apply((blocks, tail_bn, res_link, torch.is_grad_enabled(), _cache_ok()), x, *params)


EVAL_FUSE = os.environ.get("MU_EVAL_FUSE", "1") != "0"


def eval_fusable(*bns):
    if not EVAL_FUSE or torch.is_grad_enabled():
        return False
    return all(bn is None or (not bn.training and bn.running_mean is not None and bn.running_var is not None) for bn in bns)


def conv_bn_act_eval(x, weight, conv_bias, bn, act=ACT_NONE, res=None, bn2=None):
    x = x.contiguous()
    B, H, W, Cin_p = x.shape
    O, I = weight.shape[0], weight.shape[1]
    taps = weight.shape[2] * weight.shape[3]
    Cout_p = pad32(O)
    if pad32(I) != Cin_p:
        raise RuntimeError(f"conv: input has {Cin_p} (padded) channels, weight expects {I}")
    wprep = _prep_weight(weight, x.dtype, Cout_p, Cin_p, 0, True)
    fold = torch.empty((2, Cout_p), dtype=torch.float32, device=x.device)
    f = lambda t: None if t is None else t.detach().float().contiguous()
    b2 = bn2 if bn2 is not None else None
    call("mu_bn_eval_fold", ptr(f(bn.running_mean)), ptr(f(bn.running_var)), ptr(f(bn.weight)), ptr(f(bn.bias)), float(bn.eps),
         ptr(f(b2.running_mean)) if b2 is not None else None, ptr(f(b2.running_var)) if b2 is not None else None,
         ptr(f(b2.weight)) if b2 is not None else None, ptr(f(b2.bias)) if b2 is not None else None, float(b2.eps) if b2 is not None else 0.0,
         ptr(f(conv_bias)), ptr(fold[0]), ptr(fold[1]), Cout_p, O, stream())
    y = torch.empty((B, H, W, Cout_p), dtype=x.dtype, device=x.device)
    if res is not None:
        res = res.contiguous()
    call("mu_conv_fwd_fused", ptr(_enc_for(x, taps)), ptr(wprep), ptr(fold[0]), ptr(fold[1]), ptr(res), act, ptr(y), B, H, W, Cin_p, Cout_p, taps, Cin_p,
         Cout_p, mdt(x), stream())
    return y


class _MaxPool2(torch.autograd.Function):

    @staticmethod
    def forward(ctx, x, res_link=None, skip_link=None):
        x = x.contiguous()
        B, H, W, C = x.shape
        y = torch.empty((B, H // 2, W // 2, C), dtype=x.dtype, device=x.device)
        call("mu_maxpool2_fwd", ptr(x), ptr(y), B, H, W, C, dt(x), stream())
        ctx.save_for_backward(x)
        ctx.res_link, ctx.skip_link = res_link, skip_link
        if ctx.needs_input_grad[0]:
            if res_link is not None:
                res_link.armed = True
            if skip_link is not None:
                skip_link.armed = True
        return y

    @staticmethod
    @once_differentiable
    def backward(ctx, gy):
        (x,) = ctx.saved_tensors
        gy = gy.contiguous()
        B, H, W, C = x.shape
        dx = torch.empty_like(x)
        g2 = ctx.res_link.take() if ctx.res_link is not None else None
        ga = ctx.skip_link.take() if ctx.skip_link is not None else None
        if g2 is None and ga is None:
            call("mu_maxpool2_bwd", ptr(x), ptr(gy), ptr(dx), B, H, W, C, dt(x), stream())
        else:
            call("mu_maxpool2_bwd_acc", ptr(x), ptr(gy), ptr(g2), ptr(ga), ptr(dx), B, H, W, C, dt(x), stream())
        return dx, None, None


def maxpool2(x, res_link=None, skip_link=None):
    return _MaxPool2.apply(x, res_link, skip_link)


class _UpCat(torch.autograd.Function):

    @staticmethod
    def forward(ctx, x, skip, cx, cs, res_link=None, skip_link=None):
        x, skip = x.contiguous(), skip.contiguous()
        B, h, w, Cx = x.shape
        Cs = skip.shape[-1]
        if skip.shape[:3] != (B, 2 * h, 2 * w):
            raise RuntimeError(f"upsample/concat: skip {tuple(skip.shape)} does not match 2x of {tuple(x.shape)}")
        ctx.compact = (cx != Cx or cs != Cs)
        Ct = pad32(cx + cs) if ctx.compact else Cs + Cx
        y = torch.empty((B, 2 * h, 2 * w, Ct), dtype=x.dtype, device=x.device)
        if ctx.compact:
            call("mu_upcat_compact_fwd", ptr(x), ptr(skip), ptr(y), B, h, w, Cx, cx, Cs, cs, Ct, dt(x), stream())
        else:
            call("mu_upcat_fwd", ptr(x), ptr(skip), ptr(y), B, h, w, Cx, Cs, dt(x), stream())
        ctx.dims = (B, h, w, Cx, Cs, cx, cs, Ct)
        ctx.res_link = res_link if not ctx.compact else None
        if ctx.res_link is not None and (ctx.needs_input_grad[0] or ctx.needs_input_grad[1]):
            ctx.res_link.armed = True
        ctx.skip_link = skip_link if (skip_link is not None and skip_link.armed and ctx.needs_input_grad[1]) else None
        return y

    @staticmethod
    @once_differentiable
    def backward(ctx, gy):
        B, h, w, Cx, Cs, cx, cs, Ct = ctx.dims
        gy = gy.contiguous()
        dx = torch.empty((B, h, w, Cx), dtype=gy.dtype, device=gy.device)
        dskip = torch.empty((B, 2 * h, 2 * w, Cs), dtype=gy.dtype, device=gy.device)
        g2 = ctx.res_link.take() if ctx.res_link is not None else None
        if ctx.compact:
            call("mu_upcat_compact_bwd", ptr(gy), ptr(dx), ptr(dskip), B, h, w, Cx, cx, Cs, cs, Ct, dt(gy), stream())
        elif g2 is not None:
            call("mu_upcat_bwd_acc", ptr(gy), ptr(g2), ptr(dx), ptr(dskip), B, h, w, Cx, Cs, dt(gy), stream())
        else:
            call("mu_upcat_bwd", ptr(gy), ptr(dx), ptr(dskip), B, h, w, Cx, Cs, dt(gy), stream())
        if ctx.skip_link is not None:
            ctx.skip_link.put(dskip)
            dskip = None
        return dx, dskip, None, None, None, None


def upcat(x, skip, cx=None, cs=None, res_link=None, skip_link=None):
    return _UpCat.apply(x, skip, x.shape[-1] if cx is None else int(cx), skip.shape[-1] if cs is None else int(cs), res_link, skip_link)


SEED_STEP = None


class _Dropout(torch.autograd.Function):

    @staticmethod
    def forward(ctx, x, p, seed, mask):
        x = x.contiguous()
        y = torch.empty_like(x)
        if mask is not None:
            mask = mask.to(device=x.device, dtype=torch.uint8).contiguous()
        step = SEED_STEP
        call("mu_dropout_step", ptr(x), ptr(y), x.numel(), float(p), int(seed), ptr(step), ptr(mask), None, dt(x), stream())
        ctx.p, ctx.seed, ctx.step = p, seed, step
        ctx.save_for_backward(mask)
        return y

    @staticmethod
    @once_differentiable
    def backward(ctx, gy):
        (mask,) = ctx.saved_tensors
        gy = gy.contiguous()
# ... 312 lines not shown
```

Baseline: 2303 images/sec.

## Fuse conv dgrad with BN-activation backward epilogue and partial stats

Adds conv kernel variants whose epilogue computes the BN/activation backward product (dz = dy * act'(bn(x)+res)) and per-tile partial sums of dz and dz*xhat, so the conv data-gradient output feeds BN backward directly. A new rows-based BN backward then reduces these partials and applies the final dx, skipping the separate BN partial-reduction pass over dy and x. The conv-block backward loop is restructured to use this path when the shape qualifies, falling back otherwise. It adds register pressure and extra loads of x and res in the conv epilogue.

```diff
diff --git a/include/maskunet_hip.h b/include/maskunet_hip.h
--- a/include/maskunet_hip.h
+++ b/include/maskunet_hip.h
@@ -52,6 +52,10 @@
 int mu_conv_stats_rows(int B, int H, int W, int Cin, int Cout, int taps, int dtype);
 int mu_conv_fwd_stats(const void* x, const void* w, const float* bias, void* y, int B, int H, int W, int Cin, int Cout, int taps,
                       long x_ld, long y_ld, int dtype, float* stat_part, void* stream);
+int mu_conv_bnbwd_rows(int B, int H, int W, int Cin, int Cout, int taps, int dtype);
+int mu_conv_fwd_bnbwd(const void* x, const void* w, void* dz, int B, int H, int W, int Cin, int Cout, int taps, long x_ld, long y_ld,
+                      const void* bn_x, const void* bn_res, const float* mean, const float* rstd, const float* gamma, const float* beta,
+                      int act, int dtype, float* stat_part, void* stream);
 int mu_conv_fwd_plan(int B, int H, int W, int Cin, int Cout, int taps, int dtype, int with_stats);
 int mu_conv_fwd_fused_plan(int B, int H, int W, int Cin, int Cout, int taps, int dtype);
 int mu_conv_dgrad_h_plan(int B, int H, int W, int Cin, int Cout);
@@ -94,6 +98,9 @@
 int mu_bn_act_bwd(const void* x, const void* res, const void* grad_out, void* dx, void* dres, long M, int C, long ld,
                   const float* mean, const float* rstd, const float* gamma, const float* beta, int act, int training, float* dgamma,
                   float* dbeta, void* workspace, long ws_bytes, int dtype, void* stream);
+int mu_bn_bwd_rows(const void* bn_x, const void* dz, void* dx, long M, int C, long ld, const float* stat_part, int rows, const float* mean,
+                   const float* rstd, const float* gamma, const float* beta, float* dgamma, float* dbeta, void* workspace, long ws_bytes,
+                   int dtype, void* stream);
 int mu_bn_pair_compose(const float* rstd1, const float* gamma1, const float* beta1, const float* gamma2, int C, int c_valid, long M,
                        float eps1, float eps2, float momentum2, float* running_mean2, float* running_var2,
                        long* num_batches_tracked2, float* gamma_eff, float* xhat_scale, float* dgamma2_coef, float* dgamma1_coef,
diff --git a/maskunet_amd/_lib.py b/maskunet_amd/_lib.py
--- a/maskunet_amd/_lib.py
+++ b/maskunet_amd/_lib.py
@@ -45,6 +45,9 @@
     "mu_conv_plan_count": (I, [I]),
     "mu_conv_plan_name": (c_char_p, [I, I]),
     "mu_conv_fwd_stats": (I, [P, P, P, P, I, I, I, I, I, I, L, L, I, P, P]),
+    "mu_conv_bnbwd_rows": (I, [I, I, I, I, I, I, I]),
+    "mu_conv_fwd_bnbwd": (I, [P, P, P, I, I, I, I, I, I, L, L, P, P, P, P, P, P, I, I, P, P]),
+    "mu_bn_bwd_rows": (I, [P, P, P, L, I, L, P, I, P, P, P, P, P, P, P, L, I, P]),
     "mu_conv_wgrad_workspace_bytes": (L, [I, I, I, I, I, I]),
     "mu_conv_wgrad": (I, [P, P, P, I, I, I, I, I, I, I, I, L, L, P, L, I, P]),
     "mu_conv_wgrad_bias_supported": (I, [I, I, I, I]),
diff --git a/maskunet_amd/csrc/conv.hip b/maskunet_amd/csrc/conv.hip
--- a/maskunet_amd/csrc/conv.hip
+++ b/maskunet_amd/csrc/conv.hip
@@ -533,12 +533,57 @@
     }
 }
 
-template <typename T, int TM, int TN, int WR, bool RINGP, bool FEPI, int HL = 0>
+#define MU_NO_BEPI (-2)
+struct ConvBnBwd {
+    const h16* x;
+    const h16* res;
+    const float *mean, *rstd, *gamma, *beta;
+    int act;
+};
+struct BepiLane {
+    float mu[8], rs[8], ga[8], be[8], s0[8], s1[8];
+    __device__ __forceinline__ void init(const ConvBnBwd& e, int c) {
+#pragma unroll
+        for (int i = 0; i < 8; ++i) {
+            mu[i] = e.mean[c + i]; rs[i] = e.rstd[c + i]; ga[i] = e.gamma[c + i]; be[i] = e.beta[c + i];
+            s0[i] = 0.f; s1[i] = 0.f;
+        }
+    }
+};
+template <int BACT>
+__device__ __forceinline__ h16x8 bepi_piece(const h16x8 o, const ConvBnBwd& e, long off, BepiLane& L) {
+    const int act = BACT >= 0 ? BACT : e.act;
+    const h16x8 xv = *reinterpret_cast<const h16x8*>(e.x + off);
+    h16x8 rv = (h16x8)(h16)0;
+    if (e.res) rv = __builtin_nontemporal_load(reinterpret_cast<const h16x8*>(e.res + off));
+    h16x8 dz;
+#pragma unroll
+    for (int i = 0; i < 8; i += 2) {
+        const mu_f32x2 xh = (mu_f32x2{(float)xv[i], (float)xv[i + 1]} - mu_f32x2{L.mu[i], L.mu[i + 1]}) * mu_f32x2{L.rs[i], L.rs[i + 1]};
+        mu_f32x2 pre = __builtin_elementwise_fma(xh, mu_f32x2{L.ga[i], L.ga[i + 1]}, mu_f32x2{L.be[i], L.be[i + 1]});
+        if (e.res) pre += mu_f32x2{(float)rv[i], (float)rv[i + 1]};
+        float ag[2];
+        mu_act_grad2_t<true>(pre[0], pre[1], act, ag[0], ag[1]);
+        const mu_f32x2 dzf = mu_f32x2{(float)o[i], (float)o[i + 1]} * mu_f32x2{ag[0], ag[1]};
+        dz[i] = (h16)dzf[0];
+        dz[i + 1] = (h16)dzf[1];
+        const mu_f32x2 d = {(float)dz[i], (float)dz[i + 1]};
+        mu_f32x2 a0 = {L.s0[i], L.s0[i + 1]}, a1 = {L.s1[i], L.s1[i + 1]};
+        a0 += d;
+        a1 = __builtin_elementwise_fma(d, xh, a1);
+        L.s0[i] = a0[0]; L.s0[i + 1] = a0[1];
+        L.s1[i] = a1[0]; L.s1[i + 1] = a1[1];
+    }
+    return dz;
+}
+
+template <typename T, int TM, int TN, int WR, bool RINGP, bool FEPI, int HL = 0, int BACT = MU_NO_BEPI>
 __device__ __forceinline__ void conv_nt3_body(const T* __restrict__ x, const T* __restrict__ w, const float* __restrict__ bias,
                                               T* __restrict__ y, int B, int H, int W, int Cin, int Cout, long x_ld, long y_ld,
                                               const float* __restrict__ scale, const T* __restrict__ res, int act,
                                               float* __restrict__ stat_part = nullptr, float* __restrict__ yf = nullptr,
-                                              const float* __restrict__ oscale = nullptr) {
+                                              const float* __restrict__ oscale = nullptr, const ConvBnBwd& bnb = ConvBnBwd{}) {
+    constexpr bool BEPI = BACT != MU_NO_BEPI;
     using M_ = Mma<T>;
     using Frag = typename M_::Frag;
     constexpr int VN = M_::VN, KC = 8 * VN;
@@ -734,11 +779,14 @@
         }
         const int q = lane & 7;
         float ssum[8] = {0.f, 0.f, 0.f, 0.f, 0.f, 0.f, 0.f, 0.f}, ssq[8] = {0.f, 0.f, 0.f, 0.f, 0.f, 0.f, 0.f, 0.f};
+        BepiLane bl;
+        if constexpr (BEPI) bl.init(bnb, co0 + wr * 64 + q * 8);
 #pragma unroll
         for (int it = 0; it < TN * 2; ++it) {
             const int p = it * 8 + (lane >> 3);
             h16x8 o = *reinterpret_cast<const h16x8*>(Os + p * 128 + ((q ^ ((p >> 1) & 7)) << 4));
             const long gp = ((long)bimg * H + h0 + wc * TN + (p >> 4)) * W + w0 + (p & 15);
+            if constexpr (BEPI) o = bepi_piece<BACT>(o, bnb, gp * y_ld + co0 + wr * 64 + q * 8, bl);
             if constexpr (FEPI) {
                 h16x8 rv = (h16x8)(h16)0;
                 if (res) rv = *reinterpret_cast<const h16x8*>(res + gp * y_ld + co0 + wr * 64 + q * 8);
@@ -746,9 +794,10 @@
                 for (int e = 0; e < 8; ++e) o[e] = (h16)epi_act<T>((float)o[e] + (float)rv[e], act);
             }
             *reinterpret_cast<h16x8*>(y + gp * y_ld + co0 + wr * 64 + q * 8) = o;
-            if constexpr (!FEPI) { if (stat_part) tile_stats_accum(o, ssum, ssq); }
-        }
-        if constexpr (!FEPI) {
+            if constexpr (!FEPI && !BEPI) { if (stat_part) tile_stats_accum(o, ssum, ssq); }
+        }
+        if constexpr (BEPI) tile_stats_store(bl.s0, bl.s1, stat_part + ((long)tl * WC + wc) * Cout * 2, co0 + wr * 64 + q * 8, lane);
+        else if constexpr (!FEPI) {
             if (stat_part) tile_stats_store(ssum, ssq, stat_part + ((long)tl * WC + wc) * Cout * 2, co0 + wr * 64 + q * 8, lane);
         }
         return;
@@ -833,13 +882,23 @@
     conv_nt3_body<T, TM, TN, WR, false, true>(x, w, bias, y, B, H, W, Cin, Cout, x_ld, y_ld, scale, res, act);
 }
 
-template <bool FEPI, int HL = 0>
+template <int TN, int WR, bool RINGP, int BACT>
+__global__ __launch_bounds__(256, 2) void conv_nt3b_kernel(const h16* __restrict__ x, const h16* __restrict__ w, h16* __restrict__ y, int B, int H,
+                                                           int W, int Cin, int Cout, long x_ld, long y_ld, float* __restrict__ stat_part,
+                                                           const ConvBnBwd bnb) {
+    conv_nt3_body<h16, 4, TN, WR, RINGP, false, 0, BACT>(x, w, nullptr, y, B, H, W, Cin, Cout, x_ld, y_ld, nullptr, nullptr, 0, stat_part, nullptr,
+                                                         nullptr, bnb);
+}
+
+template <bool FEPI, int HL = 0, int BACT = MU_NO_BEPI>
 __device__ __forceinline__ void conv_nt4_body(const h16* __restrict__ x, const h16* __restrict__ w, const float* __restrict__ bias,
                                               h16* __restrict__ y, int B, int H, int W, int Cin, int Cout, long x_ld, long y_ld,
                                               float* __restrict__ stat_part, const float* __restrict__ scale, const h16* __restrict__ res, int act,
-                                              float* __restrict__ yf = nullptr, const float* __restrict__ oscale = nullptr) {
+                                              float* __restrict__ yf = nullptr, const float* __restrict__ oscale = nullptr,
+                                              const ConvBnBwd& bnb = ConvBnBwd{}) {
     using M_ = Mma<h16>;
     using Frag = M_::Frag;
+    constexpr bool BEPI = BACT != MU_NO_BEPI;
     constexpr int VN = 8, KC = 64, TM = 4, TN = 4, WC = 4, NWV = 8, BCO = 128;
     constexpr int TH = 16, TW = 16, HW_ = TW + 2, HROWS = (TH + 2) * HW_;
     constexpr int HINST = (HROWS + 7) / 8;
@@ -1017,11 +1076,14 @@
     }
     const int q = lane & 7;
     float ssum[8] = {0.f, 0.f, 0.f, 0.f, 0.f, 0.f, 0.f, 0.f}, ssq[8] = {0.f, 0.f, 0.f, 0.f, 0.f, 0.f, 0.f, 0.f};
+    BepiLane bl;
+    if constexpr (BEPI) bl.init(bnb, co0 + wr * 64 + q * 8);
 #pragma unroll
     for (int it = 0; it < 8; ++it) {
         const int p = it * 8 + (lane >> 3);
         h16x8 o = *reinterpret_cast<const h16x8*>(Os + p * 128 + ((q ^ ((p >> 1) & 7)) << 4));
         const long gp = ((long)bimg * H + h0 + wc * TN + (p >> 4)) * W + w0 + (p & 15);
+        if constexpr (BEPI) o = bepi_piece<BACT>(o, bnb, gp * y_ld + co0 + wr * 64 + q * 8, bl);
         if constexpr (FEPI) {
             h16x8 rv = (h16x8)(h16)0;
             if (res) rv = *reinterpret_cast<const h16x8*>(res + gp * y_ld + co0 + wr * 64 + q * 8);
@@ -1029,9 +1091,10 @@
             for (int e = 0; e < 8; ++e) o[e] = (h16)epi_act<h16>((float)o[e] + (float)rv[e], act);
         }
         *reinterpret_cast<h16x8*>(y + gp * y_ld + co0 + wr * 64 + q * 8) = o;
-        if (stat_part) tile_stats_accum(o, ssum, ssq);
-    }
-    if (stat_part) tile_stats_store(ssum, ssq, stat_part + ((long)tl * 4 + wc) * Cout * 2, co0 + wr * 64 + q * 8, lane);
+        if constexpr (!BEPI) { if (stat_part) tile_stats_accum(o, ssum, ssq); }
+    }
+    if constexpr (BEPI) tile_stats_store(bl.s0, bl.s1, stat_part + ((long)tl * 4 + wc) * Cout * 2, co0 + wr * 64 + q * 8, lane);
+    else if (stat_part) tile_stats_store(ssum, ssq, stat_part + ((long)tl * 4 + wc) * Cout * 2, co0 + wr * 64 + q * 8, lane);
 }
 
 __global__ __launch_bounds__(512, 1) void conv_nt4_kernel(const h16* __restrict__ x, const h16* __restrict__ w, const float* __restrict__ bias,
@@ -1048,6 +1111,12 @@
                                                            h16* __restrict__ y, int B, int H, int W, int Cin, int Cout, long x_ld, long y_ld,
                                                            const float* __restrict__ scale, const h16* __restrict__ res, int act) {
     conv_nt4_body<true>(x, w, bias, y, B, H, W, Cin, Cout, x_ld, y_ld, nullptr, scale, res, act);
+}
+template <int BACT>
+__global__ __launch_bounds__(512, 1) void conv_nt4b_kernel(const h16* __restrict__ x, const h16* __restrict__ w, h16* __restrict__ y, int B, int H,
+                                                           int W, int Cin, int Cout, long x_ld, long y_ld, float* __restrict__ stat_part,
+                                                           const ConvBnBwd bnb) {
+    conv_nt4_body<false, 0, BACT>(x, w, nullptr, y, B, H, W, Cin, Cout, x_ld, y_ld, stat_part, nullptr, nullptr, 0, nullptr, nullptr, bnb);
 }
 
 template <typename XT>
@@ -1240,9 +1309,11 @@
     }
 }
 
-__global__ __launch_bounds__(512, 1) void conv_nt4p_kernel(const h16* __restrict__ x, const h16* __restrict__ w, const float* __restrict__ bias,
-                                                           h16* __restrict__ y, int B, int H, int W, int Cin, int Cout, long x_ld, long y_ld,
-                                                           float* __restrict__ stat_part) {
+template <int BACT>
+__device__ __forceinline__ void conv_nt4p_body(const h16* __restrict__ x, const h16* __restrict__ w, const float* __restrict__ bias,
+                                               h16* __restrict__ y, int B, int H, int W, int Cin, int Cout, long x_ld, long y_ld,
+                                               float* __restrict__ stat_part, const ConvBnBwd& bnb = ConvBnBwd{}) {
+    constexpr bool BEPI = BACT != MU_NO_BEPI;
     using M_ = Mma<h16>;
     using Frag = M_::Frag;
     constexpr int VN = 8, KC = 64, TM = 4, TN = 4, NWV = 8, BCO = 128;
@@ -1412,18 +1483,42 @@
         {
             const int q = lane & 7;
             float ssum[8] = {0.f, 0.f, 0.f, 0.f, 0.f, 0.f, 0.f, 0.f}, ssq[8] = {0.f, 0.f, 0.f, 0.f, 0.f, 0.f, 0.f, 0.f};
+            BepiLane bl;
+            if constexpr (BEPI) {
+                int cq = co0 + wr * 64 + q * 8;
+                asm volatile("" : "+v"(cq));
+                bl.init(bnb, cq);
+            }
 #pragma unroll
             for (int it = 0; it < 8; ++it) {
                 const int p = it * 8 + (lane >> 3);
-                const h16x8 o = *reinterpret_cast<const h16x8*>(Os + p * 128 + ((q ^ ((p >> 1) & 7)) << 4));
+                h16x8 o = *reinterpret_cast<const h16x8*>(Os + p * 128 + ((q ^ ((p >> 1) & 7)) << 4));
                 const long gp = ((long)bimg * H + h0 + wc * TN + (p >> 4)) * W + w0 + (p & 15);
+                if constexpr (BEPI) {
+                    long off = gp * y_ld + co0 + wr * 64 + q * 8;
+                    asm volatile("" : "+v"(off));
+                    o = bepi_piece<BACT>(o, bnb, off, bl);
+                    *reinterpret_cast<h16x8*>(y + off) = o;
+                } else
                 *reinterpret_cast<h16x8*>(y + gp * y_ld + co0 + wr * 64 + q * 8) = o;
-                if (stat_part) tile_stats_accum(o, ssum, ssq);
-            }
-            if (stat_part) tile_stats_store(ssum, ssq, stat_part + ((long)tl * 4 + wc) * Cout * 2, co0 + wr * 64 + q * 8, lane);
+                if constexpr (!BEPI) { if (stat_part) tile_stats_accum(o, ssum, ssq); }
+            }
+            if constexpr (BEPI) tile_stats_store(bl.s0, bl.s1, stat_part + ((long)tl * 4 + wc) * Cout * 2, co0 + wr * 64 + q * 8, lane);
+            else if (stat_part) tile_stats_store(ssum, ssq, stat_part + ((long)tl * 4 + wc) * Cout * 2, co0 + wr * 64 + q * 8, lane);
         }
         if (has_next && wr == 1) __builtin_amdgcn_s_barrier();
     }
+}
+__global__ __launch_bounds__(512, 1) void conv_nt4p_kernel(const h16* __restrict__ x, const h16* __restrict__ w, const float* __restrict__ bias,
+                                                           h16* __restrict__ y, int B, int H, int W, int Cin, int Cout, long x_ld, long y_ld,
+                                                           float* __restrict__ stat_part) {
+    conv_nt4p_body<MU_NO_BEPI>(x, w, bias, y, B, H, W, Cin, Cout, x_ld, y_ld, stat_part);
+}
+template <int BACT>
+__global__ __launch_bounds__(512, 1) void conv_nt4pb_kernel(const h16* __restrict__ x, const h16* __restrict__ w, h16* __restrict__ y, int B, int H,
+                                                            int W, int Cin, int Cout, long x_ld, long y_ld, float* __restrict__ stat_part,
+                                                            const ConvBnBwd bnb) {
+    conv_nt4p_body<BACT>(x, w, nullptr, y, B, H, W, Cin, Cout, x_ld, y_ld, stat_part, bnb);
 }
 
 __global__ __launch_bounds__(512, 1) void conv_nt5_kernel(const h16* __restrict__ x, const h16* __restrict__ w, const float* __restrict__ bias,
@@ -1844,6 +1939,55 @@
         return MU_OK;
     });
     if (rc) return rc;
+    MU_CHECK_LAUNCH();
+    return MU_OK;
+}
+
+static Conv3x3Plan conv_bnbwd_pick(const ConvGeom& g, int Cin, int Cout, int taps, int dtype) {
+    if (taps != 9 || dtype != MU_F16) return {K3_NONE, 0};
+    const Conv3x3Kernel plain = conv3x3_pick(g, Cin, Cout, dtype, false).kernel;
+    if (plain == K3_NT5 || plain == K3_NT5_HALVES) return {K3_NONE, 0};
+    const Conv3x3Plan p = conv3x3_pick(g, Cin, Cout, dtype, true);
+    switch (p.kernel) {
+    case K3_NT4P: case K3_NT4: case K3_NT3_128: case K3_NT3_64_RING: case K3_NT3_64: return p;
+    default: return {K3_NONE, 0};
+    }
+}
+
+extern "C" int mu_conv_bnbwd_rows(int B, int H, int W, int Cin, int Cout, int taps, int dtype) {
+    if (!conv_plan_args_ok(B, H, W, Cin, Cout, taps, dtype)) return 0;
+    return conv_bnbwd_pick(conv_geom(B, H, W), Cin, Cout, taps, dtype).stat_rows;
+}
+
+template <int BACT>
+static void conv_bnbwd_launch(Conv3x3Kernel k, const h16* x, const h16* w, h16* dz, const ConvGeom& g, int Cin, int Cout, long x_ld, long y_ld,
+                              float* stat_part, const ConvBnBwd& e, hipStream_t st) {
+    const int B = g.B, H = g.H, W = g.W, t16 = (int)g.t16, t8 = (int)g.t8;
+    switch (k) {
+    case K3_NT4P: conv_nt4pb_kernel<BACT><<<256, 512, 0, st>>>(x, w, dz, B, H, W, Cin, Cout, x_ld, y_ld, stat_part, e); break;
+    case K3_NT4: conv_nt4b_kernel<BACT><<<t16 * (Cout / 128), 512, 0, st>>>(x, w, dz, B, H, W, Cin, Cout, x_ld, y_ld, stat_part, e); break;
+    case K3_NT3_128: conv_nt3b_kernel<4, 2, false, BACT><<<t8 * (Cout / 128), 256, 0, st>>>(x, w, dz, B, H, W, Cin, Cout, x_ld, y_ld, stat_part, e); break;
+    case K3_NT3_64_RING: conv_nt3b_kernel<2, 1, true, BACT><<<t8 * (Cout / 64), 256, 0, st>>>(x, w, dz, B, H, W, Cin, Cout, x_ld, y_ld, stat_part, e); break;
+    case K3_NT3_64: conv_nt3b_kernel<2, 1, false, BACT><<<t8 * (Cout / 64), 256, 0, st>>>(x, w, dz, B, H, W, Cin, Cout, x_ld, y_ld, stat_part, e); break;
+    default: break;
+    }
+}
+
+extern "C" int mu_conv_fwd_bnbwd(const void* x, const void* w, void* dz, int B, int H, int W, int Cin, int Cout, int taps, long x_ld, long y_ld,
+                                 const void* bn_x, const void* bn_res, const float* mean, const float* rstd, const float* gamma,
+                                 const float* beta, int act, int dtype, float* stat_part, void* stream) {
+    if (const int rc = conv_io_check(x && w && dz && bn_x && mean && rstd && gamma && beta && stat_part && B > 0 && H > 0 && W > 0, Cin, Cout,
+                                     x_ld, y_ld)) return rc;
+    if (taps != 9 || (dtype != MU_F32 && dtype != MU_F16 && dtype != MU_F32X)) return MU_ERR_ARG;
+    if (act < MU_ACT_NONE || act > MU_ACT_RELU) return MU_ERR_ARG;
+    const ConvGeom g = conv_geom(B, H, W);
+    const Conv3x3Plan p = conv_bnbwd_pick(g, Cin, Cout, taps, dtype);
+    if (p.stat_rows == 0) return MU_ERR_SHAPE;
+    const ConvBnBwd e{(const h16*)bn_x, (const h16*)bn_res, mean, rstd, gamma, beta, act};
+    if (act == MU_ACT_GELU)
+        conv_bnbwd_launch<MU_ACT_GELU>(p.kernel, (const h16*)x, (const h16*)w, (h16*)dz, g, Cin, Cout, x_ld, y_ld, stat_part, e, (hipStream_t)stream);
+    else
+        conv_bnbwd_launch<-1>(p.kernel, (const h16*)x, (const h16*)w, (h16*)dz, g, Cin, Cout, x_ld, y_ld, stat_part, e, (hipStream_t)stream);
     MU_CHECK_LAUNCH();
     return MU_OK;
 }
diff --git a/maskunet_amd/csrc/norm.hip b/maskunet_amd/csrc/norm.hip
--- a/maskunet_amd/csrc/norm.hip
+++ b/maskunet_amd/csrc/norm.hip
@@ -171,7 +171,8 @@
     else { mean[c] = 0.f; rstd[c] = 1.f; }
 }
 
-__global__ void bn_bwd_final_kernel(const double* __restrict__ part, int nblk, int C, long M, int training,
+template <bool FROWS = false>
+__global__ void bn_bwd_final_kernel(const void* __restrict__ part_, int nblk, int C, long M, int training,
                                     float* __restrict__ dgamma, float* __restrict__ dbeta, float* __restrict__ s1, float* __restrict__ s2,
                                     const float* __restrict__ xscale = nullptr, const float* __restrict__ pc2 = nullptr,
                                     const float* __restrict__ pc1 = nullptr, float* __restrict__ pair_grads = nullptr,
@@ -183,8 +184,14 @@
 #pragma unroll
     for (int u = 0; u < MU_STAT_MAXBLK / 64; ++u) {
         const int k = lane + 64 * u;
-        const double2 v = k < nblk ? *reinterpret_cast<const double2*>(part + ((long)k * C + c) * 2) : make_double2(0.0, 0.0);
-        av[u] = v.x; bv[u] = v.y;
+        if constexpr (FROWS) {
+            const float2 v = k < nblk ? *reinterpret_cast<const float2*>(reinterpret_cast<const float*>(part_) + ((long)k * C + c) * 2) : make_float2(0.f, 0.f);
+            av[u] = (double)v.x; bv[u] = (double)v.y;
+        } else {
+            const double* part = reinterpret_cast<const double*>(part_);
+            const double2 v = k < nblk ? *reinterpret_cast<const double2*>(part + ((long)k * C + c) * 2) : make_double2(0.0, 0.0);
+            av[u] = v.x; bv[u] = v.y;
+        }
     }
     float2 pv[MU_STAT_MAXBLK / 64];
     if (bound) {
@@ -635,7 +642,7 @@
     } else {
         MU_BN_ACT_SWITCH(a.act, (bn_partial_kernel<T, 1, A_, 0, ENC><<<nblk, 256, sg.lds, st>>>(a.x, a.g, nullptr, nullptr, a.M, a.C, a.ld, a.mean, a.rstd, a.gamma, a.beta, a.act, ws.part, pmax)))
     }
-    bn_bwd_final_kernel<<<mu_cdiv(a.C, 4), 256, 0, st>>>(ws.part, nblk, a.C, a.M, a.training, a.dgamma, a.dbeta, ws.s1, ws.s2, a.xscale, a.pc2, a.pc1, a.pair_grads,
+    bn_bwd_final_kernel<false><<<mu_cdiv(a.C, 4), 256, 0, st>>>(ws.part, nblk, a.C, a.M, a.training, a.dgamma, a.dbeta, ws.s1, ws.s2, a.xscale, a.pc2, a.pc1, a.pair_grads,
                                                          pmax, ENC ? a.gamma : nullptr, ENC ? a.rstd : nullptr, bound);
     if (a.res) bn_bwd_apply_kernel<T, false, ENC><<<agrid, 256, 0, st>>>(a.x, a.dres, a.dx, a.M, a.C, a.ld, a.mean, a.rstd, a.gamma, a.beta, a.act, ws.s1, ws.s2, bound, a.dy_scale);
     else { MU_BN_ACT_SWITCH(a.act, (bn_bwd_apply_kernel<T, true, ENC, A_><<<agrid, 256, 0, st>>>(a.x, a.g, a.dx, a.M, a.C, a.ld, a.mean, a.rstd, a.gamma, a.beta, a.act, ws.s1, ws.s2, bound, a.dy_scale))) }
@@ -664,6 +671,32 @@
                              float* dgamma, float* dbeta, void* workspace, long ws_bytes, int dtype, void* stream) {
     return mu_bn_act_bwd_scaled(x, res, grad_out, dx, dres, M, C, ld, mean, rstd, gamma, beta, act, training, dgamma, dbeta, nullptr,
                                 workspace, ws_bytes, dtype, stream);
+}
+
+extern "C" int mu_bn_bwd_rows(const void* bn_x, const void* dz, void* dx, long M, int C, long ld, const float* stat_part, int rows,
+                              const float* mean, const float* rstd, const float* gamma, const float* beta, float* dgamma, float* dbeta,
+                              void* workspace, long ws_bytes, int dtype, void* stream) {
+    if (!bn_x || !dz || !dx || !stat_part || !mean || !rstd || !gamma || !beta || !dgamma || !dbeta || !workspace) return MU_ERR_ARG;
+    if (M <= 0 || C <= 0 || C % 8 || ld < C || rows <= 0 || rows > M) return MU_ERR_ARG;
+    if (ws_bytes < BnWs::bytes(C)) return MU_ERR_WORKSPACE;
+    if (dtype != MU_F16) return MU_ERR_ARG;
+    StatGeom sg;
+    if (int e = stat_geom(C, Vec16<h16>::N, sg)) return e;
+    const BnWs ws(workspace, C);
+    hipStream_t st = (hipStream_t)stream;
+    if (rows <= MU_STAT_MAXBLK) {
+        bn_bwd_final_kernel<true><<<mu_cdiv(C, 4), 256, 0, st>>>(stat_part, rows, C, M, 1, dgamma, dbeta, ws.s1, ws.s2);
+    } else {
+        int rpb = 16;
+        if ((rows + rpb - 1) / rpb > MU_STAT_MAXBLK) rpb = ((rows + MU_STAT_MAXBLK - 1) / MU_STAT_MAXBLK + 7) / 8 * 8;
+        const int nblk = (rows + rpb - 1) / rpb;
+        bn_fold_rows_kernel<<<nblk, 256, 0, st>>>(stat_part, rows, rpb, 2 * C, ws.part);
+        bn_bwd_final_kernel<false><<<mu_cdiv(C, 4), 256, 0, st>>>(ws.part, nblk, C, M, 1, dgamma, dbeta, ws.s1, ws.s2);
+    }
+    bn_bwd_apply_kernel<h16, false><<<ew_grid(M * sg.cv, sg.cv), 256, 0, st>>>((const h16*)bn_x, (const h16*)dz, (h16*)dx, M, C, ld, mean, rstd, gamma, beta, 0,
+                                                                              ws.s1, ws.s2);
+    MU_CHECK_LAUNCH();
+    return MU_OK;
 }
 
 __global__ void bn_pair_compose_kernel(const float* __restrict__ rstd1, const float* __restrict__ gamma1, const float* __restrict__ beta1,
diff --git a/maskunet_amd/ops.py b/maskunet_amd/ops.py
--- a/maskunet_amd/ops.py
+++ b/maskunet_amd/ops.py
@@ -660,6 +660,33 @@
     return _BNAct.apply(x, res, bn.weight, bn.bias, bn, act, stats)
 
 
+def _conv_bn_bwd(conv_saved, bn_saved, gy, needs):
+    (cx, weight), m = conv_saved
+    (x, res, mean, rstd, g_p, b_p), (act, training, cv) = bn_saved
+    if not (needs[0] and training and m.taps == 9 and not m.is_x and not m.has_bias and gy.dtype == torch.float16 and x.dtype == torch.float16):
+        return None
+    rows_of = getattr(_lib.load(), "mu_conv_bnbwd_rows", None)
+    B, H, W, C = x.shape
+    Cd = gy.shape[-1]
+    rows = rows_of(B, H, W, Cd, C, 9, _lib.MU_F16) if rows_of is not None else 0
+    if rows <= 0 or tuple(cx.shape) != tuple(x.shape):
+        return None
+    gy = gy.contiguous()
+    M = B * H * W
+    dz = torch.empty_like(x)
+    part = torch.empty((rows, C, 2), dtype=torch.float32, device=x.device)
+    call("mu_conv_fwd_bnbwd", ptr(gy), ptr(_take_wd(m, weight, gy.dtype, C, Cd)), ptr(dz), B, H, W, Cd, C, 9, Cd, C, ptr(x), ptr(res),
+         ptr(mean), ptr(rstd), ptr(g_p), ptr(b_p), act, _lib.MU_F16, ptr(part), stream())
+    _, gw, _ = _conv_bwd(conv_saved, gy, (False, needs[1], False))
+    dgamma = torch.empty(C, dtype=torch.float32, device=x.device)
+    dbeta = torch.empty_like(dgamma)
+    ws = workspace(_lib.load().mu_bn_workspace_bytes(C), x.device)
+    dx = torch.empty_like(x) if res is not None else dz
+    call("mu_bn_bwd_rows", ptr(x), ptr(dz), ptr(dx), M, C, C, ptr(part), rows, ptr(mean), ptr(rstd), ptr(g_p), ptr(b_p), ptr(dgamma),
+         ptr(dbeta), ptr(ws), ws.numel(), _lib.MU_F16, stream())
+    return dx, (dz if res is not None else None), dgamma[:cv], dbeta[:cv], gw
+
+
 _keep_graph = getattr(torch._C._autograd, "_get_current_graph_task_keep_graph", lambda: True)
 
 
@@ -717,21 +744,36 @@
         grads = [None] * (len(ctx.needs_input_grad) - 2)
         if ctx.tail:
             gy, _, grads[-2], grads[-1] = _bn_act_bwd(units.pop(), gy)
+        done = None
         for i in reversed(range(len(ctx.plan))):
             residual, n1, h1, n2, h2 = ctx.plan[i]
             k, dres = 6 * i, None
-            if ctx.fold and i == len(ctx.plan) - 1:
+            if done is not None:
+                units.pop()
+                (gy, dres, grads[k + 4], grads[k + 5]), done = done, None
+            elif ctx.fold and i == len(ctx.plan) - 1:
                 gy, grads[k + 4], grads[k + 5], grads[-2], grads[-1] = _bn_pair_bwd(units.pop(), gy, h2)
             else:
                 gy, dres, grads[k + 4], grads[k + 5] = _bn_act_bwd(units.pop(), gy, h2)
             if dres is not None and i == 0 and ctx.link is not None:
                 ctx.link.put(dres)
                 dres = None
-            gy, grads[k + 3], _ = _conv_bwd(units.pop(), gy, n2)
-            if gy is None:
-                break
-            gy, _, grads[k + 1], grads[k + 2] = _bn_act_bwd(units.pop(), gy, h1)
-            gy, grads[k], _ = _conv_bwd(units.pop(), gy, n1)
+            c2 = units.pop()
+            pair = _conv_bn_bwd(c2, units[-1], gy, n2)
+            if pair is not None:
+                units.pop()
+                gy, _, grads[k + 1], grads[k + 2], grads[k + 3] = pair
+            else:
+                gy, grads[k + 3], _ = _conv_bwd(c2, gy, n2)
+                if gy is None:
+                    break
+                gy, _, grads[k + 1], grads[k + 2] = _bn_act_bwd(units.pop(), gy, h1)
+            c1 = units.pop()
+            pair = _conv_bn_bwd(c1, units[-1], gy, n1) if (i > 0 and dres is None) else None
+            if pair is not None:
+                done, grads[k] = pair[:4], pair[4]
+                continue
+            gy, grads[k], _ = _conv_bwd(c1, gy, n1)
             if gy is None:
                 break
             if dres is not None:
```

New measurement: 2316 images/sec, median of 6. About the same (+0.6%).
